# fuxiao0719/PanopticNeRF

Hardware: AMD Instinct MI355X
Metric: Msamples/sec (coarse+fine), KITTI-360 1408x376 (higher is better)
Workload: dtype bf16

## Files before the change

include/pnr.h:

```cpp
#ifndef PNR_H
#define PNR_H
#include <stdint.h>

#ifdef __cplusplus
extern "C" {
#endif

#define PNR_OK 0
#define PNR_EINVAL (-1)
#define PNR_EHIP (-2)
#define PNR_ENODEV (-3)

#define PNR_PREC_BF16 0
#define PNR_PREC_FP32 1

int pnr_version(void);
const char* pnr_last_error(void);
int pnr_device_check(int dev, char* buf_host, int buflen);

int pnr_stratified(const float* rays, int64_t n_rays, int n_samples, int lindisp,
                   const float* t_rand, float* z_out, void* stream);

int pnr_points(const float* rays, const float* z, int64_t n_rays, int n_samples, float* pts_out,
               void* stream);

int pnr_embed(const float* x, int64_t n, int L, float* out, void* stream);

typedef struct pnr_mlp_desc {
    int32_t D, W, skip;
    int32_t xyz_L, dir_L;
    int32_t n_sem, n_inst, head_W;
    int32_t precision;
    int32_t plan;
    int32_t head_tap;
    int32_t head_depth;
    int32_t schedule;
    int32_t clk_probe[2];
    int32_t flags;
} pnr_mlp_desc;

#define PNR_MLP_SOFTMAX 1
#define PNR_MLP_WG_CAP(n) (((n) & 0x1FF) << 16)
#define PNR_MLP_TRACE 0x7A00

typedef struct pnr_mlp_params_host {
    const float* const* pts_w; const float* const* pts_b;
    const float* alpha_w; const float* alpha_b;
    const float* feature_w; const float* feature_b;
    const float* views_w; const float* views_b;
    const float* rgb_w; const float* rgb_b;
    const float* sem0_w; const float* sem0_b; const float* sem1_w; const float* sem1_b;
    const float* inst0_w; const float* inst0_b; const float* inst1_w; const float* inst1_b;
} pnr_mlp_params_host;

int64_t pnr_mlp_packed_bytes(const pnr_mlp_desc* desc);
int pnr_mlp_pack(const pnr_mlp_desc* desc, const pnr_mlp_params_host* params, void* packed_host);

int64_t pnr_mlp_pack_workspace_bytes(const pnr_mlp_desc* desc, int backward);
int pnr_mlp_pack_device(const pnr_mlp_desc* desc, const pnr_mlp_params_host* params_dev, int backward,
                        void* workspace, void* packed, void* stream);
int pnr_mlp_repack_device(const pnr_mlp_desc* desc, const pnr_mlp_params_host* params_dev, int backward,
                          void* workspace, void* packed, void* stream);

int pnr_mlp_forward(const pnr_mlp_desc* desc, const void* packed, const float* rays, const float* z,
                    int64_t n_rays, int n_samples, float* raw, int64_t raw_stride_s,
                    int64_t raw_stride_c, void* stream);

int pnr_mlp_fused_plan(const pnr_mlp_desc* desc);
int64_t pnr_mlp_forward_composite_workspace_bytes(const pnr_mlp_desc* desc, int64_t n_rays, int n_samples, int want_weights);
int pnr_mlp_forward_composite(const pnr_mlp_desc* desc, const void* packed, const float* rays, const float* z,
                              int64_t n_rays, int n_samples, const int32_t* label_sem, const int32_t* label_inst,
                              int white_bkgd, float* rgb, float* depth, float* acc, float* weights, float* sem,
                              float* inst, float* fix_sem, float* fix_inst, void* workspace, void* stream);

int pnr_mlp_forward_tiles(const pnr_mlp_desc* desc, const void* packed, const float* rays, const float* z, int64_t n_rays,
                          int n_samples, void* workspace, void* stream);
int pnr_composite_combine(const pnr_mlp_desc* desc, const void* workspace, const float* z, int64_t n_rays, int n_samples,
                          const int32_t* label_sem, const int32_t* label_inst, int white_bkgd, float* rgb, float* depth,
                          float* acc, float* weights, float* sem, float* inst, float* fix_sem, float* fix_inst, void* stream);

int pnr_mlp_query(const pnr_mlp_desc* desc, const void* packed, const float* points, int64_t n_points,
                  float* sigma, int32_t* sem_label, int32_t* inst_label, int32_t* panoptic, const int32_t* is_thing,
                  float* sem_logits, float* inst_logits, int64_t logit_stride, void* stream);
int pnr_mlp_query_supported(const pnr_mlp_desc* desc);

int pnr_mlp_train_layout(const pnr_mlp_desc* desc, int64_t n_samples, int64_t* acts_off_host ,
                         int64_t* dys_off_host );
int pnr_mlp_forward_train(const pnr_mlp_desc* desc, const void* packed, const float* rays, const float* z,
                          int64_t n_rays, int n_samples, float* raw, int64_t raw_stride_s,
                          int64_t raw_stride_c, void* acts, void* stream);
int64_t pnr_mlp_bwd_packed_bytes(const pnr_mlp_desc* desc);
int pnr_mlp_pack_bwd(const pnr_mlp_desc* desc, const pnr_mlp_params_host* params, void* packed_host);
int pnr_mlp_backward(const pnr_mlp_desc* desc, const void* packed_bwd, const float* d_raw, const void* acts,
                     void* dys, int64_t n_rays, int n_samples, void* stream);

int64_t pnr_mlp_wgrad_workspace_bytes(const pnr_mlp_desc* desc, int64_t n_samples);
int pnr_mlp_wgrad(const pnr_mlp_desc* desc, const void* acts, const void* dys, int64_t n_samples,
                  const pnr_mlp_params_host* grads_dev, void* workspace, void* stream);

int64_t pnr_mlp_fp32_acts_floats(const pnr_mlp_desc* desc, int64_t n_samples);
int64_t pnr_mlp_backward_fp32_workspace_bytes(const pnr_mlp_desc* desc, int64_t n_samples);
int pnr_mlp_forward_train_fp32(const pnr_mlp_desc* desc, const pnr_mlp_params_host* params_dev, const float* rays,
                               const float* z, int64_t n_rays, int n_samples, float* raw, int64_t raw_stride_s,
                               int64_t raw_stride_c, float* acts, void* stream);
int pnr_mlp_backward_fp32(const pnr_mlp_desc* desc, const pnr_mlp_params_host* params_dev, const float* d_raw,
                          int64_t d_raw_stride_c, const float* acts, int64_t n_rays, int n_samples,
                          const pnr_mlp_params_host* grads_dev, void* workspace, void* stream);

int pnr_composite(const float* raw, int64_t raw_stride_s, int64_t raw_stride_c, const float* z,
                  const float* rays, const float* noise, const int32_t* label_sem,
                  const int32_t* label_inst, int64_t n_rays, int n_samples, int n_sem, int n_inst,
                  int sem_mode, int white_bkgd, float* rgb, float* depth, float* acc, float* weights,
                  float* sem, float* inst, float* fix_sem, float* fix_inst, void* stream);

int pnr_composite_backward(const float* raw, int64_t raw_stride_c, const float* z, const float* rays,
                           const float* noise, int64_t n_rays, int n_samples, int n_sem, int n_inst,
                           const float* g_rgb, const float* g_depth, const float* g_acc, const float* g_sem,
                           const float* g_inst, const float* g_weights, float* d_raw, void* stream);

int pnr_composite_backward2(const float* raw, int64_t raw_stride_c, const float* z, const float* rays,
                            const float* noise, int64_t n_rays, int n_samples, int n_sem, int n_inst,
                            const float* g_rgb, const float* g_depth, const float* g_acc, const float* g_sem,
                            const float* g_inst, const float* g_weights, const int32_t* label_sem,
                            const int32_t* label_inst, const float* g_fix_sem, const float* g_fix_inst,
                            const float* ce_sem, const float* ce_inst, float* d_raw, void* stream);
int pnr_composite_backward3(const float* raw, int64_t raw_stride_c, const float* z, const float* rays,
                            const float* noise, int64_t n_rays, int n_samples, int n_sem, int n_inst, int sem_mode,
                            const float* g_rgb, const float* g_depth, const float* g_acc, const float* g_sem,
                            const float* g_inst, const float* g_weights, const int32_t* label_sem,
                            const int32_t* label_inst, const float* g_fix_sem, const float* g_fix_inst,
                            const float* ce_sem, const float* ce_inst, float* d_raw, void* stream);

typedef struct pnr_loss_cfg {
    float w_rgb, w_depth, w_sem, w_fix_sem, w_inst, w_fix_inst;
    int32_t depth_l2;
    float fix_eps;
    int32_t maps_are_prob;
} pnr_loss_cfg;
int64_t pnr_losses_workspace_bytes(int64_t n_rays);
int pnr_losses(const pnr_loss_cfg* cfg, int64_t n_rays, int n_sem, int n_inst, const float* rgb, const float* depth,
               const float* sem, const float* fix_sem, const float* inst, const float* fix_inst, const float* rgb_gt,
               const float* depth_gt, const int32_t* sem_gt, const int32_t* inst_gt, float* losses_out, float* g_rgb,
               float* g_depth, float* g_sem, float* g_fix_sem, float* g_inst, float* g_fix_inst, void* workspace, void* stream);

int64_t pnr_ce3d_workspace_bytes(int64_t n_samples);
int pnr_ce3d(const float* raw, int64_t raw_stride_c, int first_channel, int n_classes, const int32_t* label,
             int64_t n_samples, float* out2, void* workspace, void* stream);

int pnr_gen_rays(const float* intr4_host, const float* c2w12_host, int width, int height, float near_, float far_,
                 const int32_t* pix, int64_t n_rays, float* rays, void* stream);

#define PNR_FISHEYE_NEWTON_STEPS 8
#define PNR_CAMERA_PINHOLE 0
#define PNR_CAMERA_FISHEYE 1
#define PNR_CAMERA_EQUIRECT 3

#define PNR_SINPI_P0 0x1.921fb6p+1f
#define PNR_SINPI_P1 -0x1.4abbcep+2f
#define PNR_SINPI_P2 0x1.466bc6p+1f
#define PNR_SINPI_P3 -0x1.32d2ccp-1f
#define PNR_SINPI_P4 0x1.507834p-4f
#define PNR_COSPI_Q0 0x1.000000p+0f
#define PNR_COSPI_Q1 -0x1.3bd3ccp+2f
#define PNR_COSPI_Q2 0x1.03c1f0p+2f
#define PNR_COSPI_Q3 -0x1.55d3c8p+0f
#define PNR_COSPI_Q4 0x1.e1f506p-3f
#define PNR_COSPI_Q5 -0x1.a6d1f2p-6f
#define PNR_ATANPI_A0 0x1.45f306p-2f
#define PNR_ATANPI_A1 -0x1.b29948p-4f
#define PNR_ATANPI_A2 0x1.04bc78p-4f
#define PNR_ATANPI_A3 -0x1.7352dap-5f
#define PNR_ATANPI_A4 0x1.13b6a6p-5f
#define PNR_ATANPI_A5 -0x1.3ab9c6p-6f
#define PNR_TAN_PI_8 0x1.a8279ap-2f

int pnr_gen_rays_fisheye(const float* cam7_host, const float* c2w12_host, int width, int height, float near_, float far_,
                         const int32_t* pix, int64_t n_rays, float* rays, uint8_t* valid, void* stream);

int pnr_gen_rays_equirect(const float* cam4_host, const float* c2w12_host, int width, int height, float near_, float far_,
                          const int32_t* pix, int64_t n_rays, float* rays, void* stream);

int pnr_project_points(int model, const float* cam_host, const float* w2c12_host, int width, int height, const float* points,
                       int64_t n, float* uv, float* range, uint8_t* valid, void* stream);

int pnr_reproject(int model_src, const float* cam_src_host, const float* c2w_src12_host, int width_src, int height_src,
                  const int32_t* pix, int64_t n, const float* depth_src,
                  int model_tgt, const float* cam_tgt_host, const float* w2c_tgt12_host, int width_tgt, int height_tgt,
                  const float* depth_tgt, float tol_abs, float tol_rel,
                  const int32_t* label_src, const int32_t* label_tgt, int n_classes,
                  int32_t* match, float* uv, int64_t* agree, int64_t* stats, void* stream);

int pnr_splat_points(int model, const float* cam_host, const float* w2c12_host, int width, int height, const float* points,
                     int64_t n, int64_t index_base, float near_, float far_, int radius, int64_t* zbuf, int64_t* stats,
                     void* stream);
int pnr_splat_resolve(const int64_t* zbuf, int64_t n_pix, float* depth, int32_t* index, void* stream);
int64_t pnr_depth_metrics_workspace_bytes(int64_t n);
int pnr_depth_metrics(const float* pred, const float* gt, const uint8_t* mask, int64_t n, float d_min, float d_max,
                      double* sums, int64_t* counts, void* workspace, void* stream);

int pnr_census(const uint8_t* img, int width, int height, int64_t* out, void* stream);
int64_t pnr_sgm_workspace_bytes(int width, int height, int max_disp, int paths);
int pnr_sgm_aggregate(const int64_t* census_l, const int64_t* census_r, int width, int height, int max_disp, int p1, int p2,
                      int paths, uint16_t* S, void* workspace, void* stream);
int pnr_sgm_select(const uint16_t* S, int width, int height, int max_disp, int uniqueness, int lr_tol, int16_t* d16,
                   int16_t* disp_right, void* stream);
int pnr_disparity_depth(const int16_t* d16, int64_t n, float fb, float d_min, float d_max, float* depth, void* stream);

int64_t pnr_mesh_workspace_bytes(int res_x, int res_y, int res_z);
int pnr_mesh_count(const float* field, int res_x, int res_y, int res_z, float level, void* workspace, int64_t* totals, void* stream);
int pnr_mesh_emit(const float* field, int res_x, int res_y, int res_z, float level, const float* lo_host, const float* step_host,
                  const void* workspace, float* vertices, int32_t* faces, int64_t* src, void* stream);

#define PNR_NN_PAD 1.0009765625f
#define PNR_NN_CELL_CLAMP 1048576.0f
#define PNR_NN_HASH_X 73856093u
#define PNR_NN_HASH_Y 19349663u
#define PNR_NN_HASH_Z 83492791u
#define PNR_NN_MAX_TABLE 268435456
#define PNR_CLOUD_MAX_TAU 8
#define PNR_SAMPLE_MAX_PER_FACE 65535
int64_t pnr_nn_workspace_bytes(int64_t n, int64_t table_size);
int pnr_nn_build(const float* ref, int64_t n, float max_dist, int64_t table_size, int32_t* start, float* records, void* workspace,
                 void* stream);
int pnr_nn_query(const float* ref, int64_t n, float max_dist, int64_t table_size, const int32_t* start, const float* records,
                 const float* query, int64_t m, int32_t* index, float* dist2, int64_t* stats, void* stream);
int64_t pnr_cloud_metrics_workspace_bytes(int64_t m);
int pnr_cloud_metrics(const int32_t* index, const float* dist2, const float* query, int64_t m, float max_dist,
                      const float* tau_host, int n_tau, double* sums, int64_t* counts, void* workspace, void* stream);
int64_t pnr_mesh_sample_workspace_bytes(int64_t n_faces);
int pnr_mesh_sample_count(const float* vertices, int64_t n_vertices, const int32_t* faces, int64_t n_faces, float rho, int64_t seed,
                          int32_t* start, int64_t* total, void* workspace, void* stream);
int pnr_mesh_sample_emit(const float* vertices, int64_t n_vertices, const int32_t* faces, int64_t n_faces, int64_t seed,
// ... 175 lines not shown
```

panopticnerf_amd/_lib.py:

```python
import ctypes
import os

_HERE = os.path.dirname(os.path.abspath(__file__))
LIB_PATH = os.environ.get("PNR_LIB_PATH") or os.path.join(_HERE, "libpnr.so")

c_f = ctypes.c_void_p
c_i64 = ctypes.c_int64
c_int = ctypes.c_int

PREC_BF16, PREC_FP32 = 0, 1
MLP_SOFTMAX, MLP_TRACE = 1, 0x7A00
CAMERA_PINHOLE, CAMERA_FISHEYE, CAMERA_EQUIRECT = 0, 1, 3
TAG_PIXEL, TAG_FRAME = 16, 17
SAMPLE_POOLED, SAMPLE_FRAME = 0, 1
NORMAL_OK, NORMAL_NO_DEPTH, NORMAL_NO_NEIGHBOUR, NORMAL_DEGENERATE, NORMAL_GRAZING = 0, 1, 2, 3, 4
MESHCAST_MAX_RES, MESHCAST_MAX_REACH, MESHCAST_PAD = 1024, 4096.0, 0.0625
DEPTH_MAX_RADIUS = 8
CC_KEYS, CC_VALUES = 0, 1
CC_TILE_2D, CC_TILE_3D = (32, 8), (8, 8, 4)
NN_MAX_TABLE, CLOUD_MAX_TAU, SAMPLE_MAX_PER_FACE = 1 << 28, 8, 65535


class LossCfg(ctypes.Structure):
    _fields_ = [("w_rgb", ctypes.c_float), ("w_depth", ctypes.c_float), ("w_sem", ctypes.c_float),
# ... 12 lines not shown
class RngDesc(ctypes.Structure):
    _fields_ = [("call", ctypes.c_void_p), ("ray_base", ctypes.c_int64), ("tag", ctypes.c_int32), ("scale", ctypes.c_float)]


class Frame(ctypes.Structure):
    _fields_ = [("model", ctypes.c_int32), ("width", ctypes.c_int32), ("height", ctypes.c_int32), ("cam", ctypes.c_float * 7),
                ("c2w", ctypes.c_float * 12), ("near_", ctypes.c_float), ("far_", ctypes.c_float), ("n_valid", ctypes.c_int64),
                ("valid_pix", ctypes.c_uint64), ("rgb", ctypes.c_uint64), ("depth", ctypes.c_uint64), ("sem", ctypes.c_uint64),
                ("inst", ctypes.c_uint64)]


_fp = ctypes.POINTER(ctypes.c_float)
_fpp = ctypes.POINTER(_fp)


class MlpParamsHost(ctypes.Structure):
    _fields_ = [("pts_w", _fpp), ("pts_b", _fpp),
                ("alpha_w", _fp), ("alpha_b", _fp), ("feature_w", _fp), ("feature_b", _fp),
                ("views_w", _fp), ("views_b", _fp), ("rgb_w", _fp), ("rgb_b", _fp),
                ("sem0_w", _fp), ("sem0_b", _fp), ("sem1_w", _fp), ("sem1_b", _fp),
                ("inst0_w", _fp), ("inst0_b", _fp), ("inst1_w", _fp), ("inst1_b", _fp)]


SIGNATURES = {
    "pnr_version": (c_int, []),
    "pnr_last_error": (ctypes.c_char_p, []),
    "pnr_device_check": (c_int, [c_int, ctypes.c_char_p, c_int]),
    "pnr_stratified": (c_int, [c_f, c_i64, c_int, c_int, c_f, c_f, c_f]),
    "pnr_points": (c_int, [c_f, c_f, c_i64, c_int, c_f, c_f]),
    "pnr_embed": (c_int, [c_f, c_i64, c_int, c_f, c_f]),
    "pnr_mlp_packed_bytes": (c_i64, [ctypes.POINTER(MlpDesc)]),
    "pnr_mlp_pack": (c_int, [ctypes.POINTER(MlpDesc), ctypes.POINTER(MlpParamsHost), ctypes.c_void_p]),
    "pnr_mlp_pack_workspace_bytes": (c_i64, [ctypes.POINTER(MlpDesc), c_int]),
    "pnr_mlp_pack_device": (c_int, [ctypes.POINTER(MlpDesc), ctypes.POINTER(MlpParamsHost), c_int, c_f, c_f, c_f]),
    "pnr_mlp_repack_device": (c_int, [ctypes.POINTER(MlpDesc), ctypes.POINTER(MlpParamsHost), c_int, c_f, c_f, c_f]),
    "pnr_mlp_forward": (c_int, [ctypes.POINTER(MlpDesc), c_f, c_f, c_f, c_i64, c_int, c_f, c_i64, c_i64, c_f]),
    "pnr_mlp_train_layout": (c_int, [ctypes.POINTER(MlpDesc), c_i64, ctypes.POINTER(c_i64), ctypes.POINTER(c_i64)]),
    "pnr_mlp_forward_train": (c_int, [ctypes.POINTER(MlpDesc), c_f, c_f, c_f, c_i64, c_int, c_f, c_i64, c_i64, c_f, c_f]),
    "pnr_mlp_bwd_packed_bytes": (c_i64, [ctypes.POINTER(MlpDesc)]),
    "pnr_mlp_pack_bwd": (c_int, [ctypes.POINTER(MlpDesc), ctypes.POINTER(MlpParamsHost), ctypes.c_void_p]),
    "pnr_mlp_backward": (c_int, [ctypes.POINTER(MlpDesc), c_f, c_f, c_f, c_f, c_i64, c_int, c_f]),
    "pnr_mlp_wgrad_workspace_bytes": (c_i64, [ctypes.POINTER(MlpDesc), c_i64]),
    "pnr_mlp_wgrad": (c_int, [ctypes.POINTER(MlpDesc), c_f, c_f, c_i64, ctypes.POINTER(MlpParamsHost), c_f, c_f]),
    "pnr_mlp_fp32_acts_floats": (c_i64, [ctypes.POINTER(MlpDesc), c_i64]),
    "pnr_mlp_backward_fp32_workspace_bytes": (c_i64, [ctypes.POINTER(MlpDesc), c_i64]),
    "pnr_mlp_forward_train_fp32": (c_int, [ctypes.POINTER(MlpDesc), ctypes.POINTER(MlpParamsHost), c_f, c_f, c_i64, c_int, c_f, c_i64,
                                           c_i64, c_f, c_f]),
    "pnr_mlp_backward_fp32": (c_int, [ctypes.POINTER(MlpDesc), ctypes.POINTER(MlpParamsHost), c_f, c_i64, c_f, c_i64, c_int,
                                      ctypes.POINTER(MlpParamsHost), c_f, c_f]),
    "pnr_mlp_fused_plan": (c_int, [ctypes.POINTER(MlpDesc)]),
    "pnr_mlp_forward_composite_workspace_bytes": (c_i64, [ctypes.POINTER(MlpDesc), c_i64, c_int, c_int]),
    "pnr_mlp_forward_composite": (c_int, [ctypes.POINTER(MlpDesc), c_f, c_f, c_f, c_i64, c_int, c_f, c_f, c_int,
                                          c_f, c_f, c_f, c_f, c_f, c_f, c_f, c_f, c_f, c_f]),
    "pnr_composite": (c_int, [c_f, c_i64, c_i64, c_f, c_f, c_f, c_f, c_f, c_i64, c_int, c_int, c_int, c_int,
                              c_int, c_f, c_f, c_f, c_f, c_f, c_f, c_f, c_f, c_f]),
    "pnr_composite_backward": (c_int, [c_f, c_i64, c_f, c_f, c_f, c_i64, c_int, c_int, c_int,
                                       c_f, c_f, c_f, c_f, c_f, c_f, c_f, c_f]),
    "pnr_composite_backward2": (c_int, [c_f, c_i64, c_f, c_f, c_f, c_i64, c_int, c_int, c_int,
                                        c_f, c_f, c_f, c_f, c_f, c_f, c_f, c_f, c_f, c_f, c_f, c_f, c_f, c_f]),
    "pnr_composite_backward3": (c_int, [c_f, c_i64, c_f, c_f, c_f, c_i64, c_int, c_int, c_int, c_int,
                                        c_f, c_f, c_f, c_f, c_f, c_f, c_f, c_f, c_f, c_f, c_f, c_f, c_f, c_f]),
    "pnr_losses_workspace_bytes": (c_i64, [c_i64]),
    "pnr_losses": (c_int, [ctypes.POINTER(LossCfg), c_i64, c_int, c_int] + [c_f] * 19),
    "pnr_ce3d_workspace_bytes": (c_i64, [c_i64]),
    "pnr_ce3d": (c_int, [c_f, c_i64, c_int, c_int, c_f, c_i64, c_f, c_f, c_f]),
    "pnr_gen_rays": (c_int, [ctypes.POINTER(ctypes.c_float), ctypes.POINTER(ctypes.c_float), c_int, c_int, ctypes.c_float,
                             ctypes.c_float, c_f, c_i64, c_f, c_f]),
    "pnr_gen_rays_fisheye": (c_int, [ctypes.POINTER(ctypes.c_float), ctypes.POINTER(ctypes.c_float), c_int, c_int, ctypes.c_float,
                                     ctypes.c_float, c_f, c_i64, c_f, c_f, c_f]),
    "pnr_gen_rays_equirect": (c_int, [ctypes.POINTER(ctypes.c_float), ctypes.POINTER(ctypes.c_float), c_int, c_int, ctypes.c_float,
                                      ctypes.c_float, c_f, c_i64, c_f, c_f]),
    "pnr_project_points": (c_int, [c_int, ctypes.POINTER(ctypes.c_float), ctypes.POINTER(ctypes.c_float), c_int, c_int, c_f, c_i64,
                                   c_f, c_f, c_f, c_f]),
    "pnr_reproject": (c_int, [c_int, ctypes.POINTER(ctypes.c_float), ctypes.POINTER(ctypes.c_float), c_int, c_int, c_f, c_i64, c_f,
                              c_int, ctypes.POINTER(ctypes.c_float), ctypes.POINTER(ctypes.c_float), c_int, c_int, c_f,
                              ctypes.c_float, ctypes.c_float, c_f, c_f, c_int, c_f, c_f, c_f, c_f, c_f]),
    "pnr_splat_points": (c_int, [c_int, ctypes.POINTER(ctypes.c_float), ctypes.POINTER(ctypes.c_float), c_int, c_int, c_f, c_i64, c_i64,
                                 ctypes.c_float, ctypes.c_float, c_int, c_f, c_f, c_f]),
    "pnr_splat_resolve": (c_int, [c_f, c_i64, c_f, c_f, c_f]),
    "pnr_depth_metrics_workspace_bytes": (c_i64, [c_i64]),
    "pnr_depth_metrics": (c_int, [c_f, c_f, c_f, c_i64, ctypes.c_float, ctypes.c_float, c_f, c_f, c_f, c_f]),
    "pnr_census": (c_int, [c_f, c_int, c_int, c_f, c_f]),
    "pnr_sgm_workspace_bytes": (c_i64, [c_int, c_int, c_int, c_int]),
    "pnr_sgm_aggregate": (c_int, [c_f, c_f, c_int, c_int, c_int, c_int, c_int, c_int, c_f, c_f, c_f]),
    "pnr_sgm_select": (c_int, [c_f, c_int, c_int, c_int, c_int, c_int, c_f, c_f, c_f]),
    "pnr_disparity_depth": (c_int, [c_f, c_i64, ctypes.c_float, ctypes.c_float, ctypes.c_float, c_f, c_f]),
    "pnr_mesh_workspace_bytes": (c_i64, [c_int, c_int, c_int]),
    "pnr_mesh_count": (c_int, [c_f, c_int, c_int, c_int, ctypes.c_float, c_f, c_f, c_f]),
    "pnr_mesh_emit": (c_int, [c_f, c_int, c_int, c_int, ctypes.c_float, ctypes.POINTER(ctypes.c_float), ctypes.POINTER(ctypes.c_float),
                              c_f, c_f, c_f, c_f, c_f]),
    "pnr_nn_workspace_bytes": (c_i64, [c_i64, c_i64]),
    "pnr_nn_build": (c_int, [c_f, c_i64, ctypes.c_float, c_i64, c_f, c_f, c_f, c_f]),
    "pnr_nn_query": (c_int, [c_f, c_i64, ctypes.c_float, c_i64, c_f, c_f, c_f, c_i64, c_f, c_f, c_f, c_f]),
    "pnr_cloud_metrics_workspace_bytes": (c_i64, [c_i64]),
    "pnr_cloud_metrics": (c_int, [c_f, c_f, c_f, c_i64, ctypes.c_float, ctypes.POINTER(ctypes.c_float), c_int, c_f, c_f, c_f, c_f]),
    "pnr_cc_workspace_bytes": (c_i64, [c_i64]),
    "pnr_cc_label": (c_int, [c_f, c_int, ctypes.c_float, c_int, c_int, c_int, c_int, c_f, c_f, c_f, c_f, c_f]),
    "pnr_cc_mesh": (c_int, [c_f, c_i64, c_i64, c_f, c_f, c_f, c_f, c_f, c_f]),
    "pnr_cc_stats": (c_int, [c_f, c_f, c_int, c_int, c_int, c_i64, c_f, c_f, c_f]),
    "pnr_mesh_sample_workspace_bytes": (c_i64, [c_i64]),
    "pnr_mesh_sample_count": (c_int, [c_f, c_i64, c_f, c_i64, ctypes.c_float, c_i64, c_f, c_f, c_f, c_f]),
    "pnr_mesh_sample_emit": (c_int, [c_f, c_i64, c_f, c_i64, c_i64, c_f, c_i64, c_f, c_f, c_f]),
    "pnr_mesh_grid_workspace_bytes": (c_i64, [c_int, c_int, c_int]),
    "pnr_mesh_grid_bounds": (c_int, [c_f, c_i64, c_f, c_i64, c_f, c_f, c_f]),
    "pnr_mesh_grid_count": (c_int, [c_f, c_i64, c_f, c_i64, c_int, c_int, c_int, ctypes.POINTER(ctypes.c_float), ctypes.POINTER(ctypes.c_float),
                                    c_f, c_f, c_f, c_f]),
    "pnr_mesh_grid_fill": (c_int, [c_f, c_i64, c_f, c_i64, c_int, c_int, c_int, ctypes.POINTER(ctypes.c_float), ctypes.POINTER(ctypes.c_float),
                                   c_f, c_i64, c_f, c_f, c_f]),
    "pnr_mesh_raycast": (c_int, [c_int, ctypes.POINTER(ctypes.c_float), ctypes.POINTER(ctypes.c_float), c_int, c_int, ctypes.c_float,
                                 ctypes.c_float, c_f, c_i64, c_f, c_i64, c_int, c_int, c_int, ctypes.POINTER(ctypes.c_float),
                                 ctypes.POINTER(ctypes.c_float), c_f, c_f, c_i64, c_f, c_f, c_f, c_f, c_f, c_f, c_f, c_f]),
    "pnr_mesh_cast_rays": (c_int, [c_f, c_i64, c_f, c_i64, c_f, c_i64, c_int, c_int, c_int, ctypes.POINTER(ctypes.c_float),
                                   ctypes.POINTER(ctypes.c_float), c_f, c_f, c_i64, c_f, c_f, c_f, c_f, c_f, c_f, c_f, c_f]),
    "pnr_tsdf_integrate": (c_int, [c_f, c_f, c_int, c_int, c_int, c_int, c_int, ctypes.POINTER(ctypes.c_float), ctypes.POINTER(ctypes.c_float),
                                   ctypes.c_float, ctypes.c_float, ctypes.c_float, c_f, c_f, c_f, c_f, c_f, c_f, c_f]),
    "pnr_tsdf_raycast": (c_int, [c_int, ctypes.POINTER(ctypes.c_float), ctypes.POINTER(ctypes.c_float), c_int, c_int, ctypes.c_float,
                                 ctypes.c_float, c_int, c_int, c_int, ctypes.POINTER(ctypes.c_float), ctypes.POINTER(ctypes.c_float),
                                 c_f, c_f, ctypes.c_float, ctypes.c_float, c_int, c_f, c_f, c_f, c_f, c_f]),
    "pnr_icp_workspace_bytes": (c_i64, [c_i64]),
    "pnr_icp_accumulate": (c_int, [c_int, ctypes.POINTER(ctypes.c_float), c_int, c_int, c_f, c_f, c_int, ctypes.POINTER(ctypes.c_float),
                                   ctypes.POINTER(ctypes.c_float), ctypes.POINTER(ctypes.c_float), c_int, c_int, c_f, c_f, ctypes.c_float,
                                   c_f, c_f, c_f, c_f]),
    "pnr_icp_solve": (c_int, [c_f, c_i64, c_i64, ctypes.c_float, ctypes.c_float, c_int, c_f, c_f, c_f]),
    "pnr_depth_filter": (c_int, [c_int, c_int, c_f, c_int, ctypes.POINTER(ctypes.c_float), ctypes.c_float, ctypes.c_float, c_int, c_f, c_f, c_f]),
    "pnr_depth_normals": (c_int, [c_int, ctypes.POINTER(ctypes.c_float), ctypes.POINTER(ctypes.c_float), c_int, c_int, c_f, ctypes.c_float,
                                  ctypes.c_float, ctypes.c_float, c_f, c_f, c_f, c_f]),
    "pnr_panoptic_labels": (c_int, [c_f, c_f, c_f, c_i64, c_int, c_int, c_f, c_f, c_f, c_f]),
    "pnr_confusion": (c_int, [c_f, c_f, c_i64, c_int, c_f, c_f]),
    "pnr_sample_pdf": (c_int, [c_f, c_f, c_f, c_i64, c_int, c_int, c_f, c_f, c_f, c_f]),
    "pnr_bbox_hits": (c_int, [c_f, c_i64, c_f, c_int, c_int, c_f, c_f, c_f, c_f]),
    "pnr_convex_hits": (c_int, [c_f, c_i64, c_f, c_f, c_int, c_int, c_f, c_f, c_f, c_f]),
    "pnr_restrict_rays": (c_int, [c_f, c_i64, c_f, c_f, c_int, c_f, c_f]),
    "pnr_sample_labels": (c_int, [c_f, c_i64, c_int, c_f, c_f, c_f, c_int, c_f, c_f, c_f, c_f]),
    "pnr_ray_setup": (c_int, [c_f, c_i64, c_f, c_int, c_int, c_f, c_int, c_int, c_f, c_int, c_f, c_f, c_f, c_f, c_f, c_f, c_f]),
    "pnr_sample_pdf_labels": (c_int, [c_f, c_f, c_f, c_i64, c_int, c_int, c_f, c_f, c_f, c_f, c_int, c_f, c_f, c_f, c_f]),
    "pnr_mlp_forward_tiles": (c_int, [ctypes.POINTER(MlpDesc), c_f, c_f, c_f, c_i64, c_int, c_f, c_f]),
    "pnr_rng_begin": (c_int, [c_f, c_f, c_f]),
    "pnr_rng_fill": (c_int, [ctypes.POINTER(RngDesc), c_i64, c_int, c_int, c_f, c_f]),
    "pnr_stratified_rng": (c_int, [c_f, c_i64, c_int, c_int, ctypes.POINTER(RngDesc), c_f, c_f]),
    "pnr_ray_setup_rng": (c_int, [c_f, c_i64, c_f, c_int, c_int, c_f, c_int, c_int, ctypes.POINTER(RngDesc), c_int, c_f, c_f, c_f, c_f,
                                  c_f, c_f, c_f]),
    "pnr_sample_pdf_rng": (c_int, [c_f, c_f, ctypes.POINTER(RngDesc), c_i64, c_int, c_int, c_f, c_f, c_f, c_f]),
    "pnr_sample_pdf_labels_rng": (c_int, [c_f, c_f, ctypes.POINTER(RngDesc), c_i64, c_int, c_int, c_f, c_f, c_f, c_f, c_int, c_f, c_f, c_f,
                                          c_f]),
    "pnr_composite_rng": (c_int, [c_f, c_i64, c_i64, c_f, c_f, ctypes.POINTER(RngDesc), c_f, c_f, c_i64, c_int, c_int, c_int, c_int,
                                  c_int, c_f, c_f, c_f, c_f, c_f, c_f, c_f, c_f, c_f]),
    "pnr_composite_backward_rng": (c_int, [c_f, c_i64, c_f, c_f, ctypes.POINTER(RngDesc), c_i64, c_int, c_int, c_int, c_int,
                                           c_f, c_f, c_f, c_f, c_f, c_f, c_f, c_f, c_f, c_f, c_f, c_f, c_f, c_f]),
    "pnr_sample_batch": (c_int, [c_f, c_f, c_f, c_int, ctypes.POINTER(RngDesc), c_i64, c_f, c_f, c_f, c_f, c_f, c_f, c_f, c_f]),
    "pnr_mlp_query": (c_int, [ctypes.POINTER(MlpDesc), c_f, c_f, c_i64, c_f, c_f, c_f, c_f, c_f, c_f, c_f, c_i64, c_f]),
    "pnr_mlp_query_supported": (c_int, [ctypes.POINTER(MlpDesc)]),
    "pnr_composite_combine": (c_int, [ctypes.POINTER(MlpDesc), c_f, c_f, c_i64, c_int, c_f, c_f, c_int,
                                      c_f, c_f, c_f, c_f, c_f, c_f, c_f, c_f, c_f]),
}

_lib = None


def load():
    global _lib
    if _lib is not None:
        return _lib
    if not os.path.exists(LIB_PATH):
        raise RuntimeError(
            f"{LIB_PATH} not found: the HIP extension is not built. Run "
            "`python -c 'import __graft_entry__ as g; g.build()'` (or `make -C panopticnerf_amd/csrc`). "
            "There is no CPU fallback.")
    lib = ctypes.CDLL(LIB_PATH)
    for name, (res, args) in SIGNATURES.items():
        fn = getattr(lib, name)
        fn.restype = res
        fn.argtypes = args
    _lib = lib
    return lib


def check(rc, what):
    if rc != 0:
        msg = load().pnr_last_error().decode(errors="replace")
        raise RuntimeError(f"{what} failed (code {rc}): {msg}")
```

panopticnerf_amd/csrc/pnr_composite.hip:

```cpp
#include "pnr_composite_dev.h"

struct CompositeArgs {
    const float* raw; int64_t stride_s, stride_c;
    const float* z; const float* rays; const float* noise;
    const int32_t* label_sem; const int32_t* label_inst;
    int64_t R; int N, C, K, sem_mode, white_bkgd;
    float *rgb, *depth, *acc, *weights, *sem, *inst, *fix_sem, *fix_inst;
    int use_hist;
};

#ifndef CMP_GRID_PER_CU
#define CMP_GRID_PER_CU 8
#endif
#ifndef CMP_UB
#define CMP_UB 8
#endif

__device__ __forceinline__ float dot4(const f4& w, const f4& v)
{
    return fmaf(w.v[3], v.v[3], fmaf(w.v[2], v.v[2], fmaf(w.v[1], v.v[1], w.v[0] * v.v[0])));
}

template <bool CH_MAJOR, int SUB, bool SOFTMAX, class... Rng>
__global__ __launch_bounds__(256) void k_composite(CompositeArgs a, const Rng... rng)
// ... 145 lines not shown
            add_sigma_noise4<RNG>(w + 4 * j, act[j], key, (uint32_t)ray, (uint32_t)((i0 >> 2) + j), a.noise, a.noise + s0 + 4 * j);
        const float dn = ray_dir_norm(a.rays, rl.rayc);
        const float znext = dpp_or<0x101>(zz[0], 0.0f);
        float alpha[M], Tl[M];
        float P = alpha_chain<M>(zz, znext, w, i0, N, dn, alpha, Tl);
        if (!act[0]) P = 1.0f;
        const float excl = scan_excl_dpp<L>(P, q);
        float accp = 0.0f, depp = 0.0f;
#pragma unroll
        for (int k = 0; k < M; ++k) {
            w[k] = act[k >> 2] ? (alpha[k] * Tl[k]) * excl : 0.0f;
            accp += w[k];
            depp = fmaf(w[k], zz[k], depp);
        }
        if (a.weights) {
#pragma unroll
            for (int j = 0; j < M4; ++j) st4(a.weights + s0 + 4 * j, w + 4 * j, act[j]);
        }
        const float accv = group_sum<L>(accp);
        const float depv = group_sum<L>(depp);
        if (writer) {
            if (a.depth) a.depth[ray] = depv;
            if (a.acc) a.acc[ray] = accv;
        }

        const bool want_fs = a.fix_sem && a.label_sem && a.C, want_fi = a.fix_inst && a.label_inst && a.K;
        if (want_fs || want_fi) {
            hist_zero<L>(hist, q, CK);
#pragma unroll
            for (int j = 0; j < M4; ++j) {
                int ls[4], li[4];
                ld4_labels(a.label_sem + s0 + 4 * j, act[j] && want_fs, ls);
                ld4_labels(a.label_inst + s0 + 4 * j, act[j] && want_fi, li);
#pragma unroll
                for (int k = 0; k < 4; ++k) hist_add(hist, w[4 * j + k], want_fs, ls[k], a.C, want_fi, li[k], a.K);
            }
            if (rl.valid) hist_store<L>(hist, q, ray, want_fs, a.fix_sem, a.C, want_fi, a.fix_inst, a.K);
        }

        float mx_s[SOFTMAX ? M : 1], den_s[SOFTMAX ? M : 1], mx_i[SOFTMAX ? M : 1], den_i[SOFTMAX ? M : 1];
        if constexpr (SOFTMAX) {
            auto field_stats = [&](int nch, int ch0, float (&mx)[M], float (&den)[M]) {
#pragma unroll
                for (int k = 0; k < M; ++k) { mx[k] = -INFINITY; den[k] = 0.0f; }
                for (int c = 0; c < nch; ++c) {
                    float v[M];
                    ld_row<M4>(a.raw + (int64_t)(ch0 + c) * sc + s0, act, v);
#pragma unroll
                    for (int k = 0; k < M; ++k) lse_step(mx[k], den[k], v[k]);
                }
            };
            field_stats(a.C, 4, mx_s, den_s);
            field_stats(a.K, 4 + a.C, mx_i, den_i);
        }

#pragma unroll 1
        for (int q0 = 0; q0 < nq; q0 += CMP2_UB) {
            float r[CMP2_UB];
#pragma unroll
            for (int j = 0; j < CMP2_UB; ++j) {
                const int qq = q0 + j;
                float acc = 0.0f;
#pragma unroll
                for (int k = 0; k < M; ++k) {
                    float v = nxt[j][k];
                    if (qq < 3) v = sigmoid_of(v);
                    else if constexpr (SOFTMAX) {
                        const bool fs = (qq - 3) < a.C;
                        v = softmax_of(v, fs ? mx_s[k] : mx_i[k], fs ? den_s[k] : den_i[k]);
                    }
                    acc = fmaf(w[k], v, acc);
                }
                r[j] = acc;
                const int q2 = qq + CMP2_UB;
                if (q2 < nq) ld_row<M4>(a.raw + (int64_t)(q2 + 1) * sc + s0, act, nxt[j]);
            }
            group_sum_batch<L, CMP2_UB>(r);
            if (writer) store_rows<CMP2_UB>(a, ray, q0, nq, r, accv);
        }
    }
}

static int composite_impl(const float* raw, int64_t raw_stride_s, int64_t raw_stride_c, const float* z, const float* rays,
                          const float* noise, const PnrRngDev* rng, const int32_t* label_sem, const int32_t* label_inst, int64_t n_rays,
                          int n_samples, int n_sem, int n_inst, int sem_mode, int white_bkgd, float* rgb, float* depth, float* acc,
                          float* weights, float* sem, float* inst, float* fix_sem, float* fix_inst, void* stream)
{
    PNR_REQUIRE(n_rays <= 0 || (raw && z && rays), "pnr_composite: null pointer");
    PNR_REQUIRE(n_samples >= 4 && n_samples <= 256 && (n_samples % 4) == 0,
                "pnr_composite: n_samples=%d must be a multiple of 4 in [4,256]", n_samples);
    PNR_REQUIRE(n_sem >= 0 && n_inst >= 0 && (sem_mode == 0 || sem_mode == 1), "pnr_composite: bad field sizes");
    PNR_REQUIRE((((uintptr_t)z) & 15) == 0, "pnr_composite: z must be 16-byte aligned");
    PNR_REQUIRE(!weights || (((uintptr_t)weights) & 15) == 0, "pnr_composite: weights must be 16-byte aligned");
    PNR_REQUIRE((((uintptr_t)noise) & 15) == 0 && (((uintptr_t)label_sem) & 15) == 0 && (((uintptr_t)label_inst) & 15) == 0,
                "pnr_composite: noise / label arrays must be 16-byte aligned");
    if (n_rays <= 0) return PNR_OK;
    CompositeArgs a;
    a.raw = raw; a.stride_s = raw_stride_s; a.stride_c = raw_stride_c; a.z = z; a.rays = rays; a.noise = noise;
    a.label_sem = label_sem; a.label_inst = label_inst; a.R = n_rays; a.N = n_samples; a.C = n_sem; a.K = n_inst;
    a.sem_mode = sem_mode; a.white_bkgd = white_bkgd; a.rgb = rgb; a.depth = depth; a.acc = acc; a.weights = weights;
    a.sem = sem; a.inst = inst; a.fix_sem = fix_sem; a.fix_inst = fix_inst;
    const bool want_fix = (fix_sem && label_sem && n_sem) || (fix_inst && label_inst && n_inst);
    const bool ch_major = raw_stride_s == 1 && (raw_stride_c % 4) == 0 && (((uintptr_t)raw) & 15) == 0;
    hipStream_t st = (hipStream_t)stream;
    auto hist_bytes = [&](int rpw) { return (size_t)4 * rpw * (n_sem + n_inst) * sizeof(uint32_t); };
    auto grid_for = [&](int rpw) { return pnr_grid_cap(((n_rays + rpw - 1) / rpw + 3) / 4, CMP_GRID_PER_CU); };
    if (ch_major && n_samples > 32 && n_samples <= 64 && (!want_fix || hist_bytes(8) <= 48 * 1024)) {
        a.use_hist = want_fix ? 1 : 0;
        const size_t lds = want_fix ? hist_bytes(8) : 0;
        composite_dispatch<8>(8, true, sem_mode, rng, [&](auto L, auto, auto SM, const auto&... r) {
            hipLaunchKernelGGL((k_composite2<decltype(L)::value, 2, decltype(SM)::value, std::decay_t<decltype(r)>...>), dim3(grid_for(8)), dim3(256),
                               lds, st, a, r...);
        });
        PNR_CHECK_LAUNCH("pnr_composite");
        return PNR_OK;
    }
    int sub = 1;
    while (sub < n_samples / 4) sub <<= 1;
    const int rpw = 64 / sub;
    a.use_hist = (want_fix && hist_bytes(rpw) <= 48 * 1024) ? 1 : 0;
    const size_t lds = a.use_hist ? hist_bytes(rpw) : 0;
    composite_dispatch<1, 2, 4, 8, 16, 32, 64>(sub, ch_major, sem_mode, rng, [&](auto S, auto CH, auto SM, const auto&... r) {
        hipLaunchKernelGGL((k_composite<decltype(CH)::value, decltype(S)::value, decltype(SM)::value, std::decay_t<decltype(r)>...>),
                           dim3(grid_for(rpw)), dim3(256), lds, st, a, r...);
    });
    PNR_CHECK_LAUNCH("pnr_composite");
    return PNR_OK;
}

PNR_EXPORT int pnr_composite(const float* raw, int64_t raw_stride_s, int64_t raw_stride_c, const float* z,
                             const float* rays, const float* noise, const int32_t* label_sem,
                             const int32_t* label_inst, int64_t n_rays, int n_samples, int n_sem, int n_inst,
                             int sem_mode, int white_bkgd, float* rgb, float* depth, float* acc, float* weights,
                             float* sem, float* inst, float* fix_sem, float* fix_inst, void* stream)
{
    return composite_impl(raw, raw_stride_s, raw_stride_c, z, rays, noise, nullptr, label_sem, label_inst, n_rays, n_samples, n_sem, n_inst,
                          sem_mode, white_bkgd, rgb, depth, acc, weights, sem, inst, fix_sem, fix_inst, stream);
}

PNR_EXPORT int pnr_composite_rng(const float* raw, int64_t raw_stride_s, int64_t raw_stride_c, const float* z, const float* rays,
                                 const pnr_rng* noise_host, const int32_t* label_sem, const int32_t* label_inst, int64_t n_rays,
                                 int n_samples, int n_sem, int n_inst, int sem_mode, int white_bkgd, float* rgb, float* depth, float* acc,
                                 float* weights, float* sem, float* inst, float* fix_sem, float* fix_inst, void* stream)
{
    PnrRngDev rng;
    const int rc = pnr_rng_check(noise_host, n_rays < 0 ? 0 : n_rays, "pnr_composite_rng", &rng);
    if (rc) return rc;
    PNR_REQUIRE(n_rays <= 0 || (raw_stride_s == 1 && (raw_stride_c % 4) == 0 && (((uintptr_t)raw) & 15) == 0),
                "pnr_composite_rng: channel-major, 16-byte aligned raw images only");
    return composite_impl(raw, raw_stride_s, raw_stride_c, z, rays, nullptr, &rng, label_sem, label_inst, n_rays, n_samples, n_sem, n_inst,
                          sem_mode, white_bkgd, rgb, depth, acc, weights, sem, inst, fix_sem, fix_inst, stream);
}

struct CombineArgs {
    const float* rec; int rec_floats; const float4* ps; const float* z; const int32_t* lab_s; const int32_t* lab_i;
    int64_t R; int N, C, K, white_bkgd;
    float *rgb, *depth, *acc, *weights, *sem, *inst, *fix_sem, *fix_inst;
};

template <bool LOGITS>
__global__ __launch_bounds__(256) void k_composite_combine(CombineArgs a)
{
    __shared__ uint32_t hist_all[4][128];
    const int lane = threadIdx.x & 63, wv = threadIdx.x >> 6;
    const int64_t ray = ((int64_t)blockIdx.x * blockDim.x + threadIdx.x) >> 6;
    if (ray >= a.R) return;
    const int N = a.N, T = N >> 5, RF = a.rec_floats, C = a.C, K = a.K, CK = C + K;
    const float* __restrict__ rec = a.rec + ray * T * RF;
    const float4* __restrict__ ps = a.ps + ray * N;
    const float* __restrict__ zr = a.z + ray * N;
    const bool want_s = a.lab_s && a.fix_sem && C, want_i = a.lab_i && a.fix_inst && K;
    const int32_t* __restrict__ lsr = want_s ? a.lab_s + ray * N : nullptr;
    const int32_t* __restrict__ lir = want_i ? a.lab_i + ray * N : nullptr;
    float q[8];
#pragma unroll
    for (int k = 0; k < 8; ++k) q[k] = k < T ? rec[k * RF] : 1.0f;
    float4 pv[4];
    float zv[4];
    int lsv[4], liv[4];
#pragma unroll
    for (int j = 0; j < 4; ++j) {
        const int i = lane + 64 * j;
        const bool in = i < N;
        pv[j] = in ? ps[i] : float4{0.0f, 0.0f, 0.0f, 0.0f};
        zv[j] = in ? zr[i] : 0.0f;
        lsv[j] = (in && want_s) ? lsr[i] : -1;
        liv[j] = (in && want_i) ? lir[i] : -1;
    }
    float lg[2][8];
#pragma unroll
    for (int h = 0; h < 2; ++h)
#pragma unroll
        for (int k = 0; k < 8; ++k) lg[h][k] = (LOGITS && k < T && lane + 64 * h < CK) ? rec[k * RF + PNR_FUSE_REC_LOGITS + lane + 64 * h] : 0.0f;
    float Tk[8];
    float t = 1.0f;
#pragma unroll
    for (int k = 0; k < 8; ++k) {
        Tk[k] = t;
        if (k < T) t *= q[k];
    }
    uint32_t* hist = hist_all[wv];
    if (want_s || want_i) hist_zero<64>(hist, lane, CK);
    float r5[5] = {0.0f, 0.0f, 0.0f, 0.0f, 0.0f};
#pragma unroll
    for (int j = 0; j < 4; ++j) {
        const int i = lane + 64 * j;
        if (i < N) {
            const float4 p = pv[j];
            float tk = Tk[0];
#pragma unroll
            for (int k = 1; k < 8; ++k) tk = (i >> 5) == k ? Tk[k] : tk;
            const float w = tk * p.x;
            r5[0] += w;
            r5[1] = fmaf(w, zv[j], r5[1]);
            r5[2] = fmaf(w, sigmoid_of(p.y), r5[2]);
            r5[3] = fmaf(w, sigmoid_of(p.z), r5[3]);
            r5[4] = fmaf(w, sigmoid_of(p.w), r5[4]);
            if (a.weights) a.weights[ray * N + i] = w;
            if (want_s || want_i) hist_add(hist, w, want_s, lsv[j], C, want_i, liv[j], K);
        }
    }
    group_sum_batch<64, 5>(r5);
    if (lane == 0) {
        if (a.acc) a.acc[ray] = r5[0];
        if (a.depth) a.depth[ray] = r5[1];
    }
    if (lane < 3 && a.rgb) {
        const float v = lane == 0 ? r5[2] : lane == 1 ? r5[3] : r5[4];
        a.rgb[ray * 3 + lane] = a.white_bkgd ? v + (1.0f - r5[0]) : v;
    }
#pragma unroll
    for (int h = 0; h < 2; ++h) {
        const int c = lane + 64 * h;
        if (c >= CK) continue;
        if constexpr (LOGITS) {
            float v = 0.0f;
#pragma unroll
            for (int k = 0; k < 8; ++k) if (k < T) v = fmaf(Tk[k], lg[h][k], v);
            if (c < C) { if (a.sem) a.sem[ray * C + c] = v; }
            else if (a.inst) a.inst[ray * K + (c - C)] = v;
        }
        if (c < C) { if (want_s) a.fix_sem[ray * C + c] = hist_read(hist, c); }
        else if (want_i) a.fix_inst[ray * K + (c - C)] = hist_read(hist, c);
    }
}

int pnr_composite_combine_launch(const float* rec, int rec_floats, bool logit_sums, const float4* ps, const float* z,
                                 const int32_t* label_sem, const int32_t* label_inst, int64_t R, int N, int C, int K, int white_bkgd,
                                 float* rgb, float* depth, float* acc, float* weights, float* sem, float* inst, float* fix_sem,
                                 float* fix_inst, hipStream_t st)
{
    CombineArgs a;
    a.rec = rec; a.rec_floats = rec_floats; a.ps = ps; a.z = z; a.lab_s = label_sem; a.lab_i = label_inst;
    a.R = R; a.N = N; a.C = C; a.K = K; a.white_bkgd = white_bkgd;
    a.rgb = rgb; a.depth = depth; a.acc = acc; a.weights = weights; a.sem = sem; a.inst = inst; a.fix_sem = fix_sem; a.fix_inst = fix_inst;
    const int64_t blocks = (R + 3) / 4;
    if (logit_sums) hipLaunchKernelGGL(k_composite_combine<true>, dim3((unsigned)blocks), dim3(256), 0, st, a);
    else hipLaunchKernelGGL(k_composite_combine<false>, dim3((unsigned)blocks), dim3(256), 0, st, a);
    PNR_CHECK_LAUNCH("pnr_mlp_forward_composite (combine)");
    return PNR_OK;
}
```

panopticnerf_amd/csrc/pnr_composite_dev.h:

```cpp
#pragma once
#include <type_traits>

#include "pnr_common.h"
#include "pnr_fuse_record.h"
#include "pnr_lane_ops.h"
#include "pnr_philox.h"

struct f4 { float v[4]; };

__device__ __forceinline__ f4 ld4(const float* p, bool active)
{
    f4 o;
    if (!active) { o.v[0] = o.v[1] = o.v[2] = o.v[3] = 0.0f; return o; }
    const float4 t = *reinterpret_cast<const float4*>(p);
    o.v[0] = t.x; o.v[1] = t.y; o.v[2] = t.z; o.v[3] = t.w;
    return o;
}
__device__ __forceinline__ void st4(float* p, const float* v, bool active)
{
    if (active) *reinterpret_cast<float4*>(p) = make_float4(v[0], v[1], v[2], v[3]);
}
template <class T>
__device__ __forceinline__ T* row_at(T* row, uint32_t ob)
{
// ... 25 lines not shown
    }
}

__device__ __forceinline__ void ld4_labels(const int32_t* p, bool on, int (&l)[4])
{
    l[0] = l[1] = l[2] = l[3] = -1;
    if (on) { const int4 t = *reinterpret_cast<const int4*>(p); l[0] = t.x; l[1] = t.y; l[2] = t.z; l[3] = t.w; }
}

template <int L, int M4>
struct RayLanes {
    static constexpr int RPW = 64 / L;
    int q, g, i0;
    int64_t n_groups;
    int64_t ray, rayc, s0;
    bool valid, act[M4];

    __device__ __forceinline__ RayLanes(int64_t R)
    {
        const int lane = threadIdx.x & 63;
        q = lane & (L - 1);
        g = lane / L;
        i0 = q * 4 * M4;
        n_groups = (R + RPW - 1) / RPW;
    }
    __device__ __forceinline__ void at(int64_t grp, int64_t R, int N)
    {
        ray = grp * RPW + g;
        valid = ray < R;
        rayc = valid ? ray : R - 1;
#pragma unroll
        for (int j = 0; j < M4; ++j) act[j] = valid && (i0 + 4 * j < N);
        s0 = rayc * N + (act[0] ? i0 : 0);
    }
};

__device__ __forceinline__ float ray_dir_norm(const float* rays, int64_t ray)
{
    const float dx = rays[ray * 8 + 3], dy = rays[ray * 8 + 4], dz = rays[ray * 8 + 5];
    return sqrtf((dx * dx + dy * dy) + dz * dz);
}

template <bool RNG>
__device__ __forceinline__ void add_sigma_noise4(float* sg, bool active, const PnrRngKey& key, uint32_t ray, uint32_t blk, bool have, const float* np)
{
    if constexpr (RNG) {
        if (active) {
            float n[4];
            pnr_rng_normal4(key, ray, blk, n);
#pragma unroll
            for (int k = 0; k < 4; ++k) sg[k] += n[k];
        }
    } else if (have) {
        const f4 t = ld4(np, active);
#pragma unroll
        for (int k = 0; k < 4; ++k) sg[k] += t.v[k];
    }
}

__device__ __forceinline__ float sample_dist(bool last, float z, float znext, float dn)
{
    float dist = last ? 1e10f : (znext - z);
    dist *= dn;
    return dist;
}
__device__ __forceinline__ float sample_alpha(float sigma, float dist) { return 1.0f - expf(-(fmaxf(sigma, 0.0f) * dist)); }
__device__ __forceinline__ float alpha_factor(float alpha) { return (1.0f - alpha) + 1e-10f; }

template <int M>
__device__ __forceinline__ float alpha_chain(const float (&z)[M], float znext, const float (&sg)[M], int i0, int N, float dn,
                                             float (&alpha)[M], float (&Tl)[M], float* dist = nullptr)
{
    float P = 1.0f;
#pragma unroll
    for (int k = 0; k < M; ++k) {
        const float d = sample_dist(!(i0 + k + 1 < N), z[k], (k < M - 1) ? z[k + 1] : znext, dn);
        if (dist) dist[k] = d;
        alpha[k] = sample_alpha(sg[k], d);
        Tl[k] = P;
        P *= alpha_factor(alpha[k]);
    }
    return P;
}

__device__ __forceinline__ float sigmoid_of(float v) { return 1.0f / (1.0f + expf(-v)); }

template <int SUB>
__device__ __forceinline__ float scan_excl_shfl(float P, int q)
{
    float x = P;
#pragma unroll
    for (int d = 1; d < SUB; d <<= 1) {
        const float y = __shfl_up(x, d, 64);
        if (q >= d) x *= y;
    }
    float excl = __shfl_up(x, 1, 64);
    if (q == 0) excl = 1.0f;
    return excl;
}
template <int L>
__device__ __forceinline__ float scan_excl_dpp(float P, int q)
{
    static_assert(L == 8 || L == 16, "a ray must sit inside one 16-lane DPP row");
    float x = P;
    float y = dpp_or<0x111>(x, 1.0f); x *= (L == 16 || q >= 1) ? y : 1.0f;
    y = dpp_or<0x112>(x, 1.0f); x *= (L == 16 || q >= 2) ? y : 1.0f;
    y = dpp_or<0x114>(x, 1.0f); x *= (L == 16 || q >= 4) ? y : 1.0f;
    if constexpr (L == 16) { y = dpp_or<0x118>(x, 1.0f); x *= y; }
    float excl = dpp_or<0x111>(x, 1.0f);
    if (q == 0) excl = 1.0f;
    return excl;
}

template <int L>
__device__ __forceinline__ void hist_zero(uint32_t* hist, int q, int CK)
{
    for (int c = q; c < CK; c += L) hist[c] = 0;
}
__device__ __forceinline__ void hist_add(uint32_t* hist, float w, bool want_s, const int& ls, int C, bool want_i, const int& li, int K)
{
    const uint32_t fx = (uint32_t)(w * PNR_FUSE_FIX_SCALE + 0.5f);
    if (want_s) { const int l = ls; if (l >= 0 && l < C) atomicAdd(&hist[l], fx); }
    if (want_i) { const int l = li; if (l >= 0 && l < K) atomicAdd(&hist[C + l], fx); }
}
__device__ __forceinline__ float hist_read(const uint32_t* hist, int c) { return (float)hist[c] * (1.0f / PNR_FUSE_FIX_SCALE); }
template <int L>
__device__ __forceinline__ void hist_store(const uint32_t* hist, int q, int64_t ray, bool want_s, float* fix_sem, int C, bool want_i, float* fix_inst, int K)
{
    if (want_s) for (int c = q; c < C; c += L) fix_sem[ray * C + c] = hist_read(hist, c);
    if (want_i) for (int c = q; c < K; c += L) fix_inst[ray * K + c] = hist_read(hist, C + c);
}

__device__ __forceinline__ void lse_step(float& mx, float& den, float v)
{
    const float d = v - mx, e = expf(-fabsf(d));
    den = d <= 0.0f ? den + e : den * e + 1.0f;
    mx = fmaxf(mx, v);
}
__device__ __forceinline__ float softmax_of(float v, float mx, float den) { return expf(v - mx) / den; }

template <int UB, class Args>
__device__ __forceinline__ void store_rows(const Args& a, int64_t ray, int q0, int nq, const float (&r)[UB], float accv)
{
#pragma unroll
    for (int j = 0; j < UB; ++j) {
        const int qq = q0 + j;
        if (qq >= nq) continue;
        if (qq < 3) { if (a.rgb) a.rgb[ray * 3 + qq] = a.white_bkgd ? r[j] + (1.0f - accv) : r[j]; }
        else if (qq - 3 < a.C) { if (a.sem) a.sem[ray * a.C + (qq - 3)] = r[j]; }
        else { if (a.inst) a.inst[ray * a.K + (qq - 3 - a.C)] = r[j]; }
    }
}

template <int... SUBS, class F>
static void composite_dispatch(int sub, bool ch_major, bool softmax, const PnrRngDev* rng, F&& launch)
{
    auto one = [&](auto S) {
        auto mode = [&](auto SM) {
            if (rng) launch(S, std::true_type{}, SM, *rng);
            else if (ch_major) launch(S, std::true_type{}, SM);
            else launch(S, std::false_type{}, SM);
        };
        if (softmax) mode(std::true_type{}); else mode(std::false_type{});
    };
    ((sub == SUBS ? one(std::integral_constant<int, SUBS>{}) : void()), ...);
}
```

panopticnerf_amd/csrc/pnr_mlp.hip:

```cpp
#include <stdlib.h>
#include <string.h>

#include "pnr_mlp_plan.h"

int pnr_mlp_validate(const pnr_mlp_desc* d);

#include "pnr_mlp_core.h"
#include "pnr_mlp_pp.h"
#include "pnr_mlp_fuse.h"
#include "pnr_mlp_tt.h"
#define PNR_QUERY_MAX_POINTS (((int64_t)1 << 31) - 4096)
template <int PREC, int TILES, class CTX, int KIND, int NA, int NB, int NFB_OUT, int MODE, int NOUT>
__device__ __forceinline__ void layer_regs(CTX& c, const uint32_t (&inA)[TILES][NA],
                                           const uint32_t (&inB)[TILES][NB > 0 ? NB : 1],
                                           uint32_t (&out)[TILES][NOUT], uint16_t* save = nullptr,
                                           const int* srow = nullptr)
{
    constexpr int RPB = PrecT<PREC>::RPB;
    constexpr int KS = NA / 4 + NB / 4;
    constexpr int FBC0 = pnr_layer_fbc(KIND, PREC);
    constexpr int FBC = (NFB_OUT % FBC0 == 0) ? FBC0 : 1;
    constexpr int G = (CTX::GDB / FBC) < 1 ? 1 : (CTX::GDB / FBC);
    static_assert(NOUT >= NFB_OUT * RPB, "output register array too small");
#pragma unroll
// ... 628 lines not shown
    u32x4 A[CTX::P];
    auto fetch = [&](int grp) { return fetch_sample<true>(a, grp * WAVES + c.wave, n); };
    SampleIn nextin = fetch(blockIdx.x < a.n_groups ? blockIdx.x : 0);
    FuseState fst;
    uint32_t ex[GXR];
    float dn_next;
    {
        float px, py, pz;
        sample_point(nextin, px, py, pz, dn_next);
        embed_lane<PNR_PREC_BF16, 5, 32, GXR>(px, py, pz, c.hi, ex);
    }

    for (int grp = blockIdx.x; grp < a.n_groups; grp += gridDim.x) {
        const int s0 = (grp * WAVES + c.wave) * 32 + n;
        const int samp = s0 < a.S ? s0 : -1;
        fst.zz = nextin.zz; fst.zn = nextin.zn; fst.dn = dn_next; fst.samp = samp; fst.last = nextin.last;
        fst.rec = a.rec + (int64_t)(grp * WAVES + c.wave) * a.rec_floats;
        uint32_t nxt[HR];
        pp_trunk_staged<W, 4>(c, A, grp, s0, ex, nxt, [&](int g2) { nextin = fetch(g2); },
                              [&](float& x, float& y, float& z) { sample_point(nextin, x, y, z, dn_next); });
        pp_layer_out<false, true, CTX, HR, 0>(c, A, nxt, dummy, 4, 0, samp, &fst);
#if PNR_TRACE
        ++c.titer;
#endif
    }
    pp_end(c, clk_c0, clk_r0);
}

static int pp_lds_bytes(const MlpArgs& m) { return 3 * m.slot_bytes + (PNR_TRACE ? 8 * PNR_TRACE_CHUNKS * PNR_TRACE_STAMPS * 8 : 0); }
static int pp_groups(int S) { return (S + 255) / 256; }
template <class ARGS>
static int launch_pp(void (*kern)(const ARGS), const ARGS& args, const MlpArgs& m, bool& attr_set, hipStream_t stream, const char* who)
{
    if (!attr_set) {
        PNR_HIP(hipFuncSetAttribute((const void*)kern, hipFuncAttributeMaxDynamicSharedMemorySize, 163840));
        attr_set = true;
    }
    const int cap = pnr_cu_count();
    const int grid = m.n_groups < cap ? m.n_groups : cap;
    hipLaunchKernelGGL(kern, dim3(grid), dim3(512), pp_lds_bytes(m), stream, args);
    PNR_CHECK_LAUNCH(who);
    return PNR_OK;
}

template <int W, bool TRAIN, bool FUSE = false, int TAIL = 0, bool SIGMA = false>
static int launch_mlp_pp(const MlpArgs& a0, hipStream_t stream)
{
    MlpArgs a = a0;
    PNR_REQUIRE(pp_lds_bytes(a) <= 163840, "pnr_mlp_forward: three weight slots of %d bytes exceed the 160 KiB LDS", a.slot_bytes);
    PNR_REQUIRE(a.n_chunks >= 4, "pnr_mlp_forward: network too small for the weight stream");
    a.n_groups = pp_groups(a.S);
    auto kern = k_mlp_pp<W, TRAIN, FUSE, TAIL>;
    if constexpr (SIGMA) kern = k_mlp_pp_sigma<W>;
    static thread_local bool attr_set = false;
    return launch_pp(kern, a, a, attr_set, stream, "pnr_mlp_forward");
}

template <int PREC, int W, int TILES, int WAVES, int MINW, bool TRAIN = false>
static int launch_mlp(const MlpArgs& a0, hipStream_t stream)
{
    MlpArgs a = a0;
    const int lds_bytes = 2 * a.slot_bytes + (PNR_TRACE ? WAVES * PNR_TRACE_CHUNKS * PNR_TRACE_STAMPS * 8 : 0);
    PNR_REQUIRE(lds_bytes <= 163840, "pnr_mlp_forward: weight double buffer of %d bytes exceeds the 160 KiB LDS", lds_bytes);
    PNR_REQUIRE(a.n_chunks >= 3, "pnr_mlp_forward: network too small for the weight stream");
    const int per_group = 32 * TILES * WAVES;
    a.n_groups = (a.S + per_group - 1) / per_group;
    auto kern = k_mlp_fused<PREC, W, TILES, WAVES, MINW, TRAIN>;
    static thread_local int wg_per_cu = 0;
    if (wg_per_cu == 0) {
        PNR_HIP(hipFuncSetAttribute((const void*)kern, hipFuncAttributeMaxDynamicSharedMemorySize, 163840));
        int nb = 0;
        PNR_HIP(hipOccupancyMaxActiveBlocksPerMultiprocessor(&nb, (const void*)kern, 64 * WAVES, lds_bytes));
        wg_per_cu = nb < 1 ? 1 : (nb > 4 ? 4 : nb);
    }
    const int cap = pnr_cu_count() * wg_per_cu;
    const int grid = a.n_groups < cap ? a.n_groups : cap;
    hipLaunchKernelGGL(kern, dim3(grid), dim3(64 * WAVES), lds_bytes, stream, a);
    PNR_CHECK_LAUNCH("pnr_mlp_forward");
    return PNR_OK;
}


static inline unsigned long long* clk_probe_of(const pnr_mlp_desc* d)
{
    return (unsigned long long*)(uintptr_t)(((uint64_t)(uint32_t)d->clk_probe[1] << 32) | (uint64_t)(uint32_t)d->clk_probe[0]);
}

static void mlp_args_fill(MlpArgs& a, const pnr_mlp_desc* desc, const PnrPlan& plan, const void* packed)
{
    memset(&a, 0, sizeof(a));
    a.data = (const uint8_t*)packed + plan.data_off;
    a.table = (const pnr_chunk_entry*)((const uint8_t*)packed + plan.table_off);
    a.n_chunks = (int)plan.chunks.size();
    a.slot_bytes = plan.max_chunk_frags * PNR_FRAG_BYTES;
    a.D = desc->D; a.skip = desc->skip; a.n_sem = desc->n_sem; a.n_inst = desc->n_inst;
    a.head_tap = desc->head_tap; a.head_depth = desc->head_depth == 1 ? 1 : 2;
    a.clk = clk_probe_of(desc);
#if PNR_TRACE
    if (const char* e = getenv("PNR_TRACE_PTR")) a.trace = (unsigned long long*)strtoull(e, nullptr, 0);
#endif
}

static int mlp_forward_impl(const pnr_mlp_desc* desc, const void* packed, const float* rays, const float* z,
                            int64_t n_rays, int n_samples, float* raw, int64_t raw_stride_s, int64_t raw_stride_c,
                            void* acts, void* stream)
{
    int rc = pnr_mlp_validate(desc);
    if (rc != PNR_OK) return rc;
    PNR_REQUIRE(n_rays >= 0 && n_samples >= 1, "pnr_mlp_forward: bad size");
    if (n_rays == 0) return PNR_OK;
    PNR_REQUIRE(packed && rays && z && raw, "pnr_mlp_forward: null pointer");
    PNR_REQUIRE(n_rays * (int64_t)n_samples < ((int64_t)1 << 31) - 4096, "pnr_mlp_forward: R*N=%lld exceeds 2^31",
                (long long)(n_rays * n_samples));
    PNR_REQUIRE((((uintptr_t)rays) & 15) == 0 && (((uintptr_t)packed) & 15) == 0 && (((uintptr_t)acts) & 15) == 0,
                "pnr_mlp_forward: rays / packed / acts must be 16-byte aligned");
    PNR_REQUIRE(!acts || desc->precision == PNR_PREC_BF16, "pnr_mlp_forward_train: the training path is bf16 only");
    PNR_REQUIRE(desc->plan != 4, "pnr_mlp_forward: a plan-4 (field) image is for pnr_mlp_query only");
    PNR_REQUIRE(desc->plan == 0, "pnr_mlp_forward: plan=%d images are for pnr_mlp_forward_composite only", desc->plan);
    PnrPlan plan;
    pnr_build_plan(*desc, plan);
    MlpArgs a;
    mlp_args_fill(a, desc, plan, packed);
    a.rays = rays; a.z = z; a.S = (int)(n_rays * n_samples); a.N = n_samples;
    pnr_set_div_magic(n_samples, a.n_magic, a.n_shift);
    a.raw = raw; a.ss = raw_stride_s; a.sc = raw_stride_c;
    a.acts = (uint16_t*)acts;
    if (acts) pnr_train_layout(*desc, a.S, a.acts_off, a.dys_off, a.gate_off);
    hipStream_t st = (hipStream_t)stream;
    if (desc->precision == PNR_PREC_BF16) {
        if (desc->schedule != 1 && !acts)
            return desc->W == 256 ? launch_mlp_pp<256, false>(a, st) : launch_mlp_pp<128, false>(a, st);
        if (desc->schedule == 2 && acts)
            return desc->W == 256 ? launch_mlp_pp<256, true>(a, st) : launch_mlp_pp<128, true>(a, st);
        if (acts)
            return desc->W == 256 ? launch_mlp<PNR_PREC_BF16, 256, 1, 8, 2, true>(a, st)
                                  : launch_mlp<PNR_PREC_BF16, 128, 1, 8, 2, true>(a, st);
        return desc->W == 256 ? launch_mlp<PNR_PREC_BF16, 256, 1, 8, 2>(a, st) : launch_mlp<PNR_PREC_BF16, 128, 1, 8, 2>(a, st);
    }
    return desc->W == 256 ? launch_mlp<PNR_PREC_FP32, 256, 1, 4, 1>(a, st) : launch_mlp<PNR_PREC_FP32, 128, 1, 4, 1>(a, st);
}

PNR_EXPORT int pnr_mlp_forward(const pnr_mlp_desc* desc, const void* packed, const float* rays, const float* z,
                               int64_t n_rays, int n_samples, float* raw, int64_t raw_stride_s,
                               int64_t raw_stride_c, void* stream)
{
    return mlp_forward_impl(desc, packed, rays, z, n_rays, n_samples, raw, raw_stride_s, raw_stride_c, nullptr, stream);
}

#define PNR_RAY_AUX_BYTES 128
int pnr_composite_combine_launch(const float* rec, int rec_floats, bool logit_sums, const float4* ps, const float* z,
                                 const int32_t* label_sem, const int32_t* label_inst, int64_t R, int N, int C, int K, int white_bkgd,
                                 float* rgb, float* depth, float* acc, float* weights, float* sem, float* inst, float* fix_sem,
                                 float* fix_inst, hipStream_t st);

static int record_floats(const pnr_mlp_desc& d)
{
    return d.plan == 3 ? pnr_fuse_record_floats(0, 0) : pnr_fuse_record_floats(d.n_sem, d.n_inst);
}

PNR_EXPORT int64_t pnr_mlp_forward_composite_workspace_bytes(const pnr_mlp_desc* desc, int64_t n_rays, int n_samples, int want_weights)
{
    (void)want_weights;
    if (pnr_mlp_validate(desc) != PNR_OK || n_rays < 0 || n_samples < 32 || (n_samples & 31)) return -1;
    const int64_t S = n_rays * n_samples, tiles = (S + 255) / 256 * 8;
    if (desc->plan == 3) return tiles * record_floats(*desc) * 4 + S * 16 + 256;
    return tiles * pnr_fuse_record_floats(desc->n_sem, desc->n_inst) * 4 + S * 16 + 256 + PNR_RAY_AUX_BYTES + n_rays * PNR_RAY_AUX_BYTES;
}

__global__ void __launch_bounds__(256) k_ray_aux(const float* __restrict__ rays, int64_t R, uint32_t* __restrict__ aux)
{
    const int64_t i = (int64_t)blockIdx.x * 256 + threadIdx.x;
    if (i >= 2 * R) return;
    const int64_t ray = i >> 1;
    const int hi = (int)(i & 1);
    const float dx = rays[ray * 8 + 3], dy = rays[ray * 8 + 4], dz = rays[ray * 8 + 5];
    const float nrm = sqrtf(__fadd_rn(__fadd_rn(__fmul_rn(dx, dx), __fmul_rn(dy, dy)), __fmul_rn(dz, dz)));
    uint32_t ed[8];
    embed_lane<PNR_PREC_BF16, 2, 16, 8>(dx / nrm, dy / nrm, dz / nrm, hi, ed);
    uint4* o = reinterpret_cast<uint4*>(aux + i * 16);
    o[0] = make_uint4(ed[0], ed[1], ed[2], ed[3]);
    o[1] = make_uint4(ed[4], ed[5], ed[6], ed[7]);
    o[2] = make_uint4(__float_as_uint(nrm), 0u, 0u, 0u);
}

static int fused_mlp_launch(const pnr_mlp_desc* desc, const void* packed, const float* rays, const float* z, int64_t n_rays,
                            int n_samples, void* workspace, void* stream, MlpArgs& a)
{
    int rc = pnr_mlp_validate(desc);
    if (rc != PNR_OK) return rc;
    PNR_REQUIRE(desc->precision == PNR_PREC_BF16, "pnr_mlp_forward_composite: bf16 only");
    PNR_REQUIRE(desc->plan != 4, "pnr_mlp_forward_composite: a plan-4 (field) image is for pnr_mlp_query only");
    PNR_REQUIRE(n_rays >= 1 && n_samples >= 32 && n_samples <= 256 && (n_samples & 31) == 0,
                "pnr_mlp_forward_composite: n_samples=%d must be a multiple of 32 in [32,256]", n_samples);
    PNR_REQUIRE(desc->n_sem + desc->n_inst <= 128, "pnr_mlp_forward_composite: n_sem + n_inst <= 128");
    PNR_REQUIRE(packed && rays && z && workspace, "pnr_mlp_forward_composite: null pointer");
    PNR_REQUIRE(n_rays * (int64_t)n_samples < ((int64_t)1 << 31) - 4096, "pnr_mlp_forward_composite: R*N exceeds 2^31");
    PNR_REQUIRE((((uintptr_t)rays | (uintptr_t)packed | (uintptr_t)workspace) & 15) == 0,
                "pnr_mlp_forward_composite: rays / packed / workspace must be 16-byte aligned");
    PnrPlan plan;
    pnr_build_plan(*desc, plan);
    mlp_args_fill(a, desc, plan, packed);
    a.rays = rays; a.z = z; a.S = (int)(n_rays * n_samples); a.N = n_samples;
    pnr_set_div_magic(n_samples, a.n_magic, a.n_shift);
    a.rec_floats = record_floats(*desc);
    a.rec = (float*)workspace;
    const int64_t tiles = ((int64_t)a.S + 255) / 256 * 8;
    a.ps = (float4*)(a.rec + tiles * a.rec_floats);
    hipStream_t st = (hipStream_t)stream;
    const bool softmax = (desc->flags & PNR_MLP_SOFTMAX) && desc->n_sem + desc->n_inst > 0;
    if (desc->plan == 3)
        return desc->W == 256 ? launch_mlp_pp<256, false, true, 0, true>(a, st) : launch_mlp_pp<128, false, true, 0, true>(a, st);
    if (desc->plan == 2) {
        PnrTTArgs t;
        memset(&t, 0, sizeof(t));
        t.image = a.data; t.rays = rays; t.z = z; t.S = a.S; t.N = a.N; t.n_magic = a.n_magic; t.n_shift = a.n_shift;
        t.rec = a.rec; t.rec_floats = a.rec_floats; t.ps = a.ps; t.n_sem = a.n_sem; t.n_inst = a.n_inst; t.clk = a.clk;
        PNR_REQUIRE(n_rays < ((int64_t)1 << 24), "pnr_mlp_forward_composite: the two-tile kernel addresses 2^24 rays per launch");
        uint32_t* aux = (uint32_t*)(((uintptr_t)((uint8_t*)a.ps + (int64_t)a.S * 16 + 256) + PNR_RAY_AUX_BYTES - 1)
                                    & ~(uintptr_t)(PNR_RAY_AUX_BYTES - 1));
        k_ray_aux<<<dim3((unsigned)((2 * n_rays + 255) / 256)), dim3(256), 0, st>>>(rays, n_rays, aux);
        t.aux = aux;
        t.n_wg = (desc->flags >> 16) & 0x1FF;
        const bool trace = (desc->flags & 0xFF00) == PNR_MLP_TRACE;
        return pnr_mlp_tt_launch(t, (desc->n_sem + 31) / 32, (desc->n_inst + 31) / 32, a.head_depth, a.head_tap, softmax, st, trace,
                                 trace ? ((desc->flags >> 4) & 7) : 0);
    }
    if (desc->plan == 1) {
        const int nbs = (desc->n_sem + 31) / 32, nbi = (desc->n_inst + 31) / 32;
        switch (4 * nbs + nbi + (softmax ? 16 : 0)) {
        case 4: return launch_mlp_pp<256, false, true, 4>(a, st);
        case 5: return launch_mlp_pp<256, false, true, 5>(a, st);
        case 8: return launch_mlp_pp<256, false, true, 8>(a, st);
        case 9: return launch_mlp_pp<256, false, true, 9>(a, st);
        case 20: return launch_mlp_pp<256, false, true, 20>(a, st);
        case 21: return launch_mlp_pp<256, false, true, 21>(a, st);
        case 24: return launch_mlp_pp<256, false, true, 24>(a, st);
        case 25: return launch_mlp_pp<256, false, true, 25>(a, st);
        default: PNR_REQUIRE(false, "pnr_mlp_forward_composite: no plan-1 kernel for %d + %d logit blocks", nbs, nbi);
        }
    }
    PNR_REQUIRE(!softmax, "pnr_mlp_forward_composite: softmax compositing needs the plan-1 image (pnr_mlp_fused_plan >= 1, desc.plan = 1)");
    return desc->W == 256 ? launch_mlp_pp<256, false, true>(a, st) : launch_mlp_pp<128, false, true>(a, st);
}

PNR_EXPORT int pnr_mlp_forward_tiles(const pnr_mlp_desc* desc, const void* packed, const float* rays, const float* z, int64_t n_rays,
                                     int n_samples, void* workspace, void* stream)
{
    PNR_REQUIRE(n_rays >= 0, "pnr_mlp_forward_tiles: bad size");
    if (n_rays == 0) return PNR_OK;
    MlpArgs a;
    return fused_mlp_launch(desc, packed, rays, z, n_rays, n_samples, workspace, stream, a);
}

PNR_EXPORT int pnr_composite_combine(const pnr_mlp_desc* desc, const void* workspace, const float* z, int64_t n_rays, int n_samples,
                                     const int32_t* label_sem, const int32_t* label_inst, int white_bkgd, float* rgb, float* depth,
                                     float* acc, float* weights, float* sem, float* inst, float* fix_sem, float* fix_inst, void* stream)
{
    int rc = pnr_mlp_validate(desc);
    if (rc != PNR_OK) return rc;
    PNR_REQUIRE(n_rays >= 0 && n_samples >= 32 && n_samples <= 256 && (n_samples & 31) == 0, "pnr_composite_combine: bad size");
    if (n_rays == 0) return PNR_OK;
    PNR_REQUIRE(workspace && z, "pnr_composite_combine: null pointer");
    PNR_REQUIRE(desc->plan != 4, "pnr_composite_combine: a plan-4 (field) image has no compositing workspace");
    PNR_REQUIRE((!fix_sem || label_sem) && (!fix_inst || label_inst), "pnr_composite_combine: fix_* outputs need their labels");
    PNR_REQUIRE(desc->plan != 3 || (!rgb && !sem && !inst), "pnr_composite_combine: a plan-3 (sigma-only) workspace has no rgb, semantic "
                "or instance maps: pass null for them");
    const int rf = record_floats(*desc);
    const int64_t tiles = (n_rays * n_samples + 255) / 256 * 8;
    const float* rec = (const float*)workspace;
    return pnr_composite_combine_launch(rec, rf, desc->plan != 3, (const float4*)(rec + tiles * rf), z, fix_sem ? label_sem : nullptr,
                                        fix_inst ? label_inst : nullptr, n_rays, n_samples, desc->n_sem, desc->n_inst, white_bkgd,
                                        rgb, depth, acc, weights, sem, inst, fix_sem, fix_inst, (hipStream_t)stream);
}

PNR_EXPORT int pnr_mlp_forward_composite(const pnr_mlp_desc* desc, const void* packed, const float* rays, const float* z,
                                         int64_t n_rays, int n_samples, const int32_t* label_sem, const int32_t* label_inst,
                                         int white_bkgd, float* rgb, float* depth, float* acc, float* weights, float* sem,
                                         float* inst, float* fix_sem, float* fix_inst, void* workspace, void* stream)
{
    PNR_REQUIRE(n_rays >= 0, "pnr_mlp_forward_composite: bad size");
    if (n_rays == 0) return PNR_OK;
    PNR_REQUIRE((!fix_sem || label_sem) && (!fix_inst || label_inst), "pnr_mlp_forward_composite: fix_* outputs need their labels");
    PNR_REQUIRE(!desc || desc->plan != 3 || (!rgb && !sem && !inst), "pnr_mlp_forward_composite: a plan-3 (sigma-only) image has no "
                "rgb, semantic or instance maps: pass null for them");
    MlpArgs a;
    int rc = fused_mlp_launch(desc, packed, rays, z, n_rays, n_samples, workspace, stream, a);
    if (rc != PNR_OK) return rc;
    return pnr_composite_combine_launch(a.rec, a.rec_floats, desc->plan != 3, a.ps, z, fix_sem ? label_sem : nullptr, fix_inst ? label_inst : nullptr,
                                        n_rays, n_samples, desc->n_sem, desc->n_inst, white_bkgd, rgb, depth, acc, weights, sem, inst,
                                        fix_sem, fix_inst, (hipStream_t)stream);
}

PNR_EXPORT int pnr_mlp_forward_train(const pnr_mlp_desc* desc, const void* packed, const float* rays, const float* z,
                                     int64_t n_rays, int n_samples, float* raw, int64_t raw_stride_s,
                                     int64_t raw_stride_c, void* acts, void* stream)
{
    PNR_REQUIRE(acts || n_rays == 0, "pnr_mlp_forward_train: acts is null");
    return mlp_forward_impl(desc, packed, rays, z, n_rays, n_samples, raw, raw_stride_s, raw_stride_c, acts, stream);
}

PNR_EXPORT int pnr_mlp_train_layout(const pnr_mlp_desc* desc, int64_t n_samples, int64_t* acts_off_host,
                                    int64_t* dys_off_host)
{
    int rc = pnr_mlp_validate(desc);
    if (rc != PNR_OK) return rc;
    PNR_REQUIRE(acts_off_host && dys_off_host && n_samples >= 0, "pnr_mlp_train_layout: bad arguments");
    int64_t a[24], d[24];
    pnr_train_layout(*desc, n_samples, a, d);
    memcpy(acts_off_host, a, sizeof(int64_t) * (size_t)(desc->D + 7));
    memcpy(dys_off_host, d, sizeof(int64_t) * (size_t)(desc->D + 8));
    return PNR_OK;
}

struct FieldArgs {
    MlpArgs m;
    const float* pts;
    float* sigma;
    int32_t* sem_label; int32_t* inst_label; int32_t* panoptic;
    const int32_t* is_thing;
    float* sem_logits; float* inst_logits; int64_t lstride;
    int run_sem, run_inst;
};

template <class CTX, int NA, class EPI>
__device__ __forceinline__ void pp_field_out(CTX& c, u32x4 (&A)[CTX::P], const uint32_t (&in)[NA], int n_out, EPI&& epi)
{
    using CH = PPChunk<1, NA, 0>;
    const uint32_t dummy[1] = {0};
    const int nfb = (n_out + 31) >> 5;
#pragma unroll 1
    for (int fb = 0; fb < nfb; ++fb) {
        f32x16 acc[1];
        CH::prologue(c.frag_addr(), c.bias_addr(), A, acc);
        CH::mma(c.frag_addr(), A, in, dummy, acc, [&](auto... k) { if constexpr (sizeof...(k) == 0) { c.stamp(6); c.barrier(); c.stamp(2); } else c.stamp(k...); });
        c.m_done();
        c.refill_begin();
        c.refill_one();
        epi(fb, acc[0]);
        c.refill_rest();
        c.advance();
    }
}

struct FieldBest { float v; int i; };
__device__ __forceinline__ void field_best_merge(FieldBest& b, int hi)
{
    const auto pv = __builtin_amdgcn_permlane32_swap(__float_as_uint(b.v), __float_as_uint(b.v), false, false);
    const auto pi = __builtin_amdgcn_permlane32_swap((uint32_t)b.i, (uint32_t)b.i, false, false);
    const float ov = __uint_as_float(hi ? pv[0] : pv[1]);
    const int oi = (int)(hi ? pi[0] : pi[1]);
    if (ov > b.v || (ov == b.v && oi < b.i)) { b.v = ov; b.i = oi; }
    if (b.i == 0x7fffffff) b.i = 0;
}

template <int W, bool HEADS>
__global__ __launch_bounds__(512, 2) void k_mlp_pp_field(const FieldArgs fa)
{
    constexpr int WAVES = 8;
    using CTX = CtxPP<WAVES>;
    extern __shared__ __attribute__((aligned(16))) char smem[];
    constexpr int NFB = W / 32, HFB = W / 64;
    constexpr int HR = NFB * 8, GR = HFB * 8, GXR = 16;
    const MlpArgs& a = fa.m;
    CTX c = pp_ctx<WAVES>(a, smem);
    unsigned long long clk_c0, clk_r0;
    pp_begin(c, clk_c0, clk_r0);
    const int n = c.lane & 31;

    uint32_t dummy[1] = {0};
    u32x4 A[CTX::P];
    struct PointIn { float x, y, z; };
    auto fetch_point = [&](int grp) {
        const int s = (grp * WAVES + c.wave) * 32 + n;
        const int sl = s < a.S ? s : a.S - 1;
        const float* p = fa.pts + (int64_t)sl * 3;
        PointIn in;
        in.x = p[0]; in.y = p[1]; in.z = p[2];
        return in;
    };
    PointIn nextin = fetch_point(blockIdx.x < a.n_groups ? blockIdx.x : 0);
    uint32_t ex[GXR];
    embed_lane<PNR_PREC_BF16, 5, 32, GXR>(__fadd_rn(nextin.x, 0.0f), __fadd_rn(nextin.y, 0.0f), __fadd_rn(nextin.z, 0.0f), c.hi, ex);

    for (int grp = blockIdx.x; grp < a.n_groups; grp += gridDim.x) {
        const int s0 = (grp * WAVES + c.wave) * 32 + n;
        const int samp = s0 < a.S ? s0 : -1;
        uint32_t nxt[HR];
        pp_trunk_staged<W, 1>(c, A, grp, s0, ex, nxt, [&](int g2) { nextin = fetch_point(g2); }, [&](float& x, float& y, float& z) {
            x = __fadd_rn(nextin.x, 0.0f); y = __fadd_rn(nextin.y, 0.0f); z = __fadd_rn(nextin.z, 0.0f);
        });
        pp_field_out<CTX, HR>(c, A, nxt, 4, [&](int, const f32x16& acc) {
            if (fa.sigma && samp >= 0 && c.hi == 0) fa.sigma[samp] = acc[3];
        });
        if constexpr (HEADS) {
            if (a.head_tap) {
                uint32_t ft[HR];
                pp_layer_regs<CTX, PNR_L_FEATURE, HR, 0, NFB, MODE_LINEAR, HR>(c, A, nxt, dummy, ft, nullptr, s0);
#pragma unroll
                for (int i = 0; i < HR; ++i) nxt[i] = ft[i];
            }
            int lab_sem = 0, lab_inst = -1;
#pragma unroll 1
            for (int hd = 0; hd < 2; ++hd) {
                if (!(hd ? fa.run_inst : fa.run_sem)) continue;
                const int n_out = hd ? a.n_inst : a.n_sem;
                float* const lg = hd ? fa.inst_logits : fa.sem_logits;
                FieldBest best{-INFINITY, 0x7fffffff};
                auto epi = [&](int fb, const f32x16& acc) {
                    const int lim = n_out - 4 * c.hi;
                    float* const dst0 = lg + ((int64_t)(4 * c.hi) * fa.lstride + (samp >= 0 ? samp : 0));
                    const bool st = lg != nullptr && samp >= 0;
#pragma unroll
                    for (int r = 0; r < 16; ++r) {
                        const int u = fb * 32 + (r & 3) + 8 * (r >> 2);
                        if (u < lim) {
                            if (st) dst0[(int64_t)u * fa.lstride] = acc[r];
                            const float v = acc[r] == acc[r] ? acc[r] : -INFINITY;
                            if (v > best.v) { best.v = v; best.i = u + 4 * c.hi; }
                        }
                    }
                };
                if (a.head_depth == 1) pp_field_out<CTX, HR>(c, A, nxt, n_out, epi);
                else {
                    uint32_t sh[GR];
                    pp_layer_regs<CTX, PNR_L_SEM0, HR, 0, HFB, MODE_RELU, GR>(c, A, nxt, dummy, sh, nullptr, s0);
                    pp_field_out<CTX, GR>(c, A, sh, n_out, epi);
                }
// ... 65 lines not shown
```

panopticnerf_amd/csrc/pnr_sampling.hip:

```cpp
#include "pnr_common.h"
#include "pnr_philox.h"
#include "pnr_sampling_dev.h"
#include <stdlib.h>
#include <string.h>

template <class... Rng>
__global__ __launch_bounds__(256) void k_stratified(const float* __restrict__ rays, int64_t R, int N,
                                                     int lindisp, const float* __restrict__ t_rand,
                                                     float* __restrict__ z_out, const Rng... rng)
{
    constexpr bool RNG = sizeof...(Rng) > 0;
    PnrRngKey key;
    if constexpr (RNG) key = pnr_rng_key(rng...);
    const int64_t total = R * N;
    for (int64_t s = (int64_t)blockIdx.x * blockDim.x + threadIdx.x; s < total;
         s += (int64_t)gridDim.x * blockDim.x) {
        const int64_t r = s / N;
        const int i = (int)(s - r * N);
        if constexpr (RNG) {
            const float t = pnr_rng_uniform_at(key, (uint32_t)r, i);
            z_out[s] = strat_sample(rays[r * 8 + 6], rays[r * 8 + 7], i, N, lindisp, &t);
        } else {
            z_out[s] = strat_sample(rays[r * 8 + 6], rays[r * 8 + 7], i, N, lindisp, t_rand ? t_rand + s : nullptr);
        }
    }
}

__global__ __launch_bounds__(256) void k_points(const float* __restrict__ rays, const float* __restrict__ z,
                                                 int64_t R, int N, float* __restrict__ pts)
{
    const int64_t total = R * N * 3;
    for (int64_t e = (int64_t)blockIdx.x * blockDim.x + threadIdx.x; e < total;
         e += (int64_t)gridDim.x * blockDim.x) {
        const int64_t s = e / 3;
        const int a = (int)(e - s * 3);
        const int64_t r = s / N;
        const float m = rays[r * 8 + 3 + a] * z[s];
        pts[e] = rays[r * 8 + a] + m;
    }
}

__global__ __launch_bounds__(256) void k_embed(const float* __restrict__ x, int64_t n, int L,
                                                float* __restrict__ out)
{
    const int E = 3 + 6 * L;
    const int64_t total = n * E;
    for (int64_t e = (int64_t)blockIdx.x * blockDim.x + threadIdx.x; e < total;
         e += (int64_t)gridDim.x * blockDim.x) {
        const int64_t s = e / E;
        const int c = (int)(e - s * E);
        float v;
        if (c < 3) {
            v = x[s * 3 + c];
        } else {
            const int k = (c - 3) / 6, j = (c - 3) - 6 * k;
            const int a = j % 3;
            const float arg = x[s * 3 + a] * ldexpf(1.0f, k);
            v = (j < 3) ? sinf(arg) : cosf(arg);
        }
        out[e] = v;
    }
}

struct PdfLabelArgs {
    const float* hit_t; const int32_t* hit_box; const int32_t* hit_count; int max_hits; const int32_t* box_ids;
    int32_t* label_sem; int32_t* label_inst;
};
#define PDF_MAXC 256
#define PDF_MAXT 512
template <int MAXC, int MAXT, class... Rng>
__device__ __forceinline__ void sample_pdf_body(const float* __restrict__ z, const float* __restrict__ weights,
                                                    const float* __restrict__ u, int64_t R, int Nc, int Nf,
                                                    float* __restrict__ zs_out, int32_t* __restrict__ inds_out,
                                                    float* __restrict__ zfine_out, const PdfLabelArgs lab, const Rng&... rng)
{
    constexpr bool RNG = sizeof...(Rng) > 0;
    PnrRngKey key;
    if constexpr (RNG) key = pnr_rng_key(rng...);
    __shared__ float s_z[MAXC], s_w[MAXC], s_pdf[MAXC], s_cdf[MAXC], s_bins[MAXC];
    __shared__ float s_sort[MAXT], s_out[MAXT];
    __shared__ float s_total, s_part[32];
    const int lane = threadIdx.x;
    const int nb = Nc - 1, nw = Nc - 2, Nt = Nc + Nf;
    const int P = pdf_padded(Nt);
    auto labels = [&](int64_t r, const float* sorted) {
        if (!lab.label_sem) return;
        const int mh = lab.max_hits;
        const int cnt = lab.hit_count[r] < mh ? lab.hit_count[r] : mh;
        for (int i = lane; i < Nt; i += 64) {
            const int best = label_hit(sorted[i], cnt, [&](int h, float& ti, float& to) {
                ti = lab.hit_t[(r * mh + h) * 2];
                to = lab.hit_t[(r * mh + h) * 2 + 1];
            });
            int ls, li;
            hit_ids(best, lab.hit_box + r * mh + best, lab.box_ids, &ls, &li);
            lab.label_sem[r * Nt + i] = ls;
            lab.label_inst[r * Nt + i] = li;
        }
    };
    for (int64_t r = blockIdx.x; r < R; r += gridDim.x) {
        for (int i = lane; i < Nc; i += 64) {
            s_z[i] = z[r * Nc + i];
            s_w[i] = weights[r * Nc + i];
        }
        __syncthreads();
        for (int k = lane; k < nb; k += 64) s_bins[k] = 0.5f * (s_z[k + 1] + s_z[k]);
        const float total = pdf_torch_total(s_w, nw, s_part, &s_total, lane);
        for (int j = lane; j < nw; j += 64) s_pdf[j] = (s_w[j + 1] + 1e-5f) / total;
        __syncthreads();
        pdf_cdf(lane < nw ? s_pdf[lane < nw ? lane : 0] : 0.0f, nw, nw <= 64, s_pdf, s_cdf, lane);
        for (int i = lane; i < Nf; i += 64) {
            float uu;
            if constexpr (RNG) uu = pnr_rng_uniform_at(key, (uint32_t)r, i);
            else uu = u ? u[r * Nf + i] : pnr_linspace01(i, Nf);
            int lo = 0, hi = nb;
            while (lo < hi) {
                const int mid = (lo + hi) >> 1;
                if (s_cdf[mid] <= uu) lo = mid + 1; else hi = mid;
            }
            const float zs = pdf_invert(uu, lo, nb, s_cdf, s_bins);
            if (zs_out) zs_out[r * Nf + i] = zs;
            if (inds_out) inds_out[r * Nf + i] = lo;
            s_sort[Nc + i] = zs;
        }
        if (zfine_out) {
            __syncthreads();
            bool asc = true;
            for (int i = lane; i + 1 < Nf; i += 64) asc = asc && (s_sort[Nc + i] <= s_sort[Nc + i + 1]);
            for (int i = lane; i + 1 < Nc; i += 64) asc = asc && (s_z[i] <= s_z[i + 1]);
            if (__all(asc)) {
                for (int i = lane; i < Nc; i += 64) {
                    const float v = s_z[i];
                    int lo = 0, hi = Nf;
                    while (lo < hi) { const int mid = (lo + hi) >> 1; if (s_sort[Nc + mid] < v) lo = mid + 1; else hi = mid; }
                    s_out[i + lo] = v;
                }
                for (int j = lane; j < Nf; j += 64) {
                    const float v = s_sort[Nc + j];
                    int lo = 0, hi = Nc;
                    while (lo < hi) { const int mid = (lo + hi) >> 1; if (s_z[mid] <= v) lo = mid + 1; else hi = mid; }
                    s_out[j + lo] = v;
                }
                __syncthreads();
                for (int i = lane; i < Nt; i += 64) zfine_out[r * Nt + i] = s_out[i];
                labels(r, s_out);
                __syncthreads();
                continue;
            }
            for (int i = lane; i < Nc; i += 64) s_sort[i] = s_z[i];
            for (int i = Nt + lane; i < P; i += 64) s_sort[i] = INFINITY;
            __syncthreads();
            pdf_bitonic(s_sort, P, lane);
            for (int i = lane; i < Nt; i += 64) zfine_out[r * Nt + i] = s_sort[i];
            labels(r, s_sort);
        }
        __syncthreads();
    }
}

__device__ __noinline__ void pdf_bitonic_fallback(float* s_sort, const float* s_z, const float* s_zs, int Nc, int Nf, int P, int lane)
{
    const int Nt = Nc + Nf;
    for (int i = lane; i < Nc; i += 64) s_sort[i] = s_z[i];
    for (int i = lane; i < Nf; i += 64) s_sort[Nc + i] = s_zs[i];
    for (int i = Nt + lane; i < P; i += 64) s_sort[i] = INFINITY;
    __syncthreads();
    pdf_bitonic(s_sort, P, lane);
}

#ifndef PDF_DET_WPE
#define PDF_DET_WPE 8
#endif
#if PDF_DET_WPE
__attribute__((amdgpu_waves_per_eu(PDF_DET_WPE, PDF_DET_WPE)))
#endif
__global__ __launch_bounds__(64) void k_sample_pdf_det(const float* __restrict__ z, const float* __restrict__ weights, int64_t R, int Nc,
                                                        int Nf, float* __restrict__ zfine_out, const PdfLabelArgs lab)
{
    __shared__ float s_z[64], s_w[64], s_pdf[64], s_cdf[64], s_bins[64];
    __shared__ float s_zs[192], s_out[256];
    __shared__ float s_total, s_part[32];
    const int lane = threadIdx.x;
    const int nb = Nc - 1, nw = Nc - 2, Nt = Nc + Nf;
    int topc = 1, topf = 1;
    while (topc * 2 <= Nc) topc *= 2;
    while (topf * 2 <= Nf) topf *= 2;
    const int mh = lab.max_hits;
    for (int64_t r = blockIdx.x; r < R; r += gridDim.x) {
        const float* __restrict__ zr = z + r * Nc;
        const float* __restrict__ wr = weights + r * Nc;
        const float zl = lane < Nc ? zr[lane] : 0.0f, wl = lane < Nc ? wr[lane] : 0.0f;
        int cnt = 0, h_ls = -1, h_li = -1;
        float h_ti = 0.0f, h_to = 0.0f;
        if (lab.label_sem) {
            const int c0 = lab.hit_count[r];
            cnt = c0 < mh ? c0 : mh;
            if (lane < cnt) {
                const float2 t2 = *reinterpret_cast<const float2*>(lab.hit_t + (r * mh + lane) * 2);
                h_ti = t2.x; h_to = t2.y;
                hit_ids(lane, lab.hit_box + r * mh + lane, lab.box_ids, &h_ls, &h_li);
            }
        }
        s_z[lane] = zl;
        s_w[lane] = wl;
        const float zn = __shfl_down(zl, 1, 64), wn = __shfl_down(wl, 1, 64);
        s_bins[lane] = 0.5f * (zn + zl);
        __syncthreads();
        const float total = pdf_torch_total(s_w, nw, s_part, &s_total, lane);
        const float pl = lane < nw ? (wn + 1e-5f) / total : 0.0f;
        s_pdf[lane] = pl;
        pdf_cdf(pl, nw, true, s_pdf, s_cdf, lane);
        bool asc = lane + 1 >= Nc || zl <= zn;
        for (int i = lane; i < Nf; i += 64) {
            const float uu = pnr_linspace01(i, Nf);
            int pos = 0;
            for (int st = topc; st >= 1; st >>= 1) {
                const int p = pos + st, q = p <= nb ? p : nb;
                pos = (p <= nb && s_cdf[q - 1] <= uu) ? p : pos;
            }
            s_zs[i] = pdf_invert(uu, pos, nb, s_cdf, s_bins);
        }
        __syncthreads();
        for (int i = lane; i + 1 < Nf; i += 64) asc = asc && (s_zs[i] <= s_zs[i + 1]);
        if (__all(asc)) {
            if (lane < Nc) {
                int pos = 0;
                for (int st = topf; st >= 1; st >>= 1) {
                    const int p = pos + st, q = p <= Nf ? p : Nf;
                    pos = (p <= Nf && s_zs[q - 1] < zl) ? p : pos;
                }
                s_out[lane + pos] = zl;
            }
            for (int j = lane; j < Nf; j += 64) {
                const float v = s_zs[j];
                int pos = 0;
                for (int st = topc; st >= 1; st >>= 1) {
                    const int p = pos + st, q = p <= Nc ? p : Nc;
                    pos = (p <= Nc && s_z[q - 1] <= v) ? p : pos;
                }
                s_out[j + pos] = v;
            }
            __syncthreads();
        } else {
            pdf_bitonic_fallback(s_out, s_z, s_zs, Nc, Nf, pdf_padded(Nt), lane);
        }
        float* __restrict__ zo = zfine_out + r * Nt;
        for (int i0 = 0; i0 < Nt; i0 += 256) {
            float zz[4];
            int best[4], ls[4], li[4];
            float bt[4];
#pragma unroll
            for (int k = 0; k < 4; ++k) {
                const int i = i0 + lane + 64 * k;
                zz[k] = i < Nt ? s_out[i < Nt ? i : 0] : 0.0f;
                best[k] = -1; ls[k] = -1; li[k] = -1; bt[k] = 0.0f;
                if (i < Nt) zo[i] = zz[k];
            }
            if (lab.label_sem) {
                for (int h = 0; h < cnt; ++h) {
                    const float ti = __int_as_float(__builtin_amdgcn_readlane(__float_as_int(h_ti), h));
                    const float to = __int_as_float(__builtin_amdgcn_readlane(__float_as_int(h_to), h));
                    const int hs = __builtin_amdgcn_readlane(h_ls, h), hi2 = __builtin_amdgcn_readlane(h_li, h);
#pragma unroll
                    for (int k = 0; k < 4; ++k) {
                        const bool take = ti <= zz[k] && zz[k] <= to && (best[k] < 0 || ti < bt[k]);
                        best[k] = take ? h : best[k];
                        bt[k] = take ? ti : bt[k];
                        ls[k] = take ? hs : ls[k];
                        li[k] = take ? hi2 : li[k];
                    }
                }
#pragma unroll
                for (int k = 0; k < 4; ++k) {
                    const int i = i0 + lane + 64 * k;
                    if (i < Nt) {
                        lab.label_sem[r * Nt + i] = ls[k];
                        lab.label_inst[r * Nt + i] = li[k];
                    }
                }
            }
        }
        __syncthreads();
    }
}

template <int MAXC, int MAXT, class... Rng>
__global__ __launch_bounds__(64) __attribute__((amdgpu_waves_per_eu(MAXC <= 64 ? 8 : 1, 8)))
void k_sample_pdf(const float* __restrict__ z, const float* __restrict__ weights, const float* __restrict__ u, int64_t R, int Nc, int Nf,
                  float* __restrict__ zs_out, int32_t* __restrict__ inds_out, float* __restrict__ zfine_out, const PdfLabelArgs lab,
                  const Rng... rng)
{
    sample_pdf_body<MAXC, MAXT>(z, weights, u, R, Nc, Nf, zs_out, inds_out, zfine_out, lab, rng...);
}

__global__ __launch_bounds__(256) void k_bbox_hits(const float* __restrict__ rays, int64_t R,
                                                    const float* __restrict__ box, int M, int max_hits,
                                                    float* __restrict__ hit_t, int32_t* __restrict__ hit_box,
                                                    int32_t* __restrict__ hit_count)
{
    for (int64_t r = (int64_t)blockIdx.x * blockDim.x + threadIdx.x; r < R;
         r += (int64_t)gridDim.x * blockDim.x) {
        const RayRec ry = ray_load(rays, r);
        const auto list = hit_rows(hit_t, hit_box, r, max_hits);
        hit_init(list, max_hits);
        int cnt = 0;
        for (int m = 0; m < M; ++m) {
            float tmin, tmax;
            slab_interval(box + m * 15, ry, &tmin, &tmax);
            if (tmin <= tmax) hit_insert(list, cnt, max_hits, tmin, tmax, m);
        }
        hit_count[r] = cnt;
    }
}

#define SETUP_MAXH 8
struct RaySetupArgs {
    const float* rays; int64_t R; const float* box; int M; int max_hits; const int32_t* box_ids;
    int N, lindisp, hull; const float* t_rand;
    float* hit_t; int32_t* hit_box; int32_t* hit_count; float* z; int32_t* label_sem; int32_t* label_inst;
};
template <class... Rng>
// ... 378 lines not shown
```

panopticnerf_amd/csrc/pnr_sampling_dev.h:

```cpp
#pragma once
#include "pnr_common.h"

#pragma clang fp contract(off)

__device__ __forceinline__ float pnr_linspace01(int i, int N)
{
    if (N <= 1) return 0.0f;
    const float step = 1.0f / (float)(N - 1);
    if (i < N / 2) return step * (float)i;
    return fmaf(-step, (float)(N - 1 - i), 1.0f);
}

__device__ __forceinline__ float strat_z(float nr, float fr, int i, int N, int lindisp)
{
    const float t = pnr_linspace01(i, N);
    const float omt = 1.0f - t;
    if (!lindisp) {
        const float a = nr * omt, b = fr * t;
        return a + b;
    }
    const float a = (1.0f / nr) * omt, b = (1.0f / fr) * t;
    return 1.0f / (a + b);
}

// ... 56 lines not shown
    for (int h = 0; h < n; ++h) l.set(h, make_float2(0.0f, 0.0f), -1);
}

template <class L>
__device__ __forceinline__ void hit_insert(const L& l, int& cnt, int max_hits, float tmin, float tmax, int m)
{
    const int n = cnt < max_hits ? cnt : max_hits;
    int pos = n;
    while (pos > 0 && l.t_in(pos - 1) > tmin) --pos;
    if (pos < max_hits) {
        for (int k = (n < max_hits ? n : max_hits - 1); k > pos; --k) l.set(k, l.iv(k - 1), l.box(k - 1));
        l.set(pos, make_float2(tmin, tmax), m);
    }
    ++cnt;
}

template <class L>
__device__ __forceinline__ void hit_hull(const L& l, int kept, float* near_out, float* far_out)
{
    float2 v = l.iv(0);
    float lo = v.x, hi = v.y;
    for (int h = 1; h < kept; ++h) {
        v = l.iv(h);
        lo = fminf(lo, v.x);
        hi = fmaxf(hi, v.y);
    }
    *near_out = lo;
    *far_out = hi;
}

template <class F>
__device__ __forceinline__ int label_hit(float zz, int cnt, F interval)
{
    int best = -1;
    float bt = 0.0f;
    for (int h = 0; h < cnt; ++h) {
        float ti, to;
        interval(h, ti, to);
        if (ti <= zz && zz <= to && (best < 0 || ti < bt)) {
            best = h;
            bt = ti;
        }
    }
    return best;
}

__device__ __forceinline__ void hit_ids(int best, const int32_t* box_of_best, const int32_t* __restrict__ box_ids, int* ls, int* li)
{
    *ls = -1;
    *li = -1;
    if (best >= 0) {
        const int m = *box_of_best;
        *ls = box_ids[m * 2];
        *li = box_ids[m * 2 + 1];
    }
}

__host__ __device__ __forceinline__ int pdf_padded(int Nt)
{
    int P = 1;
    while (P < Nt) P <<= 1;
    return P;
}

__device__ __forceinline__ float pdf_torch_total(const float* s_w, int nw, float* s_part, float* s_total, int lane)
{
    const bool short4 = nw >= 4 && nw < 8;
    if (lane < 32) {
        const int k = lane >> 3, l = lane & 7, nv = nw / 8, groups = nv / 4;
        float pacc = 0.0f;
        for (int g = 0; g < groups; ++g) pacc = pacc + (s_w[(g * 4 + k) * 8 + l + 1] + 1e-5f);
        if (k == 0)
            for (int v = groups * 4; v < nv; ++v) pacc = pacc + (s_w[v * 8 + l + 1] + 1e-5f);
        if (short4 && lane < 3) pacc = pacc + (s_w[lane + 2] + 1e-5f);
        s_part[lane] = pacc;
    }
    __syncthreads();
    if (lane == 0) {
        const int nv = nw / 8;
        float total = 0.0f;
        for (int j = nv * 8; j < nw; j = (short4 && j == 0) ? 4 : j + 1) total = total + (s_w[j + 1] + 1e-5f);
        for (int l = 0; l < 8; ++l) {
            float p0 = s_part[l];
            p0 = p0 + s_part[8 + l]; p0 = p0 + s_part[16 + l]; p0 = p0 + s_part[24 + l];
            total = total + p0;
        }
        *s_total = total;
    }
    __syncthreads();
    return *s_total;
}

__device__ __forceinline__ void pdf_cdf(float pl, int nw, bool one_per_lane, const float* s_pdf, float* s_cdf, int lane)
{
    double c = (double)pl;
    bool exact = one_per_lane && __all(pl == 0.0f || pl >= 0x1p-28f);
    if (exact) {
#pragma unroll
        for (int d = 1; d < 64; d <<= 1) {
            const double o = __shfl_up(c, d, 64);
            if (lane >= d) c += o;
        }
        exact = __shfl(c, 63, 64) < 1.999;
    }
    if (exact) {
        if (lane == 0) s_cdf[0] = 0.0f;
        if (lane < nw) s_cdf[lane + 1] = (float)c;
    } else {
        __syncthreads();
        if (lane == 0) {
            double cc = 0.0;
            s_cdf[0] = 0.0f;
            for (int j = 0; j < nw; ++j) {
                cc += (double)s_pdf[j];
                s_cdf[j + 1] = (float)cc;
            }
        }
    }
    __syncthreads();
}

__device__ __forceinline__ float pdf_invert(float uu, int inds, int nb, const float* s_cdf, const float* s_bins)
{
    const int below = inds - 1 > 0 ? inds - 1 : 0;
    const int above = inds < nb - 1 ? inds : nb - 1;
    const float cb = s_cdf[below];
    float denom = s_cdf[above] - cb;
    if (denom < 1e-5f) denom = 1.0f;
    const float t = (uu - cb) / denom;
    const float bb = s_bins[below];
    const float span = s_bins[above] - bb;
    const float m = t * span;
    return bb + m;
}

__device__ __forceinline__ void pdf_bitonic(float* s_sort, int P, int lane)
{
    for (int k = 2; k <= P; k <<= 1) {
        for (int j = k >> 1; j > 0; j >>= 1) {
            for (int t = lane; t < (P >> 1); t += 64) {
                const int i = ((t & ~(j - 1)) << 1) | (t & (j - 1));
                const int p = i | j;
                const float a = s_sort[i], b = s_sort[p];
                const bool asc = (i & k) == 0;
                if ((a > b) == asc) {
                    s_sort[i] = b;
                    s_sort[p] = a;
                }
            }
            __syncthreads();
        }
    }
}
```

panopticnerf_amd/ops.py:

```python
import ctypes
import functools
import math
import os

import torch

from . import _lib
from . import camera as _camera
from ._lib import MlpDesc, MlpParamsHost


def _stream():
    return ctypes.c_void_p(torch.cuda.current_stream().cuda_stream)


def _chk(t, name, dtype=torch.float32):
    if t is None:
        return None
    if not t.is_cuda:
        raise RuntimeError(f"{name}: expected a GPU tensor (the HIP path has no CPU fallback)")
    if t.dtype != dtype:
        raise TypeError(f"{name}: expected {dtype}, got {t.dtype}")
    if not t.is_contiguous():
        raise ValueError(f"{name}: tensor must be contiguous")
# ... 1555 lines not shown
        if k in table and tuple(shp) != table[k]:
            raise ValueError("mlp_wgrad: shapes[%r] is %s, the descriptor's network has %s" % (k, tuple(shp), table[k]))
    nbytes = _size_or_raise(lib.pnr_mlp_wgrad_workspace_bytes(ctypes.byref(desc), int(n_samples)), "pnr_mlp_wgrad_workspace_bytes")
    ws = torch.empty(int(nbytes), device=dev, dtype=torch.uint8)
    grads = {k: torch.empty(tuple(shp), device=dev, dtype=torch.float32) for k, shp in shapes.items()}
    G, keep = _param_struct(desc, grads, dev, "mlp_wgrad")
    _lib.check(lib.pnr_mlp_wgrad(ctypes.byref(desc), _p(acts), _p(dys), int(n_samples), ctypes.byref(G), _p(ws), _stream()),
               "pnr_mlp_wgrad")
    return grads


@_on_device
def mlp_forward_train_fp32(desc, params, rays, z):
    R, N = _level("mlp_forward_train_fp32", rays, z)
    S = R * N
    lib = _lib.load()
    n = _size_or_raise(lib.pnr_mlp_fp32_acts_floats(ctypes.byref(desc), S), "pnr_mlp_fp32_acts_floats")
    raw = torch.empty((n_channels(desc), S), device=z.device, dtype=torch.float32)
    acts = torch.empty((int(n),), device=z.device, dtype=torch.float32)
    P, keep = _param_struct(desc, params, z.device, "mlp_forward_train_fp32")
    _lib.check(lib.pnr_mlp_forward_train_fp32(ctypes.byref(desc), ctypes.byref(P), _p(rays), _p(z), R, N, _p(raw), 1, S, _p(acts),
                                              _stream()), "pnr_mlp_forward_train_fp32")
    return raw, acts


@_on_device
def mlp_backward_fp32(desc, params, d_raw, acts, n_rays, n_samples):
    d_raw, acts = _chk(d_raw, "d_raw"), _chk(acts, "acts")
    S = int(n_rays) * int(n_samples)
    if tuple(d_raw.shape) != (n_channels(desc), S):
        raise ValueError(f"d_raw: expected {(n_channels(desc), S)}, got {tuple(d_raw.shape)}")
    lib = _lib.load()
    dev = acts.device
    n = _size_or_raise(lib.pnr_mlp_fp32_acts_floats(ctypes.byref(desc), S), "pnr_mlp_fp32_acts_floats")
    _at_least("mlp_backward_fp32", "acts", acts, n, "pnr_mlp_fp32_acts_floats")
    _on("mlp_backward_fp32", dev, "acts", d_raw=d_raw)
    nbytes = _size_or_raise(lib.pnr_mlp_backward_fp32_workspace_bytes(ctypes.byref(desc), S), "pnr_mlp_backward_fp32_workspace_bytes")
    ws = torch.empty(int(nbytes), device=dev, dtype=torch.uint8)
    grads = {k: torch.empty_like(v, dtype=torch.float32, memory_format=torch.contiguous_format) for k, v in params.items()}
    P, keep = _param_struct(desc, params, dev, "mlp_backward_fp32")
    G, keep2 = _param_struct(desc, grads, dev, "mlp_backward_fp32")
    _lib.check(lib.pnr_mlp_backward_fp32(ctypes.byref(desc), ctypes.byref(P), _p(d_raw), d_raw.stride(0), _p(acts), int(n_rays),
                                         int(n_samples), ctypes.byref(G), _p(ws), _stream()), "pnr_mlp_backward_fp32")
    return grads


def n_channels(desc):
    return 4 + desc.n_sem + desc.n_inst


RAW_PAD = 64


def alloc_raw(ch, S, device, pad=RAW_PAD):
    buf = torch.empty(ch * (S + pad), device=device, dtype=torch.float32)
    return buf.as_strided((ch, S), (S + pad, 1))


def _chk_raw(raw, ch, S):
    if not raw.is_cuda or raw.dtype != torch.float32:
        raise TypeError("raw: expected a float32 GPU tensor")
    if tuple(raw.shape) != (ch, S) or raw.stride(1) != 1 or raw.stride(0) < S:
        raise ValueError(f"raw: expected shape {(ch, S)} with unit sample stride, got {tuple(raw.shape)} strides {raw.stride()}")
    return raw.stride(0)


@_on_device
def mlp_forward(desc, packed, rays, z, channel_major=True, out=None):
    R, N = _level("mlp_forward", rays, z, desc, packed)
    ch = n_channels(desc)
    S = R * N
    if channel_major:
        raw = out if out is not None else alloc_raw(ch, S, z.device)
        ss, sc = 1, _chk_raw(raw, ch, S)
    else:
        raw = out if out is not None else torch.empty((R, N, ch), device=z.device, dtype=torch.float32)
        ss, sc = ch, 1
        _count("mlp_forward", "out", _chk(raw, "raw"), S * ch, "(R, N, ch)")
    _on("mlp_forward", z.device, "z", out=raw)
    _lib.check(_lib.load().pnr_mlp_forward(ctypes.byref(desc), _p(packed), _p(rays), _p(z), R, N, _p(raw), ss, sc,
                                           _stream()), "pnr_mlp_forward")
    return raw


@_on_device
def composite(raw, z, rays, n_sem=0, n_inst=0, channel_major=True, noise=None, label_sem=None, label_inst=None,
              sem_mode=0, white_bkgd=False, want_weights=True, out=None):
    noise, draw = _draw_or(noise, "noise")
    R, N = _level("composite", rays, z)
    ch = 4 + n_sem + n_inst
    if channel_major:
        ss, sc = 1, _chk_raw(raw, ch, R * N)
    else:
        _count("composite", "raw", _chk(raw, "raw"), R * N * ch, "(R, N, ch)")
        ss, sc = ch, 1
    dev = z.device
    _count("composite", "noise", noise, R * N, "one per sample")
    label_sem, label_inst = _labels("composite", label_sem, label_inst, R * N, dev)
    _on("composite", dev, "z", raw=raw, noise=noise, call=draw.call if draw else None)
    out = _maps(out, R, N, n_sem, n_inst, label_sem, label_inst, want_weights, dev)
    g = out.get
    fn, nz, what = _twin("pnr_composite", noise, draw)
    _lib.check(fn(_p(raw), ss, sc, _p(z), _p(rays), nz, _p(label_sem), _p(label_inst), R, N, n_sem, n_inst, int(sem_mode),
                  int(bool(white_bkgd)), _p(out["rgb"]), _p(out["depth"]), _p(out["acc"]), _p(g("weights")), _p(g("semantic")),
                  _p(g("instance")), _p(g("fix_semantic")), _p(g("fix_instance")), _stream()), what)
    return out


def _maps(out, R, N, n_sem, n_inst, label_sem, label_inst, want_weights, dev, drop=()):
    f32 = dict(device=dev, dtype=torch.float32)
    shapes = {"rgb": (R, 3), "depth": (R,), "acc": (R,)}
    if want_weights:
        shapes["weights"] = (R, N)
    if n_sem:
        shapes["semantic"] = (R, n_sem)
        if label_sem is not None:
            shapes["fix_semantic"] = (R, n_sem)
    if n_inst:
        shapes["instance"] = (R, n_inst)
        if label_inst is not None:
            shapes["fix_instance"] = (R, n_inst)
    for k in drop:
        shapes.pop(k, None)
    res = {}
    for k, shp in shapes.items():
        t = out.get(k) if out else None
        if t is None:
            t = torch.empty(shp, **f32)
        elif tuple(t.shape) != shp or t.dtype != torch.float32 or t.device != dev or not t.is_contiguous():
            raise ValueError("out[%r] must be a contiguous fp32 tensor of shape %s on %s" % (k, shp, dev))
        res[k] = t
    return res


def fused_supported(desc, n_samples, sem_mode=0, noise=None):
    ok = (desc.precision == _lib.PREC_BF16 and int(sem_mode) in (0, 1) and noise is None and n_samples % 32 == 0
          and 32 <= n_samples <= 256 and desc.n_sem + desc.n_inst <= 128)
    if ok and int(sem_mode) == 1 and desc.n_sem + desc.n_inst > 0:
        ok = int(_lib.load().pnr_mlp_fused_plan(ctypes.byref(desc_for_mode(desc, 1)))) >= 1
    return ok


def desc_for_mode(desc, sem_mode):
    want = _lib.MLP_SOFTMAX if int(sem_mode) == 1 else 0
    if (desc.flags & _lib.MLP_SOFTMAX) == want:
        return desc
    return _desc_with(desc, flags=(desc.flags & ~_lib.MLP_SOFTMAX) | want)


def fused_image(sem_mode=0):
    return "softmax" if int(sem_mode) == 1 else True


@_on_device
def mlp_forward_composite(desc, packed, rays, z, label_sem=None, label_inst=None, white_bkgd=False, want_weights=True, out=None,
                          sem_mode=0, wg_cap=0):
    image = desc
    desc = desc_for_mode(desc, sem_mode)
    if wg_cap:
        desc = _desc_with(desc, flags=(desc.flags & 0xFFFF) | ((int(wg_cap) & 0x1FF) << 16))
    return _fused_level("mlp_forward_composite", desc, image, packed, rays, z, label_sem, label_inst, white_bkgd, want_weights, out)


def _fused_level(what, desc, image, packed, rays, z, label_sem, label_inst, white_bkgd, want_weights, out, drop=()):
    R, N = _level(what, rays, z, image, packed)
    dev = z.device
    label_sem, label_inst = _labels(what, label_sem, label_inst, R * N, dev)
    lib = _lib.load()
    nbytes = lib.pnr_mlp_forward_composite_workspace_bytes(ctypes.byref(desc), R, N, int(bool(want_weights)))
    if nbytes < 0:
        raise RuntimeError("pnr_mlp_forward_composite: unsupported geometry (n_samples=%d must be a multiple of 32)" % N)
    ws = torch.empty(int(nbytes), device=dev, dtype=torch.uint8)
    out = _maps(out, R, N, desc.n_sem, desc.n_inst, label_sem, label_inst, want_weights, dev, drop=drop)
    g = out.get
    _lib.check(lib.pnr_mlp_forward_composite(ctypes.byref(desc), _p(packed), _p(rays), _p(z), R, N, _p(label_sem), _p(label_inst),
                                             int(bool(white_bkgd)), _p(g("rgb")), _p(out["depth"]), _p(out["acc"]),
                                             _p(g("weights")), _p(g("semantic")), _p(g("instance")), _p(g("fix_semantic")),
                                             _p(g("fix_instance")), _p(ws), _stream()), "pnr_mlp_forward_composite")
    return out


WEIGHTS_ONLY_DROPS = ("rgb", "semantic", "instance")


def sigma_pass_supported(desc, n_samples, noise=None):
    if not (desc.precision == _lib.PREC_BF16 and noise is None and n_samples % 32 == 0 and 32 <= n_samples <= 256
            and desc.n_sem + desc.n_inst <= 128):
        return False
    return int(_lib.load().pnr_mlp_packed_bytes(ctypes.byref(_desc_with(desc, plan=3)))) > 0


@_on_device
def mlp_forward_weights(desc, packed, rays, z, label_sem=None, label_inst=None, out=None):
    if desc.plan != 3:
        raise ValueError("mlp_forward_weights: needs the plan-3 image (net.packed(level, device, fused='sigma')), not plan %d" % desc.plan)
    return _fused_level("mlp_forward_weights", desc, desc, packed, rays, z, label_sem, label_inst, False, True, out, WEIGHTS_ONLY_DROPS)


QUERY_WANTS = ("sigma", "labels", "panoptic", "logits")


def field_query_supported(desc):
    return bool(_lib.load().pnr_mlp_query_supported(ctypes.byref(desc)))


def query_keys(desc, want):
    want = (want,) if isinstance(want, str) else tuple(want)
    bad = [w for w in want if w not in QUERY_WANTS]
    if bad:
        raise ValueError("query: unknown output %r in want (known: %s)" % (bad[0], ", ".join(QUERY_WANTS)))
    keys = []
    if "sigma" in want:
        keys.append("sigma")
    if "labels" in want:
        keys += (["sem_label"] if desc.n_sem else []) + (["inst_label"] if desc.n_inst else [])
    if "panoptic" in want and desc.n_sem:
        keys.append("panoptic")
    if "logits" in want:
        keys += (["sem_logits"] if desc.n_sem else []) + (["inst_logits"] if desc.n_inst else [])
    if not keys:
        raise ValueError("query: want=%r asks for nothing this network has (n_sem=%d, n_inst=%d)" % (want, desc.n_sem, desc.n_inst))
    return keys


@_on_device
def mlp_query(desc, packed, points, want=("sigma", "labels"), is_thing=None, out=None):
    if desc.plan != 4:
        raise ValueError("mlp_query: needs the plan-4 image (net.packed(level, device, fused='field')), not plan %d" % desc.plan)
    keys = query_keys(desc, want)
    points = _chk(points, "points")
    is_thing = _chk(is_thing, "is_thing", torch.int32)
    if points.dim() != 2 or points.shape[1] != 3:
        raise ValueError("mlp_query: points must be (P, 3), got %s" % (tuple(points.shape),))
    if is_thing is not None and (not desc.n_sem or is_thing.numel() != desc.n_sem):
        raise ValueError("mlp_query: is_thing must hold n_sem=%d entries of a network with a semantic head" % desc.n_sem)
    P, dev = points.shape[0], points.device
    _packed("mlp_query", desc, packed)
    _on("mlp_query", dev, "points", packed=packed, is_thing=is_thing)
    out = dict(out) if out else {}
    res, stride = {}, P
    for k in keys:
        if k.endswith("_logits"):
            n = desc.n_sem if k == "sem_logits" else desc.n_inst
            t = out.get(k)
            if t is None:
                t = alloc_raw(n, P, dev)
            elif (not t.is_cuda or t.dtype != torch.float32 or tuple(t.shape) != (n, P) or (P > 0 and t.stride(1) != 1)
                  or (n > 1 and t.stride(0) < P)):
                raise ValueError("mlp_query: out[%r] must be a float32 GPU tensor of shape %s with unit point stride" % (k, (n, P)))
            res[k] = t
        else:
            res[k] = _own(out.get(k), (P,), torch.float32 if k == "sigma" else torch.int32, dev, "mlp_query: out[%r]" % k)
    lg = [res[k] for k in ("sem_logits", "inst_logits") if k in res]
    _on("mlp_query", dev, "points", **{"out[%r]" % k: res[k] for k in ("sem_logits", "inst_logits") if k in res})
    if lg:
        stride = lg[0].stride(0) if lg[0].shape[0] > 1 else max(P, lg[0].stride(0))
        if any((t.stride(0) if t.shape[0] > 1 else stride) != stride for t in lg):
            raise ValueError("mlp_query: sem_logits and inst_logits must share one channel stride")
    g = res.get
    _lib.check(_lib.load().pnr_mlp_query(ctypes.byref(desc), _p(packed), _p(points), P, _p(g("sigma")), _p(g("sem_label")),
                                         _p(g("inst_label")), _p(g("panoptic")), _p(is_thing), _p(g("sem_logits")),
                                         _p(g("inst_logits")), stride, _stream()), "pnr_mlp_query")
    return res


@_on_device
def composite_backward(raw, z, rays, n_sem, n_inst, grads, noise=None, label_sem=None, label_inst=None,
                       ce_sem=None, ce_inst=None, sem_mode=0):
    raw = _chk(raw, "raw")
    noise, draw = _draw_or(noise, "noise")
    R, N = _level("composite_backward", rays, z)
    dev, ch = z.device, 4 + n_sem + n_inst
    _count("composite_backward", "raw", raw, ch * R * N, "(ch, R * N)")
    _count("composite_backward", "noise", noise, R * N, "one per sample")
    label_sem, label_inst = _labels("composite_backward", label_sem, label_inst, R * N, dev)
    g = {k: _chk(v.contiguous().float(), "g_" + k) for k, v in grads.items() if v is not None}
    per_ray = {"rgb": 3, "depth": 1, "acc": 1, "weights": N, "semantic": n_sem, "fix_semantic": n_sem, "instance": n_inst, "fix_instance": n_inst}
    for k, n in per_ray.items():
        if n:
            _count("composite_backward", "g_" + k, g.get(k), R * n, "a gradient of R rows")
    ce_sem = None if ce_sem is None else _chk(ce_sem.reshape(1).float().contiguous(), "ce_sem")
    ce_inst = None if ce_inst is None else _chk(ce_inst.reshape(1).float().contiguous(), "ce_inst")
    _on("composite_backward", dev, "z", raw=raw, noise=noise, call=draw.call if draw else None, ce_sem=ce_sem, ce_inst=ce_inst,
        **{"g_" + k: v for k, v in g.items() if k in per_ray})
    d_raw = torch.empty_like(raw)
    fn, nz, what = _twin("pnr_composite_backward3", noise, draw, rng_name="pnr_composite_backward_rng", what="pnr_composite_backward")
    _lib.check(fn(_p(raw), R * N, _p(z), _p(rays), nz, R, N, n_sem, n_inst, int(sem_mode), _p(g.get("rgb")), _p(g.get("depth")),
                  _p(g.get("acc")), _p(g.get("semantic")), _p(g.get("instance")), _p(g.get("weights")), _p(label_sem), _p(label_inst),
                  _p(g.get("fix_semantic")), _p(g.get("fix_instance")), _p(ce_sem), _p(ce_inst), _p(d_raw), _stream()), what)
    return d_raw


_LOSS_KEYS = ("rgb", "depth", "semantic", "fix_semantic", "instance", "fix_instance")


@_on_device
def losses(weights, maps, targets, n_sem=0, n_inst=0, depth_l2=False, fix_eps=1e-5, want_grads=True, maps_are_prob=False):
    m = {k: _chk(v.detach().contiguous(), k) for k, v in maps.items() if k in _LOSS_KEYS and v is not None and v.numel()}
    if not m:
        raise ValueError("ops.losses: no usable map: `maps` holds none of %s with at least one ray (R = 0?)" % ", ".join(_LOSS_KEYS))
    lib = _lib.load()
    any_map = next(iter(m.values()))
    dev, R = any_map.device, any_map.shape[0]
    t_rgb, t_depth = _chk(targets.get("rgb"), "rgb_gt"), _chk(targets.get("depth"), "depth_gt")
    t_sem = _chk(targets.get("semantic"), "sem_gt", torch.int32)
    t_inst = _chk(targets.get("instance"), "inst_gt", torch.int32)
    cfg = _lib.LossCfg(*(float(weights.get(k, 0.0)) for k in _LOSS_KEYS), int(bool(depth_l2)), float(fix_eps), int(bool(maps_are_prob)))
    use = {"rgb": t_rgb is not None, "depth": t_depth is not None, "semantic": t_sem is not None, "fix_semantic": t_sem is not None,
           "instance": t_inst is not None, "fix_instance": t_inst is not None}
    m = {k: v for k, v in m.items() if use[k]}
    per_ray = {"rgb": 3, "depth": 1, "semantic": int(n_sem), "fix_semantic": int(n_sem), "instance": int(n_inst), "fix_instance": int(n_inst)}
    named = {k: (v, per_ray[k]) for k, v in m.items()}
    named.update(rgb_gt=(t_rgb, 3), depth_gt=(t_depth, 1), sem_gt=(t_sem, 1), inst_gt=(t_inst, 1))
    for name, (t, n) in named.items():
        _count("losses", name, t, R * n, "R rows")
    _on("losses", dev, "the first map", **{name: t for name, (t, n) in named.items()})
    grads = {k: torch.empty_like(v) for k, v in m.items()} if want_grads else {}
    out = torch.empty(8, device=dev, dtype=torch.float32)
    ws = torch.empty(int(lib.pnr_losses_workspace_bytes(R)), device=dev, dtype=torch.uint8)
    g = grads.get
    _lib.check(lib.pnr_losses(ctypes.byref(cfg), R, int(n_sem), int(n_inst), _p(m.get("rgb")), _p(m.get("depth")),
                              _p(m.get("semantic")), _p(m.get("fix_semantic")), _p(m.get("instance")), _p(m.get("fix_instance")),
                              _p(t_rgb), _p(t_depth), _p(t_sem), _p(t_inst), _p(out), _p(g("rgb")), _p(g("depth")),
                              _p(g("semantic")), _p(g("fix_semantic")), _p(g("instance")), _p(g("fix_instance")), _p(ws),
                              _stream()), "pnr_losses")
    return out, grads


@_on_device
def ce3d(raw, first_channel, n_classes, label):
    lib = _lib.load()
    label = _chk(label, "label", torch.int32)
    S = label.numel()
    sc = _chk_raw(raw, raw.shape[0], S)
    if not 0 <= int(first_channel) <= int(first_channel) + int(n_classes) <= raw.shape[0]:
        raise ValueError("ce3d: channels %d .. %d are not all among raw's %d" % (first_channel, first_channel + n_classes - 1, raw.shape[0]))
    _on("ce3d", raw.device, "raw", label=label)
    out = torch.empty(2, device=raw.device, dtype=torch.float32)
    ws = torch.empty(int(lib.pnr_ce3d_workspace_bytes(S)), device=raw.device, dtype=torch.uint8)
    _lib.check(lib.pnr_ce3d(_p(raw), sc, int(first_channel), int(n_classes), _p(label), S, _p(out), _p(ws), _stream()), "pnr_ce3d")
    return out


@_on_device
def sample_pdf(z, weights, n_importance, u=None, want_samples=True, out=None):
    u, draw = _draw_or(u, "u")
    R, Nc, dev = _coarse("sample_pdf", z, weights, u, draw, n_importance)
    z_fine = _own(out, (R, Nc + n_importance), torch.float32, dev, "sample_pdf")
    zs = inds = None
    if want_samples:
        zs = torch.empty((R, n_importance), device=dev, dtype=torch.float32)
        inds = torch.empty((R, n_importance), device=dev, dtype=torch.int32)
    fn, uu, what = _twin("pnr_sample_pdf", u, draw)
    _lib.check(fn(_p(z), _p(weights), uu, R, Nc, n_importance, _p(zs), _p(inds), _p(z_fine), _stream()), what)
    return z_fine, zs, inds


@_on_device
def bbox_hits(rays, box, max_hits=8):
    R, M = _rays("bbox_hits", rays), _boxes("bbox_hits", box, rays.device)
    dev = rays.device
    hit_t, hit_box, hit_count = _new_hit_lists("bbox_hits", R, max_hits, dev)
    _lib.check(_lib.load().pnr_bbox_hits(_p(rays), R, _p(box), M, max_hits, _p(hit_t), _p(hit_box), _p(hit_count),
                                         _stream()), "pnr_bbox_hits")
    return hit_t, hit_box, hit_count


@_on_device
def convex_hits(rays, planes, offsets, max_hits=8, out=None):
    rays, planes, offsets = _chk(rays, "rays"), _chk(planes, "planes"), _chk(offsets, "offsets", torch.int32)
    if rays.dim() != 2 or rays.shape[1] != 8:
        raise ValueError("convex_hits: rays must be (R, 8), not %s" % (tuple(rays.shape),))
    if planes.dim() != 2 or planes.shape[1] != 4:
        raise ValueError("convex_hits: planes must be (P, 4), not %s" % (tuple(planes.shape),))
    if offsets.dim() != 1 or offsets.numel() < 1:
        raise ValueError("convex_hits: offsets must be (M + 1,), not %s" % (tuple(offsets.shape),))
    R, M = rays.shape[0], offsets.numel() - 1
    max_hits = int(max_hits)
    if max_hits < 1:
        raise ValueError("convex_hits: max_hits must be >= 1, not %d" % max_hits)
    dev = rays.device
    if planes.shape[0] == 0 and M > 0:
        planes = planes.new_zeros((1, 4))
    hit_t, hit_box, hit_count = _new_hit_lists("convex_hits", R, max_hits, dev, out)
    _lib.check(_lib.load().pnr_convex_hits(_p(rays), R, _p(planes), _p(offsets), M, max_hits, _p(hit_t), _p(hit_box), _p(hit_count),
                                           _stream()), "pnr_convex_hits")
    return hit_t, hit_box, hit_count


RAY_SETUP_MAX_HITS = 8


@_on_device
def ray_setup(rays, box, box_ids=None, n_samples=64, max_hits=8, lindisp=False, t_rand=None, hull=False, out=None):
    t_rand, draw = _draw_or(t_rand, "t_rand")
    R, M = _rays("ray_setup", rays), _boxes("ray_setup", box, rays.device, box_ids)
    dev, N = rays.device, int(n_samples)
    _count("ray_setup", "t_rand", t_rand, R * N, "one per sample")
    _on("ray_setup", dev, "rays", t_rand=t_rand, call=draw.call if draw else None)
    hit_t, hit_box, hit_count = _new_hit_lists("ray_setup", R, max_hits, dev)
    z = _own(out, (R, N), torch.float32, dev, "ray_setup")
    ls = li = None
    if box_ids is not None:
        ls = torch.empty((R, N), device=dev, dtype=torch.int32)
        li = torch.empty((R, N), device=dev, dtype=torch.int32)
    fn, rand, what = _twin("pnr_ray_setup", t_rand, draw)
    _lib.check(fn(_p(rays), R, _p(box), M, int(max_hits), _p(box_ids), N, int(bool(lindisp)), rand, int(bool(hull)), _p(hit_t),
                  _p(hit_box), _p(hit_count), _p(z), _p(ls), _p(li), _stream()), what)
    return (hit_t, hit_box, hit_count), z, ls, li


@_on_device
def sample_pdf_labels(z, weights, n_importance, hits, box_ids, u=None, out=None):
    u, draw = _draw_or(u, "u")
    R, Nc, dev = _coarse("sample_pdf_labels", z, weights, u, draw, n_importance)
    hit_t, hit_box, hit_count = hits
    mh = _hit_lists("sample_pdf_labels", R, hit_t, hit_box, hit_count, dev, "z")
    box_ids = _chk(box_ids, "box_ids", torch.int32)
    _on("sample_pdf_labels", dev, "z", box_ids=box_ids)
    Nt = Nc + int(n_importance)
    z_fine = _own(out, (R, Nt), torch.float32, dev, "sample_pdf_labels")
    ls = torch.empty((R, Nt), device=dev, dtype=torch.int32)
    li = torch.empty((R, Nt), device=dev, dtype=torch.int32)
    fn, uu, what = _twin("pnr_sample_pdf_labels", u, draw)
    _lib.check(fn(_p(z), _p(weights), uu, R, Nc, int(n_importance), _p(z_fine), _p(hit_t), _p(hit_box), _p(hit_count), mh,
                  _p(box_ids), _p(ls), _p(li), _stream()), what)
    return z_fine, ls, li


@_on_device
def restrict_rays(rays, hit_t, hit_count):
    R = _rays("restrict_rays", rays)
    mh = _hit_lists("restrict_rays", R, hit_t, None, hit_count, rays.device, "rays")
    out = torch.empty_like(rays)
    _lib.check(_lib.load().pnr_restrict_rays(_p(rays), R, _p(hit_t), _p(hit_count), mh, _p(out), _stream()), "pnr_restrict_rays")
    return out


@_on_device
def sample_labels(z, hit_t, hit_box, hit_count, box_ids):
    z = _chk(z, "z")
    if z.dim() != 2:
        raise ValueError("sample_labels: z must be (R, N), got %s" % (tuple(z.shape),))
    R, N = z.shape
    mh = _hit_lists("sample_labels", R, hit_t, hit_box, hit_count, z.device, "z")
    box_ids = _chk(box_ids, "box_ids", torch.int32)
    _on("sample_labels", z.device, "z", box_ids=box_ids)
    ls = torch.empty((R, N), device=z.device, dtype=torch.int32)
    li = torch.empty((R, N), device=z.device, dtype=torch.int32)
    _lib.check(_lib.load().pnr_sample_labels(_p(z), R, N, _p(hit_t), _p(hit_box), _p(hit_count), mh,
                                             _p(box_ids), _p(ls), _p(li), _stream()), "pnr_sample_labels")
    return ls, li


@_on_device
def panoptic_labels(sem, inst=None, is_thing=None):
    sem, inst = _chk(sem, "sem"), _chk(inst, "inst")
    is_thing = _chk(is_thing, "is_thing", torch.int32)
    if sem.dim() != 2 or (inst is not None and (inst.dim() != 2 or inst.shape[0] != sem.shape[0])):
        raise ValueError("panoptic_labels: sem must be (R, n_sem) and inst (R, n_inst), got %s and %s"
                         % (tuple(sem.shape), None if inst is None else tuple(inst.shape)))
    R, C = sem.shape
    K = inst.shape[1] if inst is not None else 0
    _count("panoptic_labels", "is_thing", is_thing, C, "one per class of sem")
    _on("panoptic_labels", sem.device, "sem", inst=inst, is_thing=is_thing)
    out = [torch.empty(R, device=sem.device, dtype=torch.int32) for _ in range(3)]
    _lib.check(_lib.load().pnr_panoptic_labels(_p(sem), _p(inst), _p(is_thing), R, C, K, _p(out[0]), _p(out[1]), _p(out[2]),
                                               _stream()), "pnr_panoptic_labels")
    return tuple(out)


@_on_device
def confusion(pred, gt, n_classes, conf=None):
    pred, gt = _chk(pred, "pred", torch.int32), _chk(gt, "gt", torch.int32)
    if conf is None:
        conf = torch.zeros((n_classes, n_classes), device=pred.device, dtype=torch.int64)
    _chk(conf, "conf", torch.int64)
    _count("confusion", "gt", gt, pred.numel(), "one per element of pred")
    _count("confusion", "conf", conf, int(n_classes) ** 2, "(n_classes, n_classes)")
    _on("confusion", pred.device, "pred", gt=gt, conf=conf)
    _lib.check(_lib.load().pnr_confusion(_p(pred), _p(gt), pred.numel(), int(n_classes), _p(conf), _stream()), "pnr_confusion")
    return conf
```

panopticnerf_amd/renderer.py:

```python
import collections
import os

import torch

from . import ops


Prims = collections.namedtuple("Prims", "planes offsets")


def _get(cfg, name, default):
    return getattr(cfg, name, default) if cfg is not None else default


CHUNK_QUANTUM = 1024
CHUNK_TAIL = 8


def chunk_plan(n_rays, chunk_size):
    n_rays, chunk_size = int(n_rays), max(1, int(chunk_size))
    if n_rays <= 0:
        return []
    n = -(-n_rays // chunk_size)
    if n > 1 and n_rays - (n - 1) * chunk_size <= chunk_size // CHUNK_TAIL:
        n -= 1
    size = -(-n_rays // n)
    if n > 1 and chunk_size >= CHUNK_QUANTUM * CHUNK_TAIL:
        size = -(-size // CHUNK_QUANTUM) * CHUNK_QUANTUM
    out, s = [], 0
    while s < n_rays:
        e = min(n_rays, s + size)
        out.append((s, e))
        s = e
    return out


def _keyed(res, z, lv):
    return {**{f"{k}_{lv}": v for k, v in res.items()}, f"z_vals_{lv}": z}


def _level_out(out, lv):
    return {k[:-2]: v for k, v in out.items() if k.endswith(f"_{lv}") and k != f"z_vals_{lv}"}


def _fill_rows(rows, o):
    for k, v in o.items():
        if v.data_ptr() != rows[k].data_ptr():
            rows[k].copy_(v)


def _unflatten(maps, lead):
    return {k: v if v.dim() == 0 else v.reshape(*lead, *v.shape[1:]) for k, v in maps.items()}


def merge_chunks(outs):
    if len(outs) == 1:
        return outs[0]
    ret = {}
    for k in outs[0]:
        vs = [o[k] for o in outs]
        head, lv = k.rsplit("_", 1)
        if vs[0].dim() > 0:
            ret[k] = torch.cat(vs, 0)
        elif head.endswith("_n"):
            ret[k] = torch.stack(vs).sum()
        else:
            n = torch.stack([o[f"{head}_n_{lv}"] for o in outs])
            ret[k] = (torch.stack(vs) * n).sum() / n.sum().clamp(min=1.0)
    return ret


class Renderer:
    def __init__(self, net, cfg=None):
        self.net = net
        self.cfg = cfg
        self.N_samples = _get(cfg, "N_samples", 64)
        self.N_importance = _get(cfg, "N_importance", _get(cfg, "cascade_samples", 0))
        self.chunk_size = _get(cfg, "chunk_size", 65536)
        self.perturb = _get(cfg, "perturb", 0.0)
        self.raw_noise_std = _get(cfg, "raw_noise_std", 0.0)
        self.white_bkgd = _get(cfg, "white_bkgd", False)
        self.lindisp = _get(cfg, "lindisp", False)
        self.max_hits = _get(cfg, "max_hits", 8)
        self.sem_mode = {"none": 0, "logits": 0, "softmax": 1}[_get(cfg, "semantic_activation", "none")]
        self.keep_weights = _get(cfg, "keep_weights", True)
        self.fuse = bool(_get(cfg, "fuse_composite", os.environ.get("PNR_FUSE", "1") != "0"))
        self.strict_hits = bool(_get(cfg, "strict_hits", False))
        self.coarse_outputs = _get(cfg, "coarse_outputs", "all")
        if self.coarse_outputs not in ("all", "weights"):
            raise ValueError("cfg.coarse_outputs must be 'all' or 'weights', not %r" % (self.coarse_outputs,))
        if self.coarse_outputs == "weights" and self.N_importance <= 0:
            raise ValueError("cfg.coarse_outputs = 'weights' needs a fine level (N_importance > 0): without one the coarse maps are "
                             "the render's output")
        self.bbox_sampling = _get(cfg, "bbox_sampling", "none")
        if self.bbox_sampling not in ("none", "hull"):
            raise ValueError("cfg.bbox_sampling must be 'none' or 'hull', not %r" % (self.bbox_sampling,))
        self._overflow = None
        self.rng = _get(cfg, "rng", "torch")
        if self.rng not in ("torch", "device"):
            raise ValueError("cfg.rng must be 'torch' or 'device', not %r" % (self.rng,))
        self.rng_state = None
        if self.rng == "device":
            seed = _get(cfg, "rng_seed", None)
            seed = torch.initial_seed() if seed is None else int(seed)
            seed = (seed + 2 ** 63) % 2 ** 64 - 2 ** 63
            p0 = next(iter(net.parameters()), None)
            self.rng_state = torch.tensor([seed, 0], dtype=torch.int64, device=p0.device if p0 is not None else "cpu")
        self.frame_outputs = bool(_get(cfg, "frame_outputs", os.environ.get("PNR_FRAME_OUT", "1") != "0"))
        self.overlap_levels = bool(_get(cfg, "overlap_levels", os.environ.get("PNR_OVERLAP", "1") != "0"))
        self._side_streams = {}
        if self.N_importance > 0 and getattr(net, "nerf_1", None) is None and not getattr(net, "share_coarse_fine", False):
            raise ValueError("make_renderer: cfg asks for a fine pass (N_importance / cascade_samples = %d) but the network "
                             "was built without a fine NeRF -- build it with make_network(cfg) from the SAME cfg, or set "
                             "cfg.share_coarse_fine = True to evaluate one NeRF at both levels on purpose" % self.N_importance)

    def _preamble(self, rays, box, box_ids, t_rand, z_out):
        hits = lab0 = None
        hull = self.bbox_sampling == "hull"
        prims = isinstance(box, Prims)
        if box is not None and not prims and self.max_hits <= ops.RAY_SETUP_MAX_HITS:
            hits, z, ls0, li0 = ops.ray_setup(rays, box, box_ids, self.N_samples, self.max_hits, self.lindisp, t_rand, hull, out=z_out)
            lab0 = (ls0, li0)
        else:
            if prims:
                hits = ops.convex_hits(rays, box.planes, box.offsets, self.max_hits)
            elif box is not None:
                hits = ops.bbox_hits(rays, box, self.max_hits)
            rays_s = ops.restrict_rays(rays, hits[0], hits[2]) if (hits is not None and hull) else rays
            z = ops.stratified(rays_s, self.N_samples, self.lindisp, t_rand, out=z_out)
        return hits, z, lab0

    def _labels(self, z, hits, box_ids, lab=None):
        if lab is not None:
            return lab
        return ops.sample_labels(z, hits[0], hits[1], hits[2], box_ids) if hits is not None else (None, None)

    def _noise(self, lv, z, train, rng):
        if not (self.raw_noise_std > 0 and train):
            return None
        if rng is not None:
            return ops.Draw(rng[0], 3 + lv, rng[1], self.raw_noise_std)
        return torch.randn(z.shape, device=z.device) * self.raw_noise_std

    def _need_weights(self, lv):
        return self.keep_weights or (lv == 0 and self.N_importance > 0)

    def _level(self, lv, rays, z, labels, noise, out, grad, wg_cap=0):
        net, dev = self.net, rays.device
        ls, li = labels
        n0 = net.nerf(0)
        if grad:
            from . import train as _train
            return _train.level_train(self, lv, rays, z, ls, li, noise)
        weights_only = lv == 0 and self.coarse_outputs == "weights"
        need_w = self._need_weights(lv)
        d = net.nerf(lv).desc(net.precision)
        if weights_only and self.fuse and ops.sigma_pass_supported(d, z.shape[1], noise):
            desc, img = net.packed(0, dev, fused="sigma")
            return ops.mlp_forward_weights(desc, img, rays, z, ls, li, out=out)
        if not weights_only and self.fuse and ops.fused_supported(d, z.shape[1], self.sem_mode, noise):
            desc, img = net.packed(lv, dev, fused=ops.fused_image(self.sem_mode))
            return ops.mlp_forward_composite(desc, img, rays, z, ls, li, self.white_bkgd, need_w, out=out, sem_mode=self.sem_mode,
                                             wg_cap=wg_cap)
        desc, img = net.packed(lv, dev)
        raw = ops.mlp_forward(desc, img, rays, z, channel_major=True)
        res = ops.composite(raw, z, rays, n0.n_sem, n0.n_inst, True, noise, ls, li, self.sem_mode, self.white_bkgd, need_w, out=out)
        return {k: v for k, v in res.items() if k not in ops.WEIGHTS_ONLY_DROPS} if weights_only else res

    def _resample(self, z, weights, hits, box_ids, u, z_out):
        w0 = weights.detach().contiguous()
        if hits is not None:
            z_fine, ls1, li1 = ops.sample_pdf_labels(z, w0, self.N_importance, hits, box_ids, u, out=z_out)
            return z_fine, (ls1, li1)
        z_fine, _, _ = ops.sample_pdf(z, w0, self.N_importance, u, want_samples=False, out=z_out)
        return z_fine, None

    def render_rays(self, rays, box=None, box_ids=None, t_rand=None, u=None, train=False, grad=False, out=None, rng=None):
        Nc, Nf = self.N_samples, self.N_importance
        dev = rays.device
        out = out if (out and not grad) else {}
        draw = self.perturb > 0 and train
        if t_rand is None and draw:
            t_rand = ops.Draw(rng[0], 1, rng[1]) if rng is not None else torch.rand((rays.shape[0], Nc), device=dev)
        hits, z, lab0 = self._preamble(rays, box, box_ids, t_rand, out.get("z_vals_0"))
        if hits is not None and self.strict_hits:
            over = torch.stack([(hits[2] > self.max_hits).sum(), hits[2].max()])
            self._overflow = over if self._overflow is None else torch.stack([self._overflow[0] + over[0],
                                                                              torch.maximum(self._overflow[1], over[1])])
        lab0 = self._labels(z, hits, box_ids, lab0)
        o0 = self._level(0, rays, z, lab0, self._noise(0, z, train, rng), _level_out(out, 0), grad)
        ret = _keyed(o0, z, 0)
        if Nf > 0:
            if u is None and draw:
                u = ops.Draw(rng[0], 2, rng[1]) if rng is not None else torch.rand((rays.shape[0], Nf), device=dev)
            z_fine, lab1 = self._resample(z, o0["weights"], hits, box_ids, u, out.get("z_vals_1"))
            lab1 = self._labels(z_fine, hits, box_ids, lab1)
            o1 = self._level(1, rays, z_fine, lab1, self._noise(1, z_fine, train, rng), _level_out(out, 1), grad)
            ret.update(_keyed(o1, z_fine, 1))
        return ret

    def _output_maps(self, R, has_box, dev, grad=False):
        n0 = self.net.nerf(0)
        lab = True if has_box else None
        Nc, Nf = self.N_samples, self.N_importance
        ret = {}
        for lv, N in ((0, Nc), (1, Nc + Nf)) if Nf > 0 else ((0, Nc),):
            drop = ops.WEIGHTS_ONLY_DROPS if (lv == 0 and not grad and self.coarse_outputs == "weights") else ()
            m = ops._maps(None, R, N, n0.n_sem, n0.n_inst, lab, lab, grad or self._need_weights(lv), dev, drop=drop)
            ret.update(_keyed(m, torch.empty((R, N), device=dev, dtype=torch.float32), lv))
        return ret

    def _empty_outputs(self, lead, has_box, dev, grad=False):
        return _unflatten(self._output_maps(0, has_box, dev, grad), lead)

    def _overlap_caps(self, dev, plan, grad, train, has_box, t_rand, u):
        if (not self.overlap_levels or grad or train or len(plan) < 2 or not self.fuse or not self.frame_outputs or self.N_importance <= 0
                or self.strict_hits or t_rand is not None or u is not None or self.raw_noise_std > 0 and train
                or self.coarse_outputs == "weights" or torch.cuda.is_current_stream_capturing()):
            return None
        net, Nc, Nt = self.net, self.N_samples, self.N_samples + self.N_importance
        for lv, N in ((0, Nc), (1, Nt)):
            d = net.nerf(lv).desc(net.precision)
            if not ops.fused_supported(d, N, self.sem_mode, None) or net.packed(lv, dev, fused=ops.fused_image(self.sem_mode))[0].plan != 2:
                return None
        cus = torch.cuda.get_device_properties(dev).multi_processor_count
        cap_c = int(round(cus * Nc / float(Nc + Nt) / 8.0)) * 8
        cap_f = cus - cap_c
        if cus % 8 or cap_c < 8 or cap_f < 8 or abs((Nc / float(cap_c)) / (Nt / float(cap_f)) - 1.0) > 0.05:
            return None
        return cap_c, cap_f

    def _render_overlapped(self, rays, box, box_ids, plan, caps, lead):
        dev = rays.device
        cap_c, cap_f = caps
        last = len(plan) - 1
        frame = self._output_maps(rays.shape[0], box is not None, dev)
        main = torch.cuda.current_stream(dev)
        if dev not in self._side_streams:
            self._side_streams[dev] = (torch.cuda.Stream(dev), torch.cuda.Stream(dev))
        side = self._side_streams[dev]
        start = torch.cuda.Event()
        start.record(main)
        for st in side:
            st.wait_event(start)
        prev_pdf = None
        pre = {}

        def preamble(cj):
            sj, ej = plan[cj]
            return self._preamble(rays[sj:ej], box, box_ids, None, frame["z_vals_0"][sj:ej])
        try:
            for ci, (s, e) in enumerate(plan):
                r, st = rays[s:e], side[ci & 1]
                out = {k: v[s:e] for k, v in frame.items()}
                with torch.cuda.stream(st):
                    hits, z, lab0 = pre.pop(ci) if ci in pre else preamble(ci)
                    lab0 = self._labels(z, hits, box_ids, lab0)
                    if prev_pdf is not None:
                        st.wait_event(prev_pdf)
                    o0 = self._level(0, r, z, lab0, None, _level_out(out, 0), False, 0 if ci == 0 else cap_c)
                    z_fine, lab1 = self._resample(z, o0["weights"], hits, box_ids, None, out["z_vals_1"])
                    prev_pdf = torch.cuda.Event()
                    prev_pdf.record(st)
                    if ci + 2 <= last:
                        pre[ci + 2] = preamble(ci + 2)
                    lab1 = self._labels(z_fine, hits, box_ids, lab1)
                    o1 = self._level(1, r, z_fine, lab1, None, _level_out(out, 1), False, 0 if ci == last else cap_f)
                    _fill_rows(out, {**_keyed(o0, z, 0), **_keyed(o1, z_fine, 1)})
        finally:
            for st in side:
                done = torch.cuda.Event()
                done.record(st)
                main.wait_event(done)
        return _unflatten(frame, lead)

    def render(self, batch):
        rays = batch["rays"]
        if not rays.is_cuda:
            raise RuntimeError("Renderer.render: batch['rays'] must be on the GPU (no CPU fallback)")
        grad = torch.is_grad_enabled() and any(p.requires_grad for p in self.net.parameters())
        if grad and self.net.precision not in ("bf16", "fp32"):
            raise ValueError("Renderer.render: precision must be 'bf16' (the training path) or 'fp32' (its parity mode)")
        lead = rays.shape[:-1]
        rays = rays.reshape(-1, 8).float().contiguous()
        R = rays.shape[0]
        box = batch.get("bbox")
        box_ids = batch.get("bbox_ids")
        if batch.get("prim_planes") is not None:
            if box is not None:
                raise ValueError("Renderer.render: the batch has both 'bbox' and 'prim_planes' -- one prior per render: turn the "
                                 "cuboids into primitives with ConvexSet.from_boxes and join the sets with ConvexSet.concat")
            if batch.get("prim_offsets") is None or batch.get("prim_ids") is None:
                raise ValueError("Renderer.render: 'prim_planes' comes with 'prim_offsets' and 'prim_ids' (ConvexSet.batch())")
            box = Prims(batch["prim_planes"].reshape(-1, 4).float().contiguous(), batch["prim_offsets"].reshape(-1).int().contiguous())
            box_ids = batch["prim_ids"].reshape(-1, 2).int().contiguous()
            if box_ids.shape[0] != box.offsets.numel() - 1:
                raise ValueError("Renderer.render: prim_ids has %d rows for %d primitives" % (box_ids.shape[0], box.offsets.numel() - 1))
        elif box is not None:
            box = box.reshape(-1, 15).float().contiguous()
            box_ids = box_ids.reshape(-1, 2).int().contiguous()
        self._overflow = None
        if R == 0:
            return self._empty_outputs(lead, box is not None, rays.device, grad)
        t_rand, u = batch.get("t_rand"), batch.get("u")
        if t_rand is not None:
            t_rand = t_rand.reshape(R, -1).float().contiguous()
        if u is not None:
            u = u.reshape(R, -1).float().contiguous()
        train = self.net.training
        plan = chunk_plan(R, self.chunk_size)
        caps = self._overlap_caps(rays.device, plan, grad, train, box is not None, t_rand, u)
        if caps is not None:
            return self._render_overlapped(rays, box, box_ids, plan, caps, lead)
        call = None
        if self.rng == "device" and train and (self.perturb > 0 or self.raw_noise_std > 0):
            if self.rng_state.device != rays.device:
                self.rng_state = self.rng_state.to(rays.device)
            call = ops.rng_begin(self.rng_state)
        frame = self._output_maps(R, box is not None, rays.device) if (len(plan) > 1 and not grad and self.frame_outputs) else None
        outs = []
        for s, e in plan:
            rows = None if frame is None else {k: v[s:e] for k, v in frame.items()}
            o = self.render_rays(rays[s:e], box, box_ids,
                                 None if t_rand is None else t_rand[s:e],
                                 None if u is None else u[s:e], train, grad, out=rows,
                                 rng=None if call is None else (call, s))
            if frame is not None:
                _fill_rows(rows, o)
            else:
                outs.append(o)
        if self._overflow is not None:
            n_over, worst = (int(v) for v in self._overflow.tolist())
            self._overflow = None
            if n_over > 0:
                raise RuntimeError("Renderer.render: %d ray(s) cross more than max_hits = %d boxes (up to %d): the farthest "
                                   "intervals were dropped -- raise cfg.max_hits" % (n_over, self.max_hits, worst))
        return _unflatten(frame if frame is not None else merge_chunks(outs), lead)

    def render_view(self, camera, c2w, near, far, bbox=None, bbox_ids=None, prims=None):
        if torch.is_grad_enabled() and any(p.requires_grad for p in self.net.parameters()):
            raise RuntimeError("Renderer.render_view is inference only: call it under torch.no_grad() (training batches are made "
                               "with camera.rays(pix=...) and rendered with render())")
        p0 = next(iter(self.net.parameters()), None)
        if p0 is None or not p0.is_cuda:
            raise RuntimeError("Renderer.render_view: the network must be on the GPU (no CPU fallback)")
        dev, H, W = p0.device, camera.height, camera.width
        pix = camera.valid_pix(dev)
        whole = pix.numel() == H * W
        batch = {"rays": camera.rays(c2w, near, far, pix=None if whole else pix, device=dev)}
        if bbox is not None:
            batch.update(bbox=bbox, bbox_ids=bbox_ids)
        if prims is not None:
            if prims.device != dev:
                prims.to(dev)
            batch.update(prims.batch())
        out = self.render(batch)
        valid = torch.ones((H, W), dtype=torch.bool, device=dev)
        if whole:
            ret = {k: v.reshape(H, W, *v.shape[1:]) for k, v in out.items()}
        else:
            idx = pix.long()
            valid = torch.zeros(H * W, dtype=torch.bool, device=dev).index_fill_(0, idx, True).reshape(H, W)
            ret = {}
            for k, v in out.items():
                img = torch.zeros((H * W,) + tuple(v.shape[1:]), dtype=v.dtype, device=dev)
                ret[k] = img.index_copy_(0, idx, v).reshape(H, W, *v.shape[1:])
        ret["valid"] = valid
        return ret


def make_renderer(cfg, network):
    return Renderer(network, cfg)
```

Baseline: 1190.

## Fuse coarse compositing combine with PDF resampling and fine labelling in one kernel

Adds a kernel that runs the coarse-level composite combine and, in the same block, builds the PDF from the coarse weights, draws deterministic fine samples, merges and sorts them with the coarse z values, and assigns box labels to the fine samples. The renderer and ops layer route coarse levels through it when the fused path applies (inference only: no noise, no random u, no gradients). The intent is to remove the separate sample_pdf/sample_pdf_labels launches and the global round-trip of the coarse weights. The cost is one 64-thread block per ray with several block-wide syncs, which may underuse the GPU compared with the separate kernels.

New measurement: 1178. 0.99x the previous value.

```diff
diff --git a/include/pnr.h b/include/pnr.h
--- a/include/pnr.h
+++ b/include/pnr.h
@@ -78,6 +78,11 @@
 int pnr_composite_combine(const pnr_mlp_desc* desc, const void* workspace, const float* z, int64_t n_rays, int n_samples,
                           const int32_t* label_sem, const int32_t* label_inst, int white_bkgd, float* rgb, float* depth,
                           float* acc, float* weights, float* sem, float* inst, float* fix_sem, float* fix_inst, void* stream);
+int pnr_coarse_finish(const pnr_mlp_desc* desc, const void* workspace, const float* z, int64_t n_rays, int n_coarse, int n_fine,
+                      const int32_t* label_sem, const int32_t* label_inst, int white_bkgd, float* rgb, float* depth, float* acc,
+                      float* weights, float* sem, float* inst, float* fix_sem, float* fix_inst, float* z_fine,
+                      const float* hit_t, const int32_t* hit_box, const int32_t* hit_count, int max_hits,
+                      const int32_t* box_ids, int32_t* label_sem_fine, int32_t* label_inst_fine, void* stream);
 
 int pnr_mlp_query(const pnr_mlp_desc* desc, const void* packed, const float* points, int64_t n_points,
                   float* sigma, int32_t* sem_label, int32_t* inst_label, int32_t* panoptic, const int32_t* is_thing,
diff --git a/panopticnerf_amd/_lib.py b/panopticnerf_amd/_lib.py
--- a/panopticnerf_amd/_lib.py
+++ b/panopticnerf_amd/_lib.py
@@ -188,6 +188,8 @@
     "pnr_mlp_query_supported": (c_int, [ctypes.POINTER(MlpDesc)]),
     "pnr_composite_combine": (c_int, [ctypes.POINTER(MlpDesc), c_f, c_f, c_i64, c_int, c_f, c_f, c_int,
                                       c_f, c_f, c_f, c_f, c_f, c_f, c_f, c_f, c_f]),
+    "pnr_coarse_finish": (c_int, [ctypes.POINTER(MlpDesc), c_f, c_f, c_i64, c_int, c_int, c_f, c_f, c_int,
+                                  c_f, c_f, c_f, c_f, c_f, c_f, c_f, c_f, c_f, c_f, c_f, c_f, c_int, c_f, c_f, c_f, c_f]),
 }
 
 _lib = None
diff --git a/panopticnerf_amd/csrc/pnr_coarse_finish.hip b/panopticnerf_amd/csrc/pnr_coarse_finish.hip
--- /dev/null
+++ b/panopticnerf_amd/csrc/pnr_coarse_finish.hip
@@ -0,0 +1,204 @@
+#include "pnr_common.h"
+#include "pnr_composite_dev.h"
+#include "pnr_sampling_dev.h"
+
+#ifndef COARSE_FINISH_WPE
+#define COARSE_FINISH_WPE 8
+#endif
+struct CoarseFinishArgs { CombineArgs a; PdfLabelArgs lab; float* z_fine; int Nf; };
+typedef const __attribute__((address_space(4))) CoarseFinishArgs* CoarseFinishKernarg;
+
+template <bool LOGITS>
+#if COARSE_FINISH_WPE
+__attribute__((amdgpu_waves_per_eu(COARSE_FINISH_WPE, COARSE_FINISH_WPE)))
+#endif
+__global__ __launch_bounds__(64) void k_coarse_finish(const CoarseFinishArgs P)
+{
+    __shared__ uint32_t hist[128];
+    __shared__ float s_z[64], s_w[64], s_pdf[64], s_cdf[64], s_bins[64];
+    __shared__ float s_zs[192], s_out[256];
+    __shared__ float s_total, s_part[32];
+    const int lane = threadIdx.x;
+    const int Nc = P.a.N, Nf = P.Nf, T = Nc >> 5, RF = P.a.rec_floats, C = P.a.C, K = P.a.K, CK = C + K;
+    const int nb = Nc - 1, nw = Nc - 2, Nt = Nc + Nf;
+    int topc = 1, topf = 1;
+    while (topc * 2 <= Nc) topc *= 2;
+    while (topf * 2 <= Nf) topf *= 2;
+    const int mh = P.lab.max_hits;
+    CoarseFinishKernarg ka = (CoarseFinishKernarg)__builtin_amdgcn_kernarg_segment_ptr();
+    for (int64_t r = blockIdx.x; r < P.a.R; r += gridDim.x) {
+        int ln = lane;
+        asm volatile("" : "+v"(ln), "+s"(ka));
+        const __attribute__((address_space(4))) CombineArgs& a = ka->a;
+        const bool want_s = a.lab_s && a.fix_sem && C, want_i = a.lab_i && a.fix_inst && K;
+        const float* __restrict__ rec = a.rec + r * T * RF;
+        const bool in = ln < Nc;
+        const float q0 = rec[0];
+        const float4 pv = in ? a.ps[r * Nc + ln] : float4{0.0f, 0.0f, 0.0f, 0.0f};
+        const float zl = in ? a.z[r * Nc + ln] : 0.0f;
+        const int lsv = (in && want_s) ? a.lab_s[r * Nc + ln] : -1;
+        const int liv = (in && want_i) ? a.lab_i[r * Nc + ln] : -1;
+        float lg[2][2];
+#pragma unroll
+        for (int h = 0; h < 2; ++h)
+#pragma unroll
+            for (int k = 0; k < 2; ++k) lg[h][k] = (LOGITS && k < T && ln + 64 * h < CK) ? rec[k * RF + PNR_FUSE_REC_LOGITS + ln + 64 * h] : 0.0f;
+        const float Tk[2] = {1.0f, 1.0f * q0};
+        if (want_s || want_i) hist_zero<64>(hist, ln, CK);
+        float r5[5] = {0.0f, 0.0f, 0.0f, 0.0f, 0.0f};
+        float wl = 0.0f;
+        if (in) {
+            const float tk = (ln >> 5) == 1 ? Tk[1] : Tk[0];
+            const float w = tk * pv.x;
+            r5[0] += w;
+            r5[1] = fmaf(w, zl, r5[1]);
+            r5[2] = fmaf(w, sigmoid_of(pv.y), r5[2]);
+            r5[3] = fmaf(w, sigmoid_of(pv.z), r5[3]);
+            r5[4] = fmaf(w, sigmoid_of(pv.w), r5[4]);
+            if (a.weights) a.weights[r * Nc + ln] = w;
+            if (want_s || want_i) hist_add(hist, w, want_s, lsv, C, want_i, liv, K);
+            wl = w;
+        }
+        group_sum_batch<64, 5>(r5);
+        if (ln == 0) {
+            if (a.acc) a.acc[r] = r5[0];
+            if (a.depth) a.depth[r] = r5[1];
+        }
+        if (ln < 3 && a.rgb) {
+            const float v = ln == 0 ? r5[2] : ln == 1 ? r5[3] : r5[4];
+            a.rgb[r * 3 + ln] = a.white_bkgd ? v + (1.0f - r5[0]) : v;
+        }
+#pragma unroll
+        for (int h = 0; h < 2; ++h) {
+            const int c = ln + 64 * h;
+            if (c >= CK) continue;
+            if constexpr (LOGITS) {
+                float v = 0.0f;
+#pragma unroll
+                for (int k = 0; k < 2; ++k) if (k < T) v = fmaf(Tk[k], lg[h][k], v);
+                if (c < C) { if (a.sem) a.sem[r * C + c] = v; }
+                else if (a.inst) a.inst[r * K + (c - C)] = v;
+            }
+            if (c < C) { if (want_s) a.fix_sem[r * C + c] = hist_read(hist, c); }
+            else if (want_i) a.fix_inst[r * K + (c - C)] = hist_read(hist, c);
+        }
+        asm volatile("" : "+s"(ka));
+        float* __restrict__ const zfine_out = ka->z_fine;
+        PdfLabelArgs lab;
+        lab.hit_t = ka->lab.hit_t; lab.hit_box = ka->lab.hit_box; lab.hit_count = ka->lab.hit_count; lab.max_hits = mh;
+        lab.box_ids = ka->lab.box_ids; lab.label_sem = ka->lab.label_sem; lab.label_inst = ka->lab.label_inst;
+        int cnt = 0, h_ls = -1, h_li = -1;
+        float h_ti = 0.0f, h_to = 0.0f;
+        if (lab.label_sem) {
+            const int c0 = lab.hit_count[r];
+            cnt = c0 < mh ? c0 : mh;
+            if (lane < cnt) {
+                const float2 t2 = *reinterpret_cast<const float2*>(lab.hit_t + (r * mh + lane) * 2);
+                h_ti = t2.x; h_to = t2.y;
+                hit_ids(lane, lab.hit_box + r * mh + lane, lab.box_ids, &h_ls, &h_li);
+            }
+        }
+        s_z[lane] = zl;
+        s_w[lane] = wl;
+        const float zn = __shfl_down(zl, 1, 64), wn = __shfl_down(wl, 1, 64);
+        s_bins[lane] = 0.5f * (zn + zl);
+        __syncthreads();
+        const float total = pdf_torch_total(s_w, nw, s_part, &s_total, lane);
+        const float pl = lane < nw ? (wn + 1e-5f) / total : 0.0f;
+        s_pdf[lane] = pl;
+        pdf_cdf(pl, nw, true, s_pdf, s_cdf, lane);
+        bool asc = lane + 1 >= Nc || zl <= zn;
+        for (int i = lane; i < Nf; i += 64) {
+            const float uu = pnr_linspace01(i, Nf);
+            int pos = 0;
+            for (int st = topc; st >= 1; st >>= 1) {
+                const int p = pos + st, q = p <= nb ? p : nb;
+                pos = (p <= nb && s_cdf[q - 1] <= uu) ? p : pos;
+            }
+            s_zs[i] = pdf_invert(uu, pos, nb, s_cdf, s_bins);
+        }
+        __syncthreads();
+        for (int i = lane; i + 1 < Nf; i += 64) asc = asc && (s_zs[i] <= s_zs[i + 1]);
+        if (__all(asc)) {
+            if (lane < Nc) {
+                int pos = 0;
+                for (int st = topf; st >= 1; st >>= 1) {
+                    const int p = pos + st, q = p <= Nf ? p : Nf;
+                    pos = (p <= Nf && s_zs[q - 1] < zl) ? p : pos;
+                }
+                s_out[lane + pos] = zl;
+            }
+            for (int j = lane; j < Nf; j += 64) {
+                const float v = s_zs[j];
+                int pos = 0;
+                for (int st = topc; st >= 1; st >>= 1) {
+                    const int p = pos + st, q = p <= Nc ? p : Nc;
+                    pos = (p <= Nc && s_z[q - 1] <= v) ? p : pos;
+                }
+                s_out[j + pos] = v;
+            }
+            __syncthreads();
+        } else {
+            pdf_bitonic_fallback(s_out, s_z, s_zs, Nc, Nf, pdf_padded(Nt), lane);
+        }
+        float* __restrict__ zo = zfine_out + r * Nt;
+        for (int i0 = 0; i0 < Nt; i0 += 256) {
+            float zz[4];
+            int best[4], ls[4], li[4];
+            float bt[4];
+#pragma unroll
+            for (int k = 0; k < 4; ++k) {
+                const int i = i0 + lane + 64 * k;
+                zz[k] = i < Nt ? s_out[i < Nt ? i : 0] : 0.0f;
+                best[k] = -1; ls[k] = -1; li[k] = -1; bt[k] = 0.0f;
+                if (i < Nt) zo[i] = zz[k];
+            }
+            if (lab.label_sem) {
+                for (int h = 0; h < cnt; ++h) {
+                    const float ti = __int_as_float(__builtin_amdgcn_readlane(__float_as_int(h_ti), h));
+                    const float to = __int_as_float(__builtin_amdgcn_readlane(__float_as_int(h_to), h));
+                    const int hs = __builtin_amdgcn_readlane(h_ls, h), hi2 = __builtin_amdgcn_readlane(h_li, h);
+#pragma unroll
+                    for (int k = 0; k < 4; ++k) {
+                        const bool take = ti <= zz[k] && zz[k] <= to && (best[k] < 0 || ti < bt[k]);
+                        best[k] = take ? h : best[k];
+                        bt[k] = take ? ti : bt[k];
+                        ls[k] = take ? hs : ls[k];
+                        li[k] = take ? hi2 : li[k];
+                    }
+                }
+#pragma unroll
+                for (int k = 0; k < 4; ++k) {
+                    const int i = i0 + lane + 64 * k;
+                    if (i < Nt) {
+                        lab.label_sem[r * Nt + i] = ls[k];
+                        lab.label_inst[r * Nt + i] = li[k];
+                    }
+                }
+            }
+        }
+        __syncthreads();
+    }
+}
+
+int pnr_coarse_finish_launch(const float* rec, int rec_floats, bool logit_sums, const float4* ps, const float* z, const int32_t* label_sem,
+                             const int32_t* label_inst, int64_t R, int N, int n_fine, int C, int K, int white_bkgd, float* rgb, float* depth,
+                             float* acc, float* weights, float* sem, float* inst, float* fix_sem, float* fix_inst, float* z_fine,
+                             const float* hit_t, const int32_t* hit_box, const int32_t* hit_count, int max_hits, const int32_t* box_ids,
+                             int32_t* label_sem_fine, int32_t* label_inst_fine, hipStream_t st)
+{
+    CombineArgs a;
+    a.rec = rec; a.rec_floats = rec_floats; a.ps = ps; a.z = z; a.lab_s = label_sem; a.lab_i = label_inst;
+    a.R = R; a.N = N; a.C = C; a.K = K; a.white_bkgd = white_bkgd;
+    a.rgb = rgb; a.depth = depth; a.acc = acc; a.weights = weights; a.sem = sem; a.inst = inst; a.fix_sem = fix_sem; a.fix_inst = fix_inst;
+    CoarseFinishArgs P;
+    P.a = a;
+    P.lab = PdfLabelArgs{hit_t, hit_box, hit_count, max_hits, box_ids, label_sem_fine, label_inst_fine};
+    P.z_fine = z_fine;
+    P.Nf = n_fine;
+    const dim3 grid(pnr_grid_cap(R, 32)), block(64);
+    if (logit_sums) hipLaunchKernelGGL(k_coarse_finish<true>, grid, block, 0, st, P);
+    else hipLaunchKernelGGL(k_coarse_finish<false>, grid, block, 0, st, P);
+    PNR_CHECK_LAUNCH("pnr_coarse_finish");
+    return PNR_OK;
+}
diff --git a/panopticnerf_amd/csrc/pnr_composite.hip b/panopticnerf_amd/csrc/pnr_composite.hip
--- a/panopticnerf_amd/csrc/pnr_composite.hip
+++ b/panopticnerf_amd/csrc/pnr_composite.hip
@@ -321,11 +321,6 @@
                           sem_mode, white_bkgd, rgb, depth, acc, weights, sem, inst, fix_sem, fix_inst, stream);
 }
 
-struct CombineArgs {
-    const float* rec; int rec_floats; const float4* ps; const float* z; const int32_t* lab_s; const int32_t* lab_i;
-    int64_t R; int N, C, K, white_bkgd;
-    float *rgb, *depth, *acc, *weights, *sem, *inst, *fix_sem, *fix_inst;
-};
 
 template <bool LOGITS>
 __global__ __launch_bounds__(256) void k_composite_combine(CombineArgs a)
diff --git a/panopticnerf_amd/csrc/pnr_composite_dev.h b/panopticnerf_amd/csrc/pnr_composite_dev.h
--- a/panopticnerf_amd/csrc/pnr_composite_dev.h
+++ b/panopticnerf_amd/csrc/pnr_composite_dev.h
@@ -201,6 +201,12 @@
     }
 }
 
+struct CombineArgs {
+    const float* rec; int rec_floats; const float4* ps; const float* z; const int32_t* lab_s; const int32_t* lab_i;
+    int64_t R; int N, C, K, white_bkgd;
+    float *rgb, *depth, *acc, *weights, *sem, *inst, *fix_sem, *fix_inst;
+};
+
 template <int... SUBS, class F>
 static void composite_dispatch(int sub, bool ch_major, bool softmax, const PnrRngDev* rng, F&& launch)
 {
diff --git a/panopticnerf_amd/csrc/pnr_mlp.hip b/panopticnerf_amd/csrc/pnr_mlp.hip
--- a/panopticnerf_amd/csrc/pnr_mlp.hip
+++ b/panopticnerf_amd/csrc/pnr_mlp.hip
@@ -804,6 +804,11 @@
                                  const int32_t* label_sem, const int32_t* label_inst, int64_t R, int N, int C, int K, int white_bkgd,
                                  float* rgb, float* depth, float* acc, float* weights, float* sem, float* inst, float* fix_sem,
                                  float* fix_inst, hipStream_t st);
+int pnr_coarse_finish_launch(const float* rec, int rec_floats, bool logit_sums, const float4* ps, const float* z, const int32_t* label_sem,
+                             const int32_t* label_inst, int64_t R, int N, int n_fine, int C, int K, int white_bkgd, float* rgb, float* depth,
+                             float* acc, float* weights, float* sem, float* inst, float* fix_sem, float* fix_inst, float* z_fine,
+                             const float* hit_t, const int32_t* hit_box, const int32_t* hit_count, int max_hits, const int32_t* box_ids,
+                             int32_t* label_sem_fine, int32_t* label_inst_fine, hipStream_t st);
 
 static int record_floats(const pnr_mlp_desc& d)
 {
@@ -925,6 +930,38 @@
                                         rgb, depth, acc, weights, sem, inst, fix_sem, fix_inst, (hipStream_t)stream);
 }
 
+PNR_EXPORT int pnr_coarse_finish(const pnr_mlp_desc* desc, const void* workspace, const float* z, int64_t n_rays, int n_coarse, int n_fine,
+                                 const int32_t* label_sem, const int32_t* label_inst, int white_bkgd, float* rgb, float* depth, float* acc,
+                                 float* weights, float* sem, float* inst, float* fix_sem, float* fix_inst, float* z_fine,
+                                 const float* hit_t, const int32_t* hit_box, const int32_t* hit_count, int max_hits,
+                                 const int32_t* box_ids, int32_t* label_sem_fine, int32_t* label_inst_fine, void* stream)
+{
+    int rc = pnr_mlp_validate(desc);
+    if (rc != PNR_OK) return rc;
+    PNR_REQUIRE(n_rays >= 0, "pnr_coarse_finish: bad size");
+    PNR_REQUIRE(n_coarse == 32 || n_coarse == 64, "pnr_coarse_finish: n_coarse=%d must be 32 or 64", n_coarse);
+    PNR_REQUIRE(n_fine >= 1 && n_fine <= 192, "pnr_coarse_finish: n_fine=%d outside [1,192]", n_fine);
+    PNR_REQUIRE(desc->n_sem + desc->n_inst <= 128, "pnr_coarse_finish: n_sem + n_inst <= 128");
+    PNR_REQUIRE(desc->plan != 4, "pnr_coarse_finish: a plan-4 (field) image has no compositing workspace");
+    const bool labels = hit_t || hit_box || hit_count || box_ids || label_sem_fine || label_inst_fine;
+    PNR_REQUIRE(!labels || (max_hits >= 1 && max_hits <= 64), "pnr_coarse_finish: max_hits=%d outside [1,64]", max_hits);
+    if (n_rays == 0) return PNR_OK;
+    PNR_REQUIRE(workspace && z && z_fine, "pnr_coarse_finish: null pointer");
+    PNR_REQUIRE(!labels || (hit_t && hit_box && hit_count && box_ids && label_sem_fine && label_inst_fine),
+                "pnr_coarse_finish: the fine labels need hit_t, hit_box, hit_count, box_ids and both label outputs");
+    PNR_REQUIRE((!fix_sem || label_sem) && (!fix_inst || label_inst), "pnr_coarse_finish: fix_* outputs need their labels");
+    PNR_REQUIRE(desc->plan != 3 || (!rgb && !sem && !inst), "pnr_coarse_finish: a plan-3 (sigma-only) workspace has no rgb, semantic "
+                "or instance maps: pass null for them");
+    PNR_REQUIRE(n_rays * (int64_t)n_coarse < ((int64_t)1 << 31) - 4096, "pnr_coarse_finish: R*N exceeds 2^31");
+    const int rf = record_floats(*desc);
+    const int64_t tiles = (n_rays * n_coarse + 255) / 256 * 8;
+    const float* rec = (const float*)workspace;
+    return pnr_coarse_finish_launch(rec, rf, desc->plan != 3, (const float4*)(rec + tiles * rf), z, fix_sem ? label_sem : nullptr,
+                                    fix_inst ? label_inst : nullptr, n_rays, n_coarse, n_fine, desc->n_sem, desc->n_inst, white_bkgd, rgb,
+                                    depth, acc, weights, sem, inst, fix_sem, fix_inst, z_fine, hit_t, hit_box, hit_count, max_hits, box_ids,
+                                    label_sem_fine, label_inst_fine, (hipStream_t)stream);
+}
+
 PNR_EXPORT int pnr_mlp_forward_composite(const pnr_mlp_desc* desc, const void* packed, const float* rays, const float* z,
                                          int64_t n_rays, int n_samples, const int32_t* label_sem, const int32_t* label_inst,
                                          int white_bkgd, float* rgb, float* depth, float* acc, float* weights, float* sem,
diff --git a/panopticnerf_amd/csrc/pnr_sampling.hip b/panopticnerf_amd/csrc/pnr_sampling.hip
--- a/panopticnerf_amd/csrc/pnr_sampling.hip
+++ b/panopticnerf_amd/csrc/pnr_sampling.hip
@@ -62,10 +62,6 @@
     }
 }
 
-struct PdfLabelArgs {
-    const float* hit_t; const int32_t* hit_box; const int32_t* hit_count; int max_hits; const int32_t* box_ids;
-    int32_t* label_sem; int32_t* label_inst;
-};
 #define PDF_MAXC 256
 #define PDF_MAXT 512
 template <int MAXC, int MAXT, class... Rng>
@@ -158,15 +154,6 @@
     }
 }
 
-__device__ __noinline__ void pdf_bitonic_fallback(float* s_sort, const float* s_z, const float* s_zs, int Nc, int Nf, int P, int lane)
-{
-    const int Nt = Nc + Nf;
-    for (int i = lane; i < Nc; i += 64) s_sort[i] = s_z[i];
-    for (int i = lane; i < Nf; i += 64) s_sort[Nc + i] = s_zs[i];
-    for (int i = Nt + lane; i < P; i += 64) s_sort[i] = INFINITY;
-    __syncthreads();
-    pdf_bitonic(s_sort, P, lane);
-}
 
 #ifndef PDF_DET_WPE
 #define PDF_DET_WPE 8
diff --git a/panopticnerf_amd/csrc/pnr_sampling_dev.h b/panopticnerf_amd/csrc/pnr_sampling_dev.h
--- a/panopticnerf_amd/csrc/pnr_sampling_dev.h
+++ b/panopticnerf_amd/csrc/pnr_sampling_dev.h
@@ -232,3 +232,18 @@
         }
     }
 }
+
+struct PdfLabelArgs {
+    const float* hit_t; const int32_t* hit_box; const int32_t* hit_count; int max_hits; const int32_t* box_ids;
+    int32_t* label_sem; int32_t* label_inst;
+};
+
+__device__ __noinline__ void pdf_bitonic_fallback(float* s_sort, const float* s_z, const float* s_zs, int Nc, int Nf, int P, int lane)
+{
+    const int Nt = Nc + Nf;
+    for (int i = lane; i < Nc; i += 64) s_sort[i] = s_z[i];
+    for (int i = lane; i < Nf; i += 64) s_sort[Nc + i] = s_zs[i];
+    for (int i = Nt + lane; i < P; i += 64) s_sort[i] = INFINITY;
+    __syncthreads();
+    pdf_bitonic(s_sort, P, lane);
+}
diff --git a/panopticnerf_amd/ops.py b/panopticnerf_amd/ops.py
--- a/panopticnerf_amd/ops.py
+++ b/panopticnerf_amd/ops.py
@@ -1731,17 +1731,45 @@
     return "softmax" if int(sem_mode) == 1 else True
 
 
+COARSE_FINISH_MAX_FINE = 192
+COARSE_FINISH_MAX_HITS = 64
+
+
+def coarse_finish_supported(desc, n_coarse, n_importance, max_hits=None):
+    return (int(n_coarse) in (32, 64) and 1 <= int(n_importance) <= COARSE_FINISH_MAX_FINE and desc.n_sem + desc.n_inst <= 128
+            and (max_hits is None or 1 <= int(max_hits) <= COARSE_FINISH_MAX_HITS))
+
+
+class Finish:
+
+    def __init__(self, n_importance, hits=None, box_ids=None, z_out=None):
+        self.n_importance, self.hits, self.box_ids, self.z_out = int(n_importance), hits, box_ids, z_out
+        self.result = None
+
+
+def _done(what, done, z, weights, n_importance, u, out):
+    if done is None:
+        return None
+    if done.result is None or u is not None or done.n_importance != int(n_importance) or done.result[0].shape[0] != z.shape[0]:
+        raise ValueError("%s: done= is the Finish of another call (or of none): n_importance, u = None and the rays must be the level's" % what)
+    if out is not None and out.data_ptr() != done.result[0].data_ptr():
+        out.copy_(done.result[0])
+        return (out,) + tuple(done.result[1:])
+    return done.result
+
+
 @_on_device
 def mlp_forward_composite(desc, packed, rays, z, label_sem=None, label_inst=None, white_bkgd=False, want_weights=True, out=None,
-                          sem_mode=0, wg_cap=0):
+                          sem_mode=0, wg_cap=0, finish=None):
     image = desc
     desc = desc_for_mode(desc, sem_mode)
     if wg_cap:
         desc = _desc_with(desc, flags=(desc.flags & 0xFFFF) | ((int(wg_cap) & 0x1FF) << 16))
-    return _fused_level("mlp_forward_composite", desc, image, packed, rays, z, label_sem, label_inst, white_bkgd, want_weights, out)
-
-
-def _fused_level(what, desc, image, packed, rays, z, label_sem, label_inst, white_bkgd, want_weights, out, drop=()):
+    return _fused_level("mlp_forward_composite", desc, image, packed, rays, z, label_sem, label_inst, white_bkgd, want_weights, out,
+                        finish=finish)
+
+
+def _fused_level(what, desc, image, packed, rays, z, label_sem, label_inst, white_bkgd, want_weights, out, drop=(), finish=None):
     R, N = _level(what, rays, z, image, packed)
     dev = z.device
     label_sem, label_inst = _labels(what, label_sem, label_inst, R * N, dev)
@@ -1752,6 +1780,32 @@
     ws = torch.empty(int(nbytes), device=dev, dtype=torch.uint8)
     out = _maps(out, R, N, desc.n_sem, desc.n_inst, label_sem, label_inst, want_weights, dev, drop=drop)
     g = out.get
+    if finish is not None:
+        Nf, hits, mh = finish.n_importance, finish.hits, None
+        hit_t = hit_box = hit_count = box_ids = ls1 = li1 = None
+        if hits is not None:
+            hit_t, hit_box, hit_count = hits
+            mh = _hit_lists(what, R, hit_t, hit_box, hit_count, dev, "z")
+            box_ids = _chk(finish.box_ids, "box_ids", torch.int32)
+            if box_ids is None:
+                raise ValueError("%s: finish.hits come with finish.box_ids" % what)
+            _on(what, dev, "z", box_ids=box_ids)
+            ls1 = torch.empty((R, N + Nf), device=dev, dtype=torch.int32)
+            li1 = torch.empty((R, N + Nf), device=dev, dtype=torch.int32)
+        if not coarse_finish_supported(desc, N, Nf, mh):
+            raise ValueError("%s: finish= with %d + %d samples, max_hits = %s is outside pnr_coarse_finish's domain "
+                             "(coarse_finish_supported)" % (what, N, Nf, mh))
+        z_fine = _own(finish.z_out, (R, N + Nf), torch.float32, dev, what)
+        if R > 0:
+            _lib.check(lib.pnr_mlp_forward_tiles(ctypes.byref(desc), _p(packed), _p(rays), _p(z), R, N, _p(ws), _stream()),
+                       "pnr_mlp_forward_tiles")
+            _lib.check(lib.pnr_coarse_finish(ctypes.byref(desc), _p(ws), _p(z), R, N, Nf, _p(label_sem), _p(label_inst),
+                                             int(bool(white_bkgd)), _p(g("rgb")), _p(out["depth"]), _p(out["acc"]), _p(g("weights")),
+                                             _p(g("semantic")), _p(g("instance")), _p(g("fix_semantic")), _p(g("fix_instance")),
+                                             _p(z_fine), _p(hit_t), _p(hit_box), _p(hit_count), int(mh or 0), _p(box_ids), _p(ls1),
+                                             _p(li1), _stream()), "pnr_coarse_finish")
+        finish.result = (z_fine, ls1, li1)
+        return out
     _lib.check(lib.pnr_mlp_forward_composite(ctypes.byref(desc), _p(packed), _p(rays), _p(z), R, N, _p(label_sem), _p(label_inst),
                                              int(bool(white_bkgd)), _p(g("rgb")), _p(out["depth"]), _p(out["acc"]),
                                              _p(g("weights")), _p(g("semantic")), _p(g("instance")), _p(g("fix_semantic")),
@@ -1770,10 +1824,22 @@
 
 
 @_on_device
-def mlp_forward_weights(desc, packed, rays, z, label_sem=None, label_inst=None, out=None):
+def mlp_forward_weights(desc, packed, rays, z, label_sem=None, label_inst=None, out=None, finish=None):
     if desc.plan != 3:
         raise ValueError("mlp_forward_weights: needs the plan-3 image (net.packed(level, device, fused='sigma')), not plan %d" % desc.plan)
-    return _fused_level("mlp_forward_weights", desc, desc, packed, rays, z, label_sem, label_inst, False, True, out, WEIGHTS_ONLY_DROPS)
+    return _fused_level("mlp_forward_weights", desc, desc, packed, rays, z, label_sem, label_inst, False, True, out, WEIGHTS_ONLY_DROPS,
+                        finish=finish)
+
+
+def coarse_finish(desc, packed, rays, z, n_importance, label_sem=None, label_inst=None, hits=None, box_ids=None, white_bkgd=False,
+                  want_weights=True, out=None, z_out=None, sem_mode=0, wg_cap=0):
+    fin = Finish(n_importance, hits, box_ids, z_out)
+    if desc.plan == 3:
+        maps = mlp_forward_weights(desc, packed, rays, z, label_sem, label_inst, out=out, finish=fin)
+    else:
+        maps = mlp_forward_composite(desc, packed, rays, z, label_sem, label_inst, white_bkgd, want_weights, out=out, sem_mode=sem_mode,
+                                     wg_cap=wg_cap, finish=fin)
+    return (maps,) + tuple(fin.result)
 
 
 QUERY_WANTS = ("sigma", "labels", "panoptic", "logits")
@@ -1922,7 +1988,12 @@
 
 
 @_on_device
-def sample_pdf(z, weights, n_importance, u=None, want_samples=True, out=None):
+def sample_pdf(z, weights, n_importance, u=None, want_samples=True, out=None, done=None):
+    got = _done("sample_pdf", done, z, weights, n_importance, u, out)
+    if got is not None:
+        if want_samples:
+            raise ValueError("sample_pdf: done= holds z_fine only (want_samples=False)")
+        return got[0], None, None
     u, draw = _draw_or(u, "u")
     R, Nc, dev = _coarse("sample_pdf", z, weights, u, draw, n_importance)
     z_fine = _own(out, (R, Nc + n_importance), torch.float32, dev, "sample_pdf")
@@ -1990,7 +2061,12 @@
 
 
 @_on_device
-def sample_pdf_labels(z, weights, n_importance, hits, box_ids, u=None, out=None):
+def sample_pdf_labels(z, weights, n_importance, hits, box_ids, u=None, out=None, done=None):
+    got = _done("sample_pdf_labels", done, z, weights, n_importance, u, out)
+    if got is not None:
+        if got[1] is None:
+            raise ValueError("sample_pdf_labels: done= was made without hits: it holds no labels")
+        return got
     u, draw = _draw_or(u, "u")
     R, Nc, dev = _coarse("sample_pdf_labels", z, weights, u, draw, n_importance)
     hit_t, hit_box, hit_count = hits
diff --git a/panopticnerf_amd/renderer.py b/panopticnerf_amd/renderer.py
--- a/panopticnerf_amd/renderer.py
+++ b/panopticnerf_amd/renderer.py
@@ -108,6 +108,7 @@
             self.rng_state = torch.tensor([seed, 0], dtype=torch.int64, device=p0.device if p0 is not None else "cpu")
         self.frame_outputs = bool(_get(cfg, "frame_outputs", os.environ.get("PNR_FRAME_OUT", "1") != "0"))
         self.overlap_levels = bool(_get(cfg, "overlap_levels", os.environ.get("PNR_OVERLAP", "1") != "0"))
+        self.coarse_finish = bool(_get(cfg, "coarse_finish", os.environ.get("PNR_COARSE_FINISH", "1") != "0"))
         self._side_streams = {}
         if self.N_importance > 0 and getattr(net, "nerf_1", None) is None and not getattr(net, "share_coarse_fine", False):
             raise ValueError("make_renderer: cfg asks for a fine pass (N_importance / cascade_samples = %d) but the network "
@@ -145,7 +146,7 @@
     def _need_weights(self, lv):
         return self.keep_weights or (lv == 0 and self.N_importance > 0)
 
-    def _level(self, lv, rays, z, labels, noise, out, grad, wg_cap=0):
+    def _level(self, lv, rays, z, labels, noise, out, grad, wg_cap=0, finish=None):
         net, dev = self.net, rays.device
         ls, li = labels
         n0 = net.nerf(0)
@@ -157,23 +158,35 @@
         d = net.nerf(lv).desc(net.precision)
         if weights_only and self.fuse and ops.sigma_pass_supported(d, z.shape[1], noise):
             desc, img = net.packed(0, dev, fused="sigma")
-            return ops.mlp_forward_weights(desc, img, rays, z, ls, li, out=out)
+            return ops.mlp_forward_weights(desc, img, rays, z, ls, li, out=out, finish=finish)
         if not weights_only and self.fuse and ops.fused_supported(d, z.shape[1], self.sem_mode, noise):
             desc, img = net.packed(lv, dev, fused=ops.fused_image(self.sem_mode))
             return ops.mlp_forward_composite(desc, img, rays, z, ls, li, self.white_bkgd, need_w, out=out, sem_mode=self.sem_mode,
-                                             wg_cap=wg_cap)
+                                             wg_cap=wg_cap, finish=finish)
         desc, img = net.packed(lv, dev)
         raw = ops.mlp_forward(desc, img, rays, z, channel_major=True)
         res = ops.composite(raw, z, rays, n0.n_sem, n0.n_inst, True, noise, ls, li, self.sem_mode, self.white_bkgd, need_w, out=out)
         return {k: v for k, v in res.items() if k not in ops.WEIGHTS_ONLY_DROPS} if weights_only else res
 
-    def _resample(self, z, weights, hits, box_ids, u, z_out):
+    def _resample(self, z, weights, hits, box_ids, u, z_out, done=None):
         w0 = weights.detach().contiguous()
         if hits is not None:
-            z_fine, ls1, li1 = ops.sample_pdf_labels(z, w0, self.N_importance, hits, box_ids, u, out=z_out)
+            z_fine, ls1, li1 = ops.sample_pdf_labels(z, w0, self.N_importance, hits, box_ids, u, out=z_out, done=done)
             return z_fine, (ls1, li1)
-        z_fine, _, _ = ops.sample_pdf(z, w0, self.N_importance, u, want_samples=False, out=z_out)
+        z_fine, _, _ = ops.sample_pdf(z, w0, self.N_importance, u, want_samples=False, out=z_out, done=done)
         return z_fine, None
+
+    def _finish(self, z, hits, box_ids, noise, u, grad, z_out):
+        if (not self.coarse_finish or grad or not self.fuse or self.N_importance <= 0 or noise is not None or u is not None
+                or os.environ.get("PNR_SAMPLE_PDF_GENERAL")):
+            return None
+        N = z.shape[1]
+        d = self.net.nerf(0).desc(self.net.precision)
+        fused = (ops.sigma_pass_supported(d, N, noise) if self.coarse_outputs == "weights"
+                 else ops.fused_supported(d, N, self.sem_mode, noise))
+        if not fused or not ops.coarse_finish_supported(d, N, self.N_importance, None if hits is None else hits[0].shape[1]):
+            return None
+        return ops.Finish(self.N_importance, hits, box_ids if hits is not None else None, z_out)
 
     def render_rays(self, rays, box=None, box_ids=None, t_rand=None, u=None, train=False, grad=False, out=None, rng=None):
         Nc, Nf = self.N_samples, self.N_importance
@@ -188,15 +201,18 @@
             self._overflow = over if self._overflow is None else torch.stack([self._overflow[0] + over[0],
                                                                               torch.maximum(self._overflow[1], over[1])])
         lab0 = self._labels(z, hits, box_ids, lab0)
-        o0 = self._level(0, rays, z, lab0, self._noise(0, z, train, rng), _level_out(out, 0), grad)
+        noise0 = self._noise(0, z, train, rng)
+        if Nf <= 0:
+            return _keyed(self._level(0, rays, z, lab0, noise0, _level_out(out, 0), grad), z, 0)
+        if u is None and draw:
+            u = ops.Draw(rng[0], 2, rng[1]) if rng is not None else torch.rand((rays.shape[0], Nf), device=dev)
+        fin = self._finish(z, hits, box_ids, noise0, u, grad, out.get("z_vals_1"))
+        o0 = self._level(0, rays, z, lab0, noise0, _level_out(out, 0), grad, finish=fin)
+        z_fine, lab1 = self._resample(z, o0["weights"], hits, box_ids, u, out.get("z_vals_1"), done=fin)
+        lab1 = self._labels(z_fine, hits, box_ids, lab1)
+        o1 = self._level(1, rays, z_fine, lab1, self._noise(1, z_fine, train, rng), _level_out(out, 1), grad)
         ret = _keyed(o0, z, 0)
-        if Nf > 0:
-            if u is None and draw:
-                u = ops.Draw(rng[0], 2, rng[1]) if rng is not None else torch.rand((rays.shape[0], Nf), device=dev)
-            z_fine, lab1 = self._resample(z, o0["weights"], hits, box_ids, u, out.get("z_vals_1"))
-            lab1 = self._labels(z_fine, hits, box_ids, lab1)
-            o1 = self._level(1, rays, z_fine, lab1, self._noise(1, z_fine, train, rng), _level_out(out, 1), grad)
-            ret.update(_keyed(o1, z_fine, 1))
+        ret.update(_keyed(o1, z_fine, 1))
         return ret
 
     def _output_maps(self, R, has_box, dev, grad=False):
@@ -258,8 +274,9 @@
                     lab0 = self._labels(z, hits, box_ids, lab0)
                     if prev_pdf is not None:
                         st.wait_event(prev_pdf)
-                    o0 = self._level(0, r, z, lab0, None, _level_out(out, 0), False, 0 if ci == 0 else cap_c)
-                    z_fine, lab1 = self._resample(z, o0["weights"], hits, box_ids, None, out["z_vals_1"])
+                    fin = self._finish(z, hits, box_ids, None, None, False, out["z_vals_1"])
+                    o0 = self._level(0, r, z, lab0, None, _level_out(out, 0), False, 0 if ci == 0 else cap_c, finish=fin)
+                    z_fine, lab1 = self._resample(z, o0["weights"], hits, box_ids, None, out["z_vals_1"], done=fin)
                     prev_pdf = torch.cuda.Event()
                     prev_pdf.record(st)
                     if ci + 2 <= last:
```
